# umautobots/LONER

Hardware: AMD Instinct MI355X
Metric: training rays/sec (higher is better)
Workload: dtype f32

## Files before the change

include/loner_hip.h:

```cpp
#ifndef LONER_HIP_H
#define LONER_HIP_H

#include <stddef.h>
#include <stdint.h>

#ifdef __cplusplus
extern "C" {
#endif

#define LNR_RAY_STRIDE 13
#define LNR_LOSS_RAYS_PER_BLOCK 4
#define LNR_MAX_LEVELS 32

typedef enum LnrStatus {
    LNR_OK = 0,
    LNR_ERR_INVALID_ARG = -1,
    LNR_ERR_UNSUPPORTED = -2,
    LNR_ERR_LAUNCH = -3,
    LNR_ERR_WORKSPACE = -4
} LnrStatus;

typedef enum LnrEncoding { LNR_ENC_HASHGRID = 0, LNR_ENC_FREQUENCY = 1 } LnrEncoding;

typedef enum LnrPrecision { LNR_PREC_F32 = 0, LNR_PREC_F16 = 1, LNR_PREC_F32_CHAIN = 2 } LnrPrecision;

typedef enum LnrPosRounding { LNR_POS_FMA = 0, LNR_POS_MUL_ADD = 1 } LnrPosRounding;

#define LNR_POISON_NAN_LOSS 1
#define LNR_POISON_POSE_GRAD 2
#define LNR_POISON_POSE 3

#define LNR_BWD_TABLE_ATOMICS 1
#define LNR_BWD_BINS 4
#define LNR_BWD_BINS_W8 8
#define LNR_BWD_DEFER_WEIGHT_FOLD 16
#define LNR_BWD_REPORT_REGIONS 2
#define LNR_BWD_OVERWRITE_GRAD 32

typedef enum LnrActivation {
    LNR_ACT_NONE = 0, LNR_ACT_RELU = 1, LNR_ACT_SINE = 2, LNR_ACT_LEAKY_RELU = 3,
    LNR_ACT_EXPONENTIAL = 4, LNR_ACT_SIGMOID = 5, LNR_ACT_SQUAREPLUS = 6,
    LNR_ACT_SOFTPLUS = 7, LNR_ACT_TANH = 8
} LnrActivation;

typedef struct LnrNetSpec {
    int32_t encoding;
    int32_t n_levels;
    int32_t n_features;
    int32_t log2_table;
    int32_t base_res;
    float   per_level_scale;
    int32_t n_frequencies;
    int32_t activation;
    int32_t n_neurons;
    int32_t n_hidden;
    int32_t precision;
    int32_t pos_rounding;
    int32_t enc_dim;
    int32_t in_dim;
    int32_t n_mlp_params;
    int64_t n_params;
    float    level_scale[LNR_MAX_LEVELS];
    uint32_t level_res[LNR_MAX_LEVELS];
    uint32_t level_size[LNR_MAX_LEVELS];
    uint32_t level_offset[LNR_MAX_LEVELS];
    uint32_t level_hashed[LNR_MAX_LEVELS];
} LnrNetSpec;

typedef struct LnrLossConfig {
    int32_t selection;
    float min_js, max_js, js_alpha;
    float los_lambda;
    float depth_lambda;
    float min_eps;
    float fixed_eps;
} LnrLossConfig;

const char* lnr_last_error(void);
int  lnr_version(void);

int lnr_profile_enable(int32_t on);
int lnr_profile_read(char* names, int32_t name_stride, float* total_ms, int32_t* calls, int32_t capacity);

int lnr_net_spec_finalize(LnrNetSpec* spec );

size_t lnr_density_workspace(const LnrNetSpec* spec , int64_t n_points);
size_t lnr_density_workspace_forward(const LnrNetSpec* spec , int64_t n_points);

typedef enum LnrRouteKind {
    LNR_ROUTE_UNSUPPORTED = 0, LNR_ROUTE_WIDE = 1, LNR_ROUTE_F16_FAST = 2, LNR_ROUTE_F16_FREQ = 3, LNR_ROUTE_F16_GEN = 4,
    LNR_ROUTE_BF3 = 5, LNR_ROUTE_FAST32 = 6, LNR_ROUTE_REGS = 7, LNR_ROUTE_LDS = 8
} LnrRouteKind;
typedef struct LnrDensityRoute { int32_t kind, w_lds, waves, dw64, f16_part; } LnrDensityRoute;
int lnr_density_route(const LnrNetSpec* spec , int64_t n_points, int32_t backward, LnrDensityRoute* out );

#define LNR_WORKSPACE_STATUS_BYTES 256
#define LNR_STATUS_CLIPPED 0
#define LNR_STATUS_OVF_LEVEL0 16
int lnr_density_workspace_init(void* workspace, size_t workspace_bytes, void* stream);
int lnr_density_workspace_release(void* workspace);

int lnr_density_forward(const LnrNetSpec* spec , const float* params,
                        const float* pts, int64_t n_points,
                        const float* rays, const float* z, int32_t n_rays, int32_t n_samples,
                        const int32_t* n_rays_dev,
                        float* sigma ,
                        void* workspace, size_t workspace_bytes, void* stream);

int lnr_density_backward(const LnrNetSpec* spec , const float* params,
                         const float* pts, int64_t n_points,
                         const float* rays, const float* z, int32_t n_rays, int32_t n_samples,
                         const int32_t* n_rays_dev,
                         const float* d_sigma, float* grad_params, float* d_pts, float* d_rays,
                         int32_t reuse_features, int32_t flags, void* workspace, size_t workspace_bytes,
                         void* input_grad_event ,
                         void* stream);

int lnr_density_fold_weight_grads(const LnrNetSpec* spec , int64_t n_points, float* grad_params,
                                  void* workspace, size_t workspace_bytes, int32_t flags, void* stream);

int lnr_build_lidar_rays(const float* directions , const float* distances ,
                         int64_t n_points, const int64_t* index , int32_t n_index,
                         const float* transform , float range_min, float range_max,
                         float scale, const float* shift ,
                         float* rays , float* depths ,
                         uint8_t* keep , void* stream);

int lnr_build_window_rays(const float* const* directions, const float* const* distances, const float* const_distance,
                          const int64_t* n_points, const int32_t* seg_start, const int32_t* seg_pose, int32_t n_seg,
                          const int64_t* index, int64_t* index_out, uint64_t seed, const float* transforms,
                          float range_min, float range_max, float scale, const float* shift ,
                          float* rays, float* depths, uint8_t* keep, void* stream);

int lnr_build_camera_rays(const float* directions , int64_t n_pixels, const int64_t* index ,
                          int32_t n_rays, int32_t width, const float* transform , float range_min, float scale,
                          const float* shift , float* rays , void* stream);

int lnr_pose_forward(const float* pose6, int32_t n, float* transforms, void* stream);
int lnr_pose_backward(const float* pose6, const float* d_transforms, const uint8_t* mask, int32_t n, float* d_pose6,
                      int32_t accumulate, int32_t* poison_dev, int32_t poison_tag, void* stream);

int lnr_compact_rays(const float* rays_in, const float* depths_in, const uint8_t* keep, const int64_t* src_index,
                     int32_t n_in, const int32_t* seg_start , int32_t n_seg,
                     float* rays_out, float* depths_out, int64_t* src_index_out,
                     int32_t* out_seg_start, int32_t* n_out_dev, void* stream);

int lnr_compact_rays_front(const float* rays_in, const float* depths_in, const uint8_t* keep, const int64_t* src_index,
                           int32_t n_in, const int32_t* seg_start , int32_t n_seg,
                           float* rays_out, float* depths_out, int64_t* src_index_out,
                           int32_t* out_seg_start, int32_t* n_out_dev,
                           int32_t* counts_dev , const int32_t* seg_order , int32_t cap,
                           float* record , void* stream);

int lnr_first_ray_key(const float* rays, const int32_t* out_seg_start , const int32_t* seg_order ,
                      int32_t n_seg, int64_t* key_out , void* stream);

#define LNR_FRONT_HEADER 4
int lnr_shard_front_pack(const float* rays, const int32_t* out_seg_start , const int32_t* seg_order ,
                         int32_t n_seg, const float* depths, int32_t n_rays, const int32_t* n_rays_dev, int32_t cap,
                         float* record , void* stream);
int lnr_shard_front_reduce(const float* records , int32_t world, int32_t stride,
                           int32_t* counts_dev , float* far0_dev , void* stream);

#define LNR_COMM_ID_BYTES 128
typedef enum LnrCommDtype { LNR_COMM_F32 = 0, LNR_COMM_BF16 = 1, LNR_COMM_I64 = 2, LNR_COMM_I32 = 3, LNR_COMM_U8 = 4 } LnrCommDtype;
typedef enum LnrCommOp { LNR_COMM_SUM = 0, LNR_COMM_MIN = 1, LNR_COMM_MAX = 2 } LnrCommOp;
int lnr_comm_available(void);
int lnr_comm_unique_id(void* id , size_t id_bytes);
int lnr_comm_init(const void* id, size_t id_bytes, int32_t rank, int32_t world, void** comm_out);
int lnr_comm_destroy(void* comm);
int lnr_comm_all_reduce(void* comm, void* buf, size_t count, int32_t dtype , int32_t op , void* stream);
int lnr_comm_reduce_scatter(void* comm, const void* send, void* recv, size_t recv_count, int32_t dtype, void* stream);
int lnr_comm_all_gather(void* comm, const void* send, void* recv, size_t bytes_per_rank, void* stream);
int lnr_comm_broadcast(void* comm, void* buf, size_t bytes, int32_t root, void* stream);

int lnr_lidar_rays_backward(const float* d_rays , const float* rays ,
                            const int64_t* src_index , const int32_t* seg_start ,
                            int32_t n_seg, const float* const* directions ,
                            const int64_t* n_points , const float* transforms ,
                            float scale, float* d_transform , void* stream);

int lnr_occ_interpolate(const float* grid , int32_t V, const float* pts ,
                        int64_t n, float* out , void* stream);

int lnr_sample_rays_occ(const float* rays, int32_t n_rays, const int32_t* n_rays_dev,
                        const float* grid, int32_t V, int32_t n_samples, float perturb,
                        const float* steps, const float* u_jitter, const float* u_pdf, uint64_t seed,
                        float* z_out ,
                        int64_t* dbg_inds, float* dbg_probs, float* dbg_cdf, void* stream);

int lnr_sample_rays_uniform(const float* rays, int32_t n_rays, const int32_t* n_rays_dev,
                            int32_t n_samples, float perturb, const float* steps,
                            const float* u_jitter, uint64_t seed, float* z_out, void* stream);

#define LNR_DRAW_JITTER 0
#define LNR_DRAW_PDF 1
#define LNR_DRAW_NOISE 2
#define LNR_DRAW_RAY_INDEX 16
int lnr_rng_draws(int32_t which, uint64_t seed, int32_t n_rays, int32_t n_per_ray, float* out , void* stream);

int lnr_render_forward(const float* sigma, const float* z, const float* rays, int32_t n_rays,
                       const int32_t* n_rays_dev, int32_t n_samples,
                       const float* noise, float noise_std, uint64_t seed,
                       float* depth, float* weights, float* opacity, float* variance, void* stream);

int lnr_render_forward_peak(const float* sigma, const float* z, const float* rays, int32_t n_rays,
                            const int32_t* n_rays_dev, int32_t n_samples,
                            const float* noise, float noise_std, uint64_t seed,
                            float* depth, float* opacity, float* variance, float* peak_z, int32_t* peak_index, void* stream);

int lnr_depth_colormap(const float* values, int64_t n, float multiplier, double min_depth, double max_depth,
                       const uint8_t* table , uint8_t* rgba , void* stream);

int lnr_render_backward(const float* sigma, const float* z, const float* rays, int32_t n_rays,
                        const int32_t* n_rays_dev, int32_t n_samples,
                        const float* noise, float noise_std, uint64_t seed,
                        const float* g_depth, const float* g_weights, const float* g_opacity,
                        const float* g_variance, float* d_sigma, float* d_rays, void* stream);

int lnr_points_grad_to_rays(const float* d_pts , const float* z, int32_t n_rays,
                            const int32_t* n_rays_dev, int32_t n_samples, float* d_rays, void* stream);

typedef struct LnrMeshGrid {
    int32_t n[3];
    float lo[3], hi[3];
    double first[3], inv_step[3];
    const double* axis[3];
} LnrMeshGrid;

int lnr_render_mesh_accumulate(const float* sigma, const float* z, const float* rays, int32_t n_rays, const int32_t* n_rays_dev,
                               int32_t n_samples, const float* noise, float noise_std, uint64_t seed, const LnrMeshGrid* grid,
                               float depth_max, int32_t use_var, float var_max, float* volume, uint64_t* counters, void* stream);

#define LNR_MC_TABLE_WIDTH 16
size_t lnr_mc_workspace(int32_t nx, int32_t ny, int32_t nz);
int lnr_mc_count(const float* volume, int32_t nx, int32_t ny, int32_t nz, float level, void* workspace, size_t workspace_bytes,
                 uint64_t* totals_dev, void* stream);
int lnr_mc_emit(const float* volume, int32_t nx, int32_t ny, int32_t nz, float level, const float* spacing ,
                const float* origin , void* workspace, size_t workspace_bytes, int64_t n_verts, int64_t n_tris,
                float* verts, int32_t* tris, void* stream);
int lnr_mc_case_table(int8_t* out);

size_t lnr_cloud_workspace(int64_t n_points);

int lnr_lidar_scan_points(const float* depth, const float* variance, const int64_t* ray_index, int64_t n_rays,
                          const float* directions, int64_t n_directions, float scale, float var_max, float depth_max,
                          void* workspace, size_t workspace_bytes, double* points, int32_t* n_points_dev, void* stream);

int lnr_voxel_down_sample(const double* points, int64_t n_points, const int32_t* n_points_dev, double voxel_size,
                          void* workspace, size_t workspace_bytes, double* out, int64_t* info_dev, void* stream);

int lnr_cloud_append_transformed(const double* src, int64_t n_points, const double* transform, double* dst, void* stream);

size_t lnr_nn_grid_bytes(int64_t n_targets);
int lnr_nn_grid_build(const double* targets, int64_t n_targets, double cell_edge, void* workspace, size_t workspace_bytes,
                      void* grid, size_t grid_bytes, int64_t* info_dev, void* stream);

int lnr_nn_distance(const void* grid, int64_t n_targets, const double* queries, int64_t n_queries, double* distance,
                    double* sq_distance, void* workspace, size_t workspace_bytes, int64_t* counters_dev, void* stream);

#define LNR_KNN_MAX 32
#define LNR_ICP_RESULT 64

int lnr_cloud_normals(const void* grid, int64_t n_points, int32_t knn, double* normals, double* covariances, void* workspace,
                      size_t workspace_bytes, int64_t* counters_dev, void* stream);

int lnr_icp_correspondences(const void* grid, int64_t n_targets, const double* queries, int64_t n_queries, double max_distance,
                            int32_t* index, double* sq_distance, int64_t* counters_dev, void* stream);

size_t lnr_icp_workspace(int64_t n_source);
int lnr_icp_point_to_plane(const void* grid, int64_t n_targets, const double* target_normals, const double* source, int64_t n_source,
                           double max_distance, const double* init, double relative_fitness, double relative_rmse, int32_t max_iteration,
                           void* workspace, size_t workspace_bytes, double* result_dev, int64_t* info_dev, void* stream);

size_t lnr_mesh_sample_workspace(int64_t n_triangles);
int lnr_mesh_sample_points(const double* vertices, int64_t n_vertices, const int32_t* triangles, int64_t n_triangles, int64_t n_points,
                           uint64_t seed, void* workspace, size_t workspace_bytes, double* points, int32_t* triangle_index,
                           int64_t* info_dev, void* stream);

size_t lnr_cloud_tools_workspace(int64_t n_points);

int lnr_cloud_knn_mean_distance(const void* grid, int64_t n_points, int32_t nb_neighbors, double* mean_distance, void* workspace,
                                size_t workspace_bytes, int64_t* counters_dev, void* stream);

int lnr_cloud_outlier_threshold(const void* grid, const double* mean_distance, int64_t n_points, double std_ratio, void* workspace,
                                size_t workspace_bytes, double* result_dev, void* stream);

int lnr_cloud_trajectory_transform(const double* points, const double* timestamps, int64_t n_points, const double* traj_times,
                                   const double* traj_positions, const double* traj_rotations, const double* traj_rotvecs,
                                   int64_t n_poses, double min_range, void* workspace, size_t workspace_bytes, double* out,
                                   int64_t* info_dev, void* stream);

#define LNR_MOCOMP_CONSTS 30
#define LNR_SKY_MAX_RAYS 65160

int lnr_frame_cloud(const float* ray_directions, const float* distances, int64_t n_points, int64_t start, int64_t stop, int64_t step,
                    double* points, void* stream);

int lnr_motion_compensate(float* ray_directions, float* distances, const void* timestamps, int32_t timestamps_fp64, int64_t n_points,
                          double t0, double denom, const double* consts , void* stream);

size_t lnr_sky_rays_workspace(void);
int lnr_sky_rays(const float* ray_directions, int64_t n_points, const float* rotation, void* workspace, size_t workspace_bytes,
                 float* sky, int64_t sky_stride, int32_t* info_dev, void* stream);

#define LNR_SCAN_MAX_FOV_SEGMENTS 8
#define LNR_SCAN_TIME_NONE 0
#define LNR_SCAN_TIME_GIVEN 1
#define LNR_SCAN_TIME_RECOMPUTE 2
#define LNR_SCAN_NANOSECONDS 1
#define LNR_SCAN_NEGATIVE_START 2
#define LNR_SCAN_LOCAL 4
#define LNR_SCAN_GLOBAL 8
#define LNR_SCAN_CONSTANT 16
#define LNR_SCAN_NO_TIMES 32

size_t lnr_scan_from_points_workspace(int64_t n_points);
int lnr_scan_from_points(const float* xyz, const float* point_times , int64_t n_points, int32_t time_mode, float stamp,
                         int32_t fov_enabled, const float* fov_segments , int32_t n_fov_segments, float min_range,
                         void* workspace, size_t workspace_bytes, float* ray_directions, float* distances, float* timestamps,
                         int64_t* order, int64_t* info_dev, void* stream);

int lnr_weights_gt(const float* s , const float* g , const float* eps_ray,
                   float eps_scalar, int32_t normalise, int32_t n_rays, int32_t n_samples,
                   float* out , void* stream);

int lnr_logits_grad(const float* s , const float* g , int32_t n_rays, int32_t n_samples,
                    float margin, float l_free, float l_occ, float* out, void* stream);

int lnr_render_ftb_gather(const float* rays, const float* z, int32_t n_samples, const int32_t* idx, const int32_t* n_alive_dev,
                          int32_t cap, int32_t b0, int32_t block_samples, float* rays_c , float* z_c ,
                          int32_t* next_count_dev, void* stream);
int lnr_render_ftb_composite(const float* sigma_c , const float* z, const float* rays, int32_t n_samples, const int32_t* idx,
                             const int32_t* n_alive_dev, int32_t cap, int32_t b0, int32_t block_samples,
                             const float* noise , float noise_std, uint64_t seed, float* transmittance, float* depth_acc, float* opacity_acc, int32_t* next_idx, int32_t* next_count_dev,
                             int32_t last, void* stream);

int lnr_count_opaque(const float* rays, const float* depth_gt, int32_t n_rays, const int32_t* n_rays_dev,
                     const float* far0_dev, int32_t* counts_dev , void* stream);
int lnr_los_loss_fused(const float* sigma, const float* z, const float* rays, const float* depth_gt,
                       int32_t n_rays, const int32_t* n_rays_dev, int32_t n_samples,
                       const float* noise, float noise_std, uint64_t seed,
                       float scale, const LnrLossConfig* cfg , const int32_t* counts_dev, const float* far0_dev,
                       float* loss_out, float* d_sigma, float* d_rays, float* ray_stats,
                       float* weights_out, float* block_partials, int32_t* poison_dev, int32_t poison_tag, void* stream);

int lnr_adam_step(float* params, float* grads, float* exp_avg, float* exp_avg_sq, int64_t count,
                  float lr, float beta1, float beta2, float eps, int32_t step, float grad_scale,
                  int32_t zero_grad, const int32_t* poison_dev, void* stream);

int lnr_occ_grid_step(float* grid, int32_t V, const float* rays, const float* z, const float* depth_gt,
                      int32_t n_rays, const int32_t* n_rays_dev, int32_t n_samples, float scale,
                      float lr, float margin, float l_free, float l_occ, int64_t* grad_acc, void* stream);
int lnr_occ_grid_apply(float* grid, int64_t* grad_acc, int64_t count, float lr, int32_t zero_grad, const int32_t* poison_dev,
                       void* stream);

int lnr_selftest_mfma(float* out , void* stream);

#ifdef __cplusplus
}
#endif
#endif
```

loner_amd/csrc/lnr_pose.hip:

```cpp
#include "lnr_common.h"

struct QuatParts { float w, x, y, z, k, theta, half; bool small; };

__device__ __forceinline__ QuatParts pose_quat(const float* __restrict__ p) {
    QuatParts q;
    const float a = p[3], b = p[4], c = p[5];
    q.theta = sqrtf(a * a + b * b + c * c);
    q.half = 0.5f * q.theta;
    q.small = fabsf(q.theta) < 1e-6f;
    q.k = q.small ? 0.5f - q.theta * q.theta / 48.0f : sinf(q.half) / q.theta;
    q.w = cosf(q.half); q.x = a * q.k; q.y = b * q.k; q.z = c * q.k;
    return q;
}

__global__ void pose_forward_kernel(const float* __restrict__ pose6, int n, float* __restrict__ T12) {
    const int i = blockIdx.x * blockDim.x + threadIdx.x;
    if (i >= n) return;
    const float* p = pose6 + 6 * i;
    const QuatParts q = pose_quat(p);
    const float w = q.w, x = q.x, y = q.y, z = q.z;
    const float s2 = 2.0f / (w * w + x * x + y * y + z * z);
    float* T = T12 + 12 * i;
    T[0] = 1.0f - s2 * (y * y + z * z); T[1] = s2 * (x * y - z * w);        T[2] = s2 * (x * z + y * w);        T[3] = p[0];
    T[4] = s2 * (x * y + z * w);        T[5] = 1.0f - s2 * (x * x + z * z); T[6] = s2 * (y * z - x * w);        T[7] = p[1];
    T[8] = s2 * (x * z - y * w);        T[9] = s2 * (y * z + x * w);        T[10] = 1.0f - s2 * (x * x + y * y); T[11] = p[2];
}

__global__ void pose_backward_kernel(const float* __restrict__ pose6, const float* __restrict__ dT12, const uint8_t* __restrict__ mask,
                                     int n, float* __restrict__ d_pose6, int accumulate, int32_t* __restrict__ poison, int32_t poison_tag) {
    const int i = blockIdx.x * blockDim.x + threadIdx.x;
    if (i >= n) return;
    const float* p = pose6 + 6 * i;
    const float* G = dT12 + 12 * i;
    const QuatParts q = pose_quat(p);
    const float w = q.w, x = q.x, y = q.y, z = q.z;
    const float nn = w * w + x * x + y * y + z * z;
    const float s2 = 2.0f / nn;
    const float G00 = G[0], G01 = G[1], G02 = G[2], G10 = G[4], G11 = G[5], G12 = G[6], G20 = G[8], G21 = G[9], G22 = G[10];
    const float d_s2 = -G00 * (y * y + z * z) + G01 * (x * y - z * w) + G02 * (x * z + y * w) + G10 * (x * y + z * w) - G11 * (x * x + z * z) +
                       G12 * (y * z - x * w) + G20 * (x * z - y * w) + G21 * (y * z + x * w) - G22 * (x * x + y * y);
    float dw = s2 * (-z * G01 + y * G02 + z * G10 - x * G12 - y * G20 + x * G21);
    float dx = s2 * (y * G01 + z * G02 + y * G10 - 2.0f * x * G11 - w * G12 + z * G20 + w * G21 - 2.0f * x * G22);
    float dy = s2 * (-2.0f * y * G00 + x * G01 + w * G02 + x * G10 + z * G12 - w * G20 + z * G21 - 2.0f * y * G22);
    float dz = s2 * (-2.0f * z * G00 - w * G01 + x * G02 + w * G10 - 2.0f * z * G11 + y * G12 + x * G20 + y * G21);
    const float ds2_dq = -0.5f * s2 * s2 * 2.0f;
    dw += d_s2 * ds2_dq * w; dx += d_s2 * ds2_dq * x; dy += d_s2 * ds2_dq * y; dz += d_s2 * ds2_dq * z;
    const float a = p[3], b = p[4], c = p[5];
    const float dk = q.small ? -q.theta / 24.0f : (0.5f * cosf(q.half) * q.theta - sinf(q.half)) / (q.theta * q.theta);
    const float d_theta = dk * (a * dx + b * dy + c * dz) - 0.5f * sinf(q.half) * dw;
    const float inv_theta = q.theta > 0.0f ? 1.0f / q.theta : 0.0f;
    const float m = mask ? (mask[i] ? 1.0f : 0.0f) : 1.0f;
    float out[6];
    out[0] = G[3]; out[1] = G[7]; out[2] = G[11];
    out[3] = q.k * dx + d_theta * a * inv_theta;
    out[4] = q.k * dy + d_theta * b * inv_theta;
    out[5] = q.k * dz + d_theta * c * inv_theta;
    float* o = d_pose6 + 6 * i;
    bool bad_grad = false, bad_pose = false;
    for (int j = 0; j < 6; ++j) {
        const float v = (accumulate ? o[j] : 0.0f) + (m != 0.0f ? out[j] : 0.0f);
        o[j] = v;
        bad_grad |= !isfinite(v);
        bad_pose |= !isfinite(p[j]);
    }
    if (poison != nullptr && (bad_grad || bad_pose) && atomicCAS(poison, 0, bad_grad ? LNR_POISON_POSE_GRAD : LNR_POISON_POSE) == 0)
        poison[1] = poison_tag;
}

extern "C" int lnr_pose_forward(const float* pose6, int32_t n, float* transforms, void* stream) {
    LNR_REQUIRE(pose6 && transforms && n >= 0, "lnr_pose_forward: bad argument");
    if (n == 0) return LNR_OK;
    hipLaunchKernelGGL(pose_forward_kernel, dim3(lnr_div_up(n, 64)), dim3(64), 0, (hipStream_t)stream, pose6, n, transforms);
    LNR_CHECK_LAUNCH("lnr_pose_forward");
    return LNR_OK;
}

extern "C" int lnr_pose_backward(const float* pose6, const float* d_transforms, const uint8_t* mask, int32_t n, float* d_pose6,
                                 int32_t accumulate, int32_t* poison_dev, int32_t poison_tag, void* stream) {
    LNR_REQUIRE(pose6 && d_transforms && d_pose6 && n >= 0, "lnr_pose_backward: bad argument");
    if (n == 0) return LNR_OK;
    hipLaunchKernelGGL(pose_backward_kernel, dim3(lnr_div_up(n, 64)), dim3(64), 0, (hipStream_t)stream, pose6, d_transforms, mask, n,
                       d_pose6, accumulate, poison_dev, poison_tag);
    LNR_CHECK_LAUNCH("lnr_pose_backward");
    return LNR_OK;
}
```

loner_amd/csrc/lnr_rays.hip:

```cpp
#include "lnr_common.h"

#define LNR_MAX_SEG 64

struct SegTable {
    int32_t n;
    int32_t start[LNR_MAX_SEG + 1];
};
struct DirTable {
    const float* dirs[LNR_MAX_SEG];
    int64_t n_points[LNR_MAX_SEG];
};

__device__ __forceinline__ float cube_exit(const float o[3], const float d[3], int* axis_out, float* t_out, float* dd_out) {
    float best = 0.0f;
    int best_axis = 0;
    float best_t = 0.0f, best_dd = 1.0f;
#pragma unroll
    for (int a = 0; a < 3; ++a) {
        const float dd = d[a] + 1e-15f;
        const float t_lo = (-1.0f - o[a]) / dd;
        const float t_hi = (1.0f - o[a]) / dd;
        const float c_lo = fmaxf(t_lo, 0.0f), c_hi = fmaxf(t_hi, 0.0f);
        const bool hi_sel = c_hi > c_lo;
        const float c = hi_sel ? c_hi : c_lo;
        const float t_raw = hi_sel ? t_hi : t_lo;
        if (a == 0 || c < best) { best = c; best_axis = a; best_t = t_raw; best_dd = dd; }
    }
    if (axis_out) { *axis_out = best_axis; *t_out = best_t; *dd_out = best_dd; }
    return best;
}

__global__ void build_lidar_rays_kernel(const float* __restrict__ directions, const float* __restrict__ distances, int64_t n_points,
                                        const int64_t* __restrict__ index, int n_index, const float* __restrict__ T,
                                        float range_min, float range_max, float scale, float sx, float sy, float sz,
                                        float* __restrict__ rays, float* __restrict__ depths, uint8_t* __restrict__ keep) {
    const int i = blockIdx.x * blockDim.x + threadIdx.x;
    if (i >= n_index) return;
    const int64_t src = index[i];
    const float l0 = directions[src], l1 = directions[n_points + src], l2 = directions[2 * n_points + src];
    const float dist = distances[src];
    float o[3], d[3];
    o[0] = (T[3] + sx) / scale;
    o[1] = (T[7] + sy) / scale;
    o[2] = (T[11] + sz) / scale;
    float v[3];
#pragma unroll
    for (int r = 0; r < 3; ++r) v[r] = T[4 * r] * l0 + T[4 * r + 1] * l1 + T[4 * r + 2] * l2;
    const float nrm = sqrtf(v[0] * v[0] + v[1] * v[1] + v[2] * v[2]);
#pragma unroll
    for (int r = 0; r < 3; ++r) d[r] = v[r] / nrm;
    const float near = range_min / scale;
    const float far_range = range_max / scale;
    const float far = fminf(far_range, cube_exit(o, d, nullptr, nullptr, nullptr));
    float* rec = rays + (size_t)i * LNR_RAY_STRIDE;
    rec[0] = o[0]; rec[1] = o[1]; rec[2] = o[2];
    rec[3] = d[0]; rec[4] = d[1]; rec[5] = d[2];
    rec[6] = -d[0]; rec[7] = -d[1]; rec[8] = -d[2];
    rec[9] = 0.0f; rec[10] = 0.0f;
    rec[11] = near; rec[12] = far;
    depths[i] = dist / scale;
    keep[i] = (far > near + 1.0f / scale) ? 1 : 0;
}

extern "C" int lnr_build_lidar_rays(const float* directions, const float* distances, int64_t n_points, const int64_t* index,
                                    int32_t n_index, const float* transform, float range_min, float range_max, float scale,
                                    const float* shift, float* rays, float* depths, uint8_t* keep, void* stream) {
    LNR_REQUIRE(directions && distances && index && transform && shift && rays && depths && keep, "lnr_build_lidar_rays: null argument");
    LNR_REQUIRE(n_points > 0 && n_index >= 0 && scale > 0.0f, "lnr_build_lidar_rays: bad sizes");
    if (n_index == 0) return LNR_OK;
    hipLaunchKernelGGL(build_lidar_rays_kernel, dim3(lnr_div_up(n_index, 256)), dim3(256), 0, (hipStream_t)stream, directions, distances,
                       n_points, index, n_index, transform, range_min, range_max, scale, shift[0], shift[1], shift[2], rays, depths, keep);
    LNR_CHECK_LAUNCH("lnr_build_lidar_rays");
    return LNR_OK;
}

struct WindowTable {
    int32_t n_seg;
    int32_t start[LNR_MAX_SEG + 1];
    int32_t pose[LNR_MAX_SEG];
    const float* dirs[LNR_MAX_SEG];
    const float* dist[LNR_MAX_SEG];
    float const_dist[LNR_MAX_SEG];
    int64_t n_points[LNR_MAX_SEG];
};

__global__ void build_window_rays_kernel(const WindowTable tab, const int64_t* __restrict__ index, int64_t* __restrict__ index_out,
                                         uint64_t seed, const float* __restrict__ transforms, float range_min, float range_max,
                                         float scale, float sx, float sy, float sz, float* __restrict__ rays,
                                         float* __restrict__ depths, uint8_t* __restrict__ keep) {
    const int i = blockIdx.x * blockDim.x + threadIdx.x;
    const int total = tab.start[tab.n_seg];
    if (i >= total) return;
    int seg = 0;
    while (seg + 1 < tab.n_seg && i >= tab.start[seg + 1]) ++seg;
    const int64_t n_points = tab.n_points[seg];
    int64_t src;
    if (index) src = index[i];
    else {
        const float u = lnr_rand_uniform(seed, 0x44ull + (uint64_t)seg, (uint64_t)(i - tab.start[seg]) >> 2, (uint32_t)(i - tab.start[seg]) & 3u);
        src = (int64_t)(u * (float)n_points);
        if (src >= n_points) src = n_points - 1;
    }
    if (index_out) index_out[i] = src;
    const float* D = tab.dirs[seg];
    const float l0 = D[src], l1 = D[n_points + src], l2 = D[2 * n_points + src];
    const float dist = tab.dist[seg] ? tab.dist[seg][src] : tab.const_dist[seg];
    const float* T = transforms + 12 * tab.pose[seg];
    float o[3], d[3], v[3];
    o[0] = (T[3] + sx) / scale; o[1] = (T[7] + sy) / scale; o[2] = (T[11] + sz) / scale;
#pragma unroll
    for (int r = 0; r < 3; ++r) v[r] = T[4 * r] * l0 + T[4 * r + 1] * l1 + T[4 * r + 2] * l2;
    const float nrm = sqrtf(v[0] * v[0] + v[1] * v[1] + v[2] * v[2]);
#pragma unroll
    for (int r = 0; r < 3; ++r) d[r] = v[r] / nrm;
    const float near = range_min / scale;
    const float far = fminf(range_max / scale, cube_exit(o, d, nullptr, nullptr, nullptr));
    float* rec = rays + (size_t)i * LNR_RAY_STRIDE;
    rec[0] = o[0]; rec[1] = o[1]; rec[2] = o[2];
    rec[3] = d[0]; rec[4] = d[1]; rec[5] = d[2];
    rec[6] = -d[0]; rec[7] = -d[1]; rec[8] = -d[2];
    rec[9] = 0.0f; rec[10] = 0.0f; rec[11] = near; rec[12] = far;
    depths[i] = dist / scale;
    keep[i] = (far > near + 1.0f / scale) ? 1 : 0;
}

extern "C" int lnr_build_window_rays(const float* const* directions, const float* const* distances, const float* const_distance,
                                     const int64_t* n_points, const int32_t* seg_start, const int32_t* seg_pose, int32_t n_seg,
                                     const int64_t* index, int64_t* index_out, uint64_t seed, const float* transforms,
                                     float range_min, float range_max, float scale, const float* shift, float* rays, float* depths,
                                     uint8_t* keep, void* stream) {
    LNR_REQUIRE(directions && distances && const_distance && n_points && seg_start && seg_pose && transforms && shift && rays && depths && keep,
                "lnr_build_window_rays: null argument");
    LNR_REQUIRE(n_seg >= 1 && n_seg <= LNR_MAX_SEG, "lnr_build_window_rays: n_seg must be in [1,%d]", LNR_MAX_SEG);
    LNR_REQUIRE(index != nullptr || index_out != nullptr, "lnr_build_window_rays: need index or index_out");
    WindowTable tab;
    tab.n_seg = n_seg;
    for (int s = 0; s < n_seg; ++s) {
        tab.start[s] = seg_start[s]; tab.pose[s] = seg_pose[s]; tab.dirs[s] = directions[s]; tab.dist[s] = distances[s];
        tab.const_dist[s] = const_distance[s]; tab.n_points[s] = n_points[s];
        LNR_REQUIRE(directions[s] != nullptr && n_points[s] > 0, "lnr_build_window_rays: segment %d has no points", s);
    }
    tab.start[n_seg] = seg_start[n_seg];
    const int total = seg_start[n_seg];
    if (total <= 0) return LNR_OK;
    hipLaunchKernelGGL(build_window_rays_kernel, dim3(lnr_div_up(total, 256)), dim3(256), 0, (hipStream_t)stream, tab, index, index_out, seed,
                       transforms, range_min, range_max, scale, shift[0], shift[1], shift[2], rays, depths, keep);
    LNR_CHECK_LAUNCH("lnr_build_window_rays");
    return LNR_OK;
}

__global__ void build_camera_rays_kernel(const float* __restrict__ directions, int64_t n_pixels, const int64_t* __restrict__ index, int n_rays, int width,
                                         const float* __restrict__ T, float range_min, float scale, float sx, float sy, float sz,
                                         float* __restrict__ rays) {
// ... 13 lines not shown
    o[2] = (T[11] + sz) / scale;
#pragma unroll
    for (int r = 0; r < 3; ++r) v[r] = T[4 * r] * l0 + T[4 * r + 1] * l1 + T[4 * r + 2] * l2;
    const float nrm = sqrtf(v[0] * v[0] + v[1] * v[1] + v[2] * v[2]);
#pragma unroll
    for (int r = 0; r < 3; ++r) d[r] = v[r] / nrm;
    rec[0] = o[0]; rec[1] = o[1]; rec[2] = o[2];
    rec[3] = d[0]; rec[4] = d[1]; rec[5] = d[2];
    rec[6] = -d[0]; rec[7] = -d[1]; rec[8] = -d[2];
    rec[9] = (float)(src % width); rec[10] = (float)(src / width);
    rec[11] = range_min / scale;
    rec[12] = cube_exit(o, d, nullptr, nullptr, nullptr);
}

extern "C" int lnr_build_camera_rays(const float* directions, int64_t n_pixels, const int64_t* index, int32_t n_rays, int32_t width,
                                     const float* transform, float range_min, float scale, const float* shift, float* rays, void* stream) {
    LNR_REQUIRE(directions && transform && shift && rays, "lnr_build_camera_rays: null argument");
    LNR_REQUIRE(n_pixels > 0 && n_rays >= 0 && width > 0 && scale > 0.0f, "lnr_build_camera_rays: bad sizes");
    LNR_REQUIRE(index != nullptr || (int64_t)n_rays <= n_pixels, "lnr_build_camera_rays: %d rays of an image of %lld pixels", n_rays, (long long)n_pixels);
    if (n_rays == 0) return LNR_OK;
    hipLaunchKernelGGL(build_camera_rays_kernel, dim3(lnr_div_up(n_rays, 256)), dim3(256), 0, (hipStream_t)stream, directions, n_pixels, index,
                       n_rays, width, transform, range_min, scale, shift[0], shift[1], shift[2], rays);
    LNR_CHECK_LAUNCH("lnr_build_camera_rays");
    return LNR_OK;
}

struct SegOrder { int n; int order[LNR_MAX_SEG]; };
struct CompactTail { int32_t* counts; float* record; int cap; SegOrder ord; };

__global__ void __launch_bounds__(1024)
compact_rays_kernel(const float* __restrict__ rays_in, const float* __restrict__ depths_in, const uint8_t* __restrict__ keep,
                    const int64_t* __restrict__ src_in, int n_in, const SegTable seg, float* __restrict__ rays_out,
                    float* __restrict__ depths_out, int64_t* __restrict__ src_out, int32_t* __restrict__ out_seg_start,
                    int32_t* __restrict__ n_out, const CompactTail tail) {
    __shared__ int wave_tot[16];
    __shared__ int running;
    const int tid = threadIdx.x, lane = tid & 63, wave = tid >> 6;
    if (tid == 0) running = 0;
    __syncthreads();
    for (int base = 0; base < n_in; base += 1024) {
        const int i = base + tid;
        const bool k = (i < n_in) && keep[i];
        const unsigned long long b = __ballot(k);
        const int within = __popcll(b & ((1ull << lane) - 1ull));
        if (lane == 0) wave_tot[wave] = __popcll(b);
        __syncthreads();
        int before = running;
        for (int w = 0; w < wave; ++w) before += wave_tot[w];
        const int pos = before + within;
        if (i < n_in) {
            for (int s = 0; s <= seg.n; ++s) if (seg.start[s] == i) out_seg_start[s] = pos;
        }
        if (k) {
            const float* a = rays_in + (size_t)i * LNR_RAY_STRIDE;
            float* o = rays_out + (size_t)pos * LNR_RAY_STRIDE;
#pragma unroll
            for (int c = 0; c < LNR_RAY_STRIDE; ++c) o[c] = a[c];
            depths_out[pos] = depths_in[i];
            if (src_out) src_out[pos] = src_in[i];
        }
        __syncthreads();
        if (tid == 0) { int t = 0; for (int w = 0; w < 16; ++w) t += wave_tot[w]; running += t; }
        __syncthreads();
    }
    if (tid <= seg.n && seg.start[tid] >= n_in) out_seg_start[tid] = running;
    if (tid == 0) *n_out = running;
    if (tail.counts == nullptr && tail.record == nullptr) return;
    __syncthreads();
    const int n = running;
    if (tail.counts != nullptr) {
        __shared__ int partial[16];
        const float far0 = n > 0 ? rays_out[12] : 0.0f;
        int c = 0;
        for (int i = tid; i < n; i += 1024) {
            const float d = depths_out[i];
            c += ((d > 0.0f) && !(d > far0)) ? 1 : 0;
        }
        for (int o = 32; o > 0; o >>= 1) c += __shfl_xor(c, o, 64);
        if (lane == 0) partial[wave] = c;
        __syncthreads();
        if (tid == 0) {
            int t = 0;
            for (int w = 0; w < 16; ++w) t += partial[w];
            tail.counts[0] = n;
            tail.counts[1] = t;
        }
    }
    if (tail.record != nullptr) {
        const int m = min(n, tail.cap);
        if (tid == 0) {
            long long k = 0x7FFFFFFFFFFFFFFFll;
            for (int sgi = 0; sgi < tail.ord.n; ++sgi) {
                const int lo = out_seg_start[sgi], hi = out_seg_start[sgi + 1];
                if (hi > lo) {
                    k = ((long long)tail.ord.order[sgi] << 32) | (long long)__float_as_uint(rays_out[(size_t)lo * LNR_RAY_STRIDE + 12]);
                    break;
                }
            }
            tail.record[0] = __uint_as_float((uint32_t)((unsigned long long)k & 0xFFFFFFFFull));
            tail.record[1] = __uint_as_float((uint32_t)((unsigned long long)k >> 32));
            tail.record[2] = __int_as_float(m);
            tail.record[3] = 0.0f;
        }
        for (int i = tid; i < tail.cap; i += 1024) tail.record[LNR_FRONT_HEADER + i] = i < m ? depths_out[i] : 0.0f;
    }
}

extern "C" int lnr_compact_rays(const float* rays_in, const float* depths_in, const uint8_t* keep, const int64_t* src_index, int32_t n_in,
                                const int32_t* seg_start, int32_t n_seg, float* rays_out, float* depths_out, int64_t* src_index_out,
                                int32_t* out_seg_start, int32_t* n_out_dev, void* stream) {
    LNR_REQUIRE(rays_in && depths_in && keep && seg_start && rays_out && depths_out && out_seg_start && n_out_dev, "lnr_compact_rays: null argument");
    LNR_REQUIRE(n_seg >= 1 && n_seg <= LNR_MAX_SEG, "lnr_compact_rays: n_seg must be in [1,%d]", LNR_MAX_SEG);
    LNR_REQUIRE((src_index == nullptr) == (src_index_out == nullptr), "lnr_compact_rays: src_index in/out must both be given or both be null");
    SegTable seg;
    seg.n = n_seg;
    for (int s = 0; s <= n_seg; ++s) seg.start[s] = seg_start[s];
    LNR_REQUIRE(seg.start[0] == 0 && seg.start[n_seg] == n_in, "lnr_compact_rays: seg_start must run from 0 to n_in");
    CompactTail tail;
    tail.counts = nullptr; tail.record = nullptr; tail.cap = 0; tail.ord.n = 0;
    hipLaunchKernelGGL(compact_rays_kernel, dim3(1), dim3(1024), 0, (hipStream_t)stream, rays_in, depths_in, keep, src_index, n_in, seg,
                       rays_out, depths_out, src_index_out, out_seg_start, n_out_dev, tail);
    LNR_CHECK_LAUNCH("lnr_compact_rays");
    return LNR_OK;
}

extern "C" int lnr_compact_rays_front(const float* rays_in, const float* depths_in, const uint8_t* keep, const int64_t* src_index, int32_t n_in,
                                      const int32_t* seg_start, int32_t n_seg, float* rays_out, float* depths_out, int64_t* src_index_out,
                                      int32_t* out_seg_start, int32_t* n_out_dev, int32_t* counts_dev, const int32_t* seg_order, int32_t cap,
                                      float* record, void* stream) {
    LNR_REQUIRE(rays_in && depths_in && keep && seg_start && rays_out && depths_out && out_seg_start && n_out_dev, "lnr_compact_rays_front: null argument");
    LNR_REQUIRE(n_seg >= 1 && n_seg <= LNR_MAX_SEG, "lnr_compact_rays_front: n_seg must be in [1,%d]", LNR_MAX_SEG);
    LNR_REQUIRE((src_index == nullptr) == (src_index_out == nullptr), "lnr_compact_rays_front: src_index in/out must both be given or both be null");
    LNR_REQUIRE((counts_dev != nullptr) != (record != nullptr), "lnr_compact_rays_front: pass counts_dev (unsharded batch) or record (sharded), one of them");
    SegTable seg;
    seg.n = n_seg;
    for (int s = 0; s <= n_seg; ++s) seg.start[s] = seg_start[s];
    LNR_REQUIRE(seg.start[0] == 0 && seg.start[n_seg] == n_in, "lnr_compact_rays_front: seg_start must run from 0 to n_in");
    CompactTail tail;
    tail.counts = counts_dev; tail.record = record; tail.cap = cap; tail.ord.n = 0;
    if (record != nullptr) {
        LNR_REQUIRE(seg_order != nullptr && cap >= n_in, "lnr_compact_rays_front: a front record of %d depth slots cannot hold the %d candidate rays of this rank", cap, n_in);
        tail.ord.n = n_seg;
        for (int s = 0; s < n_seg; ++s) {
            LNR_REQUIRE(seg_order[s] >= 0 && (s == 0 || seg_order[s] > seg_order[s - 1]), "lnr_compact_rays_front: seg_order must be non-negative and ascending");
            tail.ord.order[s] = seg_order[s];
        }
    }
    hipLaunchKernelGGL(compact_rays_kernel, dim3(1), dim3(1024), 0, (hipStream_t)stream, rays_in, depths_in, keep, src_index, n_in, seg,
                       rays_out, depths_out, src_index_out, out_seg_start, n_out_dev, tail);
    LNR_CHECK_LAUNCH("lnr_compact_rays_front");
    return LNR_OK;
}

__global__ void first_ray_key_kernel(const float* __restrict__ rays, const int32_t* __restrict__ out_seg_start, const SegOrder ord, long long* __restrict__ key) {
    if (threadIdx.x != 0 || blockIdx.x != 0) return;
    long long k = 0x7FFFFFFFFFFFFFFFll;
    for (int s = 0; s < ord.n; ++s) {
        const int lo = out_seg_start[s], hi = out_seg_start[s + 1];
        if (hi > lo) {
            k = ((long long)ord.order[s] << 32) | (long long)__float_as_uint(rays[(size_t)lo * LNR_RAY_STRIDE + 12]);
            break;
        }
    }
    *key = k;
}

extern "C" int lnr_first_ray_key(const float* rays, const int32_t* out_seg_start, const int32_t* seg_order, int32_t n_seg, int64_t* key_out, void* stream) {
    LNR_REQUIRE(rays && out_seg_start && seg_order && key_out, "lnr_first_ray_key: null argument");
    LNR_REQUIRE(n_seg >= 1 && n_seg <= LNR_MAX_SEG, "lnr_first_ray_key: n_seg must be in [1,%d]", LNR_MAX_SEG);
    SegOrder ord;
    ord.n = n_seg;
    for (int s = 0; s < n_seg; ++s) {
        LNR_REQUIRE(seg_order[s] >= 0 && (s == 0 || seg_order[s] > seg_order[s - 1]), "lnr_first_ray_key: seg_order must be non-negative and ascending");
        ord.order[s] = seg_order[s];
    }
    hipLaunchKernelGGL(first_ray_key_kernel, dim3(1), dim3(64), 0, (hipStream_t)stream, rays, out_seg_start, ord, reinterpret_cast<long long*>(key_out));
    LNR_CHECK_LAUNCH("lnr_first_ray_key");
    return LNR_OK;
}

__global__ void __launch_bounds__(256)
shard_front_pack_kernel(const float* __restrict__ rays, const int32_t* __restrict__ out_seg_start, const SegOrder ord,
                        const float* __restrict__ depths, int n_rays, const int32_t* __restrict__ n_rays_dev, int cap, float* __restrict__ rec) {
    const int n = min(lnr_live_rays(n_rays, n_rays_dev), cap);
    if (threadIdx.x == 0) {
        long long k = 0x7FFFFFFFFFFFFFFFll;
        for (int s = 0; s < ord.n; ++s) {
            const int lo = out_seg_start[s], hi = out_seg_start[s + 1];
            if (hi > lo) {
                k = ((long long)ord.order[s] << 32) | (long long)__float_as_uint(rays[(size_t)lo * LNR_RAY_STRIDE + 12]);
                break;
            }
        }
        rec[0] = __uint_as_float((uint32_t)((unsigned long long)k & 0xFFFFFFFFull));
        rec[1] = __uint_as_float((uint32_t)((unsigned long long)k >> 32));
        rec[2] = __int_as_float(n);
        rec[3] = 0.0f;
    }
    for (int i = threadIdx.x; i < cap; i += blockDim.x) rec[LNR_FRONT_HEADER + i] = i < n ? depths[i] : 0.0f;
}

__global__ void __launch_bounds__(1024)
shard_front_reduce_kernel(const float* __restrict__ recs, int world, int stride, int32_t* __restrict__ counts, float* __restrict__ far0_out) {
    __shared__ int partial[16];
    unsigned long long kmin = 0x7FFFFFFFFFFFFFFFull;
    int n_all = 0;
    for (int r = 0; r < world; ++r) {
        const float* rec = recs + (size_t)r * stride;
        const unsigned long long k = (unsigned long long)__float_as_uint(rec[0]) | ((unsigned long long)__float_as_uint(rec[1]) << 32);
        kmin = k < kmin ? k : kmin;
        n_all += max(0, min(__float_as_int(rec[2]), stride - LNR_FRONT_HEADER));
    }
    const float far0 = __uint_as_float((uint32_t)(kmin & 0xFFFFFFFFull));
    int c = 0;
    for (int r = 0; r < world; ++r) {
        const float* rec = recs + (size_t)r * stride;
        const int n = max(0, min(__float_as_int(rec[2]), stride - LNR_FRONT_HEADER));
        for (int i = threadIdx.x; i < n; i += blockDim.x) {
            const float d = rec[LNR_FRONT_HEADER + i];
            c += ((d > 0.0f) && !(d > far0)) ? 1 : 0;
        }
    }
    for (int o = 32; o > 0; o >>= 1) c += __shfl_xor(c, o, 64);
    if ((threadIdx.x & 63) == 0) partial[threadIdx.x >> 6] = c;
    __syncthreads();
    if (threadIdx.x == 0) {
        int t = 0;
        for (int w = 0; w < (int)(blockDim.x >> 6); ++w) t += partial[w];
        counts[0] = n_all;
        counts[1] = t;
        far0_out[0] = far0;
    }
}

extern "C" int lnr_shard_front_pack(const float* rays, const int32_t* out_seg_start, const int32_t* seg_order, int32_t n_seg,
                                    const float* depths, int32_t n_rays, const int32_t* n_rays_dev, int32_t cap, float* record, void* stream) {
    LNR_REQUIRE(record && cap >= 0 && n_rays >= 0 && n_seg >= 0 && n_seg <= LNR_MAX_SEG, "lnr_shard_front_pack: bad argument");
    LNR_REQUIRE(n_seg == 0 || (rays && out_seg_start && seg_order && depths), "lnr_shard_front_pack: null argument");
    LNR_REQUIRE(n_seg == 0 || n_rays <= cap, "lnr_shard_front_pack: a front record of %d depth slots cannot hold the %d rays of this rank "
                "(every rank must size its record for the fullest rank: DistContext.front_capacity)", cap, n_rays);
    SegOrder ord;
    ord.n = n_seg;
    for (int s = 0; s < n_seg; ++s) {
        LNR_REQUIRE(seg_order[s] >= 0 && (s == 0 || seg_order[s] > seg_order[s - 1]), "lnr_shard_front_pack: seg_order must be non-negative and ascending");
        ord.order[s] = seg_order[s];
    }
    hipLaunchKernelGGL(shard_front_pack_kernel, dim3(1), dim3(256), 0, (hipStream_t)stream, rays, out_seg_start, ord, depths,
                       n_seg == 0 ? 0 : n_rays, n_seg == 0 ? nullptr : n_rays_dev, cap, record);
    LNR_CHECK_LAUNCH("lnr_shard_front_pack");
    return LNR_OK;
}

extern "C" int lnr_shard_front_reduce(const float* records, int32_t world, int32_t stride, int32_t* counts_dev, float* far0_dev, void* stream) {
    LNR_REQUIRE(records && counts_dev && far0_dev && world >= 1 && stride >= LNR_FRONT_HEADER, "lnr_shard_front_reduce: bad argument");
    hipLaunchKernelGGL(shard_front_reduce_kernel, dim3(1), dim3(1024), 0, (hipStream_t)stream, records, world, stride, counts_dev, far0_dev);
    LNR_CHECK_LAUNCH("lnr_shard_front_reduce");
    return LNR_OK;
}

__global__ void __launch_bounds__(256)
lidar_rays_backward_kernel(const float* __restrict__ d_rays, const float* __restrict__ rays, const int64_t* __restrict__ src_index,
                           const int32_t* __restrict__ seg_start, const DirTable dirs, const float* __restrict__ transforms,
                           float scale, float far_range_unused, float* __restrict__ d_transform) {
    __shared__ float red[4][12];
    const int seg = blockIdx.x;
    const int lo = seg_start[seg], hi = seg_start[seg + 1];
    const float* T = transforms + seg * 12;
    const float* D = dirs.dirs[seg];
    const int64_t n = dirs.n_points[seg];
    float acc[12];
#pragma unroll
    for (int k = 0; k < 12; ++k) acc[k] = 0.0f;
    for (int ray = lo + threadIdx.x; ray < hi; ray += blockDim.x) {
        const float* g = d_rays + (size_t)ray * LNR_RAY_STRIDE;
        const float* rec = rays + (size_t)ray * LNR_RAY_STRIDE;
        const int64_t src = src_index[ray];
        const float l[3] = {D[src], D[n + src], D[2 * n + src]};
        float go[3] = {g[0], g[1], g[2]};
        float gd[3] = {g[3] - g[6], g[4] - g[7], g[5] - g[8]};
        const float gfar = g[12];
        const float o[3] = {rec[0], rec[1], rec[2]};
        const float d[3] = {rec[3], rec[4], rec[5]};
        if (gfar != 0.0f) {
            int axis; float t_raw, dd;
            const float clip = cube_exit(o, d, &axis, &t_raw, &dd);
            if (clip <= rec[12] && t_raw > 0.0f) {
                const float inv = 1.0f / dd;
                const float go_a = -gfar * inv, gd_a = -gfar * t_raw * inv;
                if (axis == 0) { go[0] += go_a; gd[0] += gd_a; } else if (axis == 1) { go[1] += go_a; gd[1] += gd_a; } else { go[2] += go_a; gd[2] += gd_a; }
            }
        }
        float v[3];
#pragma unroll
        for (int r = 0; r < 3; ++r) v[r] = T[4 * r] * l[0] + T[4 * r + 1] * l[1] + T[4 * r + 2] * l[2];
        const float nrm = sqrtf(v[0] * v[0] + v[1] * v[1] + v[2] * v[2]);
        const float dot = d[0] * gd[0] + d[1] * gd[1] + d[2] * gd[2];
#pragma unroll
        for (int r = 0; r < 3; ++r) {
            const float gv = (gd[r] - d[r] * dot) / nrm;
            acc[4 * r + 0] += gv * l[0];
            acc[4 * r + 1] += gv * l[1];
            acc[4 * r + 2] += gv * l[2];
            acc[4 * r + 3] += go[r] / scale;
        }
    }
    const int lane = threadIdx.x & 63, wave = threadIdx.x >> 6;
// ... 22 lines not shown
```

loner_amd/csrc/lnr_render.hip:

```cpp
#include "lnr_common.h"
#include "lnr_render_ray.h"

__device__ __forceinline__ float wave_excl_suffix_sum(float v, int lane) {
    float inc = v;
#pragma unroll
    for (int o = 1; o < 64; o <<= 1) {
        float t = __shfl_down(inc, o, 64);
        if (lane + o < 64) inc += t;
    }
    float ex = __shfl_down(inc, 1, 64);
    return lane == 63 ? 0.0f : ex;
}

template <int C>
__device__ __forceinline__ void render_ray_backward(const RayState<C>& st, const float G[C], float g_far, int ray, int S, int lane,
                                                    const float* __restrict__ rayrec, float* __restrict__ d_sigma,
                                                    float* __restrict__ d_rays) {
    const int base = lane * C;
    float gw[C];
    float local = 0.0f;
#pragma unroll
    for (int t = 0; t < C; ++t) { gw[t] = G[t] * st.w[t]; local += gw[t]; }
    const float behind_lanes = wave_excl_suffix_sum(local, lane);
    float suffix = behind_lanes;
// ... 41 lines not shown
    if (lane == 0) {
        if (depth) depth[ray] = st.depth;
        if (opacity) opacity[ray] = st.opacity;
        if (variance) variance[ray] = st.variance;
    }
}

template <int C>
__global__ void __launch_bounds__(RENDER_BLOCK)
render_backward_kernel(const float* __restrict__ sigma, const float* __restrict__ z, const float* __restrict__ rays, int n_rays,
                       const int32_t* __restrict__ n_rays_dev, int S, const float* __restrict__ noise, float noise_std,
                       uint64_t seed, const float* __restrict__ g_depth, const float* __restrict__ g_weights,
                       const float* __restrict__ g_opacity, const float* __restrict__ g_variance,
                       float* __restrict__ d_sigma, float* __restrict__ d_rays) {
    const int lane = threadIdx.x & 63;
    const int ray = blockIdx.x * RAYS_PER_BLOCK + (threadIdx.x >> 6);
    if (ray >= lnr_live_rays(n_rays, n_rays_dev)) return;
    const float* rr = rays + (size_t)ray * LNR_RAY_STRIDE;
    RayState<C> st;
    render_ray<C>(st, sigma, z, noise, noise_std, seed, ray, S, lane, rr);
    const float gD = g_depth ? g_depth[ray] : 0.0f;
    const float gO = g_opacity ? g_opacity[ray] : 0.0f;
    const float gV = g_variance ? g_variance[ray] : 0.0f;
    float q_part = 0.0f;
#pragma unroll
    for (int t = 0; t < C; ++t) q_part += st.w[t] * (st.depth - st.z[t]);
    const float gD_tot = gD + gV * 2.0f * wave_sum(q_part);
    const float far = rr[12];
    float G[C];
#pragma unroll
    for (int t = 0; t < C; ++t) {
        const int i = lane * C + t;
        const float q = st.depth - st.z[t];
        float g = gO + gD_tot * (st.z[t] - far) + gV * q * q;
        if (g_weights && i < S) g += g_weights[(size_t)ray * S + i];
        G[t] = (i < S) ? g : 0.0f;
    }
    render_ray_backward<C>(st, G, gD_tot * (1.0f - st.opacity), ray, S, lane, rr, d_sigma, d_rays);
}

__device__ __forceinline__ float std_normal_cdf(float x) { return 0.5f * (1.0f + erff(x / 1.41421356237309515f)); }

__device__ __forceinline__ float target_raw(float s, float g, float eps, float sd, float clip_norm) {
    const bool inside = (s - (g - eps) > 0.0f) && ((g + eps) - s > 0.0f);
    if (!inside) return 0.0f;
    const float t = (s - g) / sd;
    return 0.39894228040143270f * expf(-0.5f * (t * t)) / sd / clip_norm;
}

__device__ __forceinline__ void target_params(float g, float eps, float* sd, float* clip_norm) {
    *sd = eps / 3.0f;
    const float lo = (g - eps - g) / *sd;
    const float hi = (g + eps - g) / *sd;
    *clip_norm = std_normal_cdf(hi) - std_normal_cdf(lo);
}

__device__ __forceinline__ float gaussian_kl(float m1, float s1, float m2, float s2) {
    const float d = m1 - m2;
    return logf(s2 / s1) + (s1 * s1 + d * d) / (2.0f * (s2 * s2)) - 0.5f;
}
__device__ __forceinline__ float gaussian_js(float m1, float s1, float m2, float s2) {
    const float mm = 0.5f * (m1 + m2);
    const float sm = 0.5f * sqrtf(s1 * s1 + s2 * s2);
    return 0.5f * gaussian_kl(m1, s1, mm, sm) + 0.5f * gaussian_kl(m2, s2, mm, sm);
}

template <int C>
__device__ __forceinline__ void los_loss_ray(const float* __restrict__ sigma, const float* __restrict__ z, const float* __restrict__ rays,
                                             const float* __restrict__ depth_gt, int S, const float* __restrict__ noise, float noise_std,
                                             uint64_t seed, float scale, const LnrLossConfig& cfg, const int32_t* __restrict__ counts,
                                             float* terms, bool terms_atomic, float* __restrict__ d_sigma, float* __restrict__ d_rays,
                                             float* __restrict__ ray_stats, float* __restrict__ weights_out, int ray, int lane,
                                             const float* __restrict__ far0_dev) {
    const float* rr = rays + (size_t)ray * LNR_RAY_STRIDE;
    RayState<C> st;
    render_ray<C>(st, sigma, z, noise, noise_std, seed, ray, S, lane, rr);

    const float dgt = depth_gt[ray];
    const float far0 = far0_dev ? far0_dev[0] : rays[12];
    const bool opaque = (dgt > 0.0f) && !(dgt > far0);
    const float g = dgt * scale;
    const float n_all = (float)counts[0] * (float)S;
    const float n_op = (float)counts[1];

    float m_part = 0.0f;
#pragma unroll
    for (int t = 0; t < C; ++t) m_part += (st.z[t] * scale) * st.w[t];
    const float wden = st.opacity + 1e-10f;
    const float mean = wave_sum(m_part) / wden;
    float v_part = 0.0f;
#pragma unroll
    for (int t = 0; t < C; ++t) { const float q = st.z[t] * scale - mean; v_part += q * q * st.w[t]; }
    const float var = wave_sum(v_part) / wden + 1e-10f;
    const float sd_pred = sqrtf(var);
    const float js = gaussian_js(g, cfg.min_eps / 3.0f, mean, sd_pred);

    float eps;
    if (cfg.selection <= 1) {
        float score = js;
        if (score < cfg.min_js) score = 0.0f;
        if (score > cfg.max_js) score = cfg.max_js;
        eps = cfg.min_eps * (1.0f + cfg.js_alpha * score);
    } else {
        eps = cfg.fixed_eps;
    }
    float sd_t, clip_norm;
    target_params(g, eps, &sd_t, &clip_norm);
    float raw[C];
    float r_part = 0.0f;
#pragma unroll
    for (int t = 0; t < C; ++t) {
        raw[t] = (lane * C + t < S) ? target_raw(st.z[t] * scale, g, eps, sd_t, clip_norm) : 0.0f;
        r_part += raw[t];
    }
    const float rden = wave_sum(r_part) + 1e-6f;

    const bool l1 = (cfg.selection == 0 || cfg.selection == 2);
    const float depth_m = st.depth * scale;
    const float gO = opaque ? ((st.opacity - 1.0f > 0.0f) ? 1.0f : (st.opacity - 1.0f < 0.0f ? -1.0f : 0.0f)) / n_op : 0.0f;
    const float gD = opaque ? cfg.depth_lambda * 2.0f * (depth_m - g) * scale / n_op : 0.0f;
    const float far = rr[12];
    float G[C];
    float los_part = 0.0f;
#pragma unroll
    for (int t = 0; t < C; ++t) {
        const int i = lane * C + t;
        const float target = opaque ? raw[t] / rden : 0.0f;
        const float diff = st.w[t] - target;
        float gw;
        if (l1) { los_part += fabsf(diff); gw = (diff > 0.0f ? 1.0f : (diff < 0.0f ? -1.0f : 0.0f)); }
        else { los_part += diff * diff; gw = 2.0f * diff; }
        G[t] = (i < S) ? cfg.los_lambda * gw / n_all + gO + gD * (st.z[t] - far) : 0.0f;
        if (weights_out && i < S) weights_out[(size_t)ray * S + i] = st.w[t];
    }
    const float los_sum = wave_sum(los_part);
    render_ray_backward<C>(st, G, gD * (1.0f - st.opacity), ray, S, lane, rr, d_sigma, d_rays);

    if (lane == 0) {
        const float l_depth = opaque ? cfg.depth_lambda * (depth_m - g) * (depth_m - g) / n_op : 0.0f;
        const float l_los = cfg.los_lambda * los_sum / n_all;
        const float l_op = opaque ? fabsf(st.opacity - 1.0f) / n_op : 0.0f;
        const float t5[5] = {l_depth + l_los + l_op, l_depth, l_los, l_op, eps};
#pragma unroll
        for (int q = 0; q < 5; ++q) { if (terms_atomic) atomicAdd(terms + q, t5[q]); else terms[q] = t5[q]; }
        if (ray_stats) {
            float* o = ray_stats + (size_t)ray * 8;
            o[0] = st.depth; o[1] = st.opacity; o[2] = st.variance; o[3] = mean; o[4] = sd_pred; o[5] = js; o[6] = eps;
            o[7] = opaque ? 1.0f : 0.0f;
        }
    }
}


template <int C>
__global__ void __launch_bounds__(RENDER_BLOCK)
los_loss_fused_kernel(const float* __restrict__ sigma, const float* __restrict__ z, const float* __restrict__ rays,
                      const float* __restrict__ depth_gt, int n_rays, const int32_t* __restrict__ n_rays_dev, int S,
                      const float* __restrict__ noise, float noise_std, uint64_t seed, float scale, const LnrLossConfig cfg,
                      const int32_t* __restrict__ counts, float* __restrict__ loss_out, float* __restrict__ d_sigma,
                      float* __restrict__ d_rays, float* __restrict__ ray_stats, float* __restrict__ weights_out,
                      float* __restrict__ block_partials, const float* __restrict__ far0_dev) {
    __shared__ float s_terms[RAYS_PER_BLOCK][5];
    const int lane = threadIdx.x & 63;
    const int ray = blockIdx.x * RAYS_PER_BLOCK + (threadIdx.x >> 6);
    const bool alive = ray < lnr_live_rays(n_rays, n_rays_dev);
    if (block_partials) {
        if (lane < 5) s_terms[threadIdx.x >> 6][lane] = 0.0f;
        if (alive) los_loss_ray<C>(sigma, z, rays, depth_gt, S, noise, noise_std, seed, scale, cfg, counts, s_terms[threadIdx.x >> 6], false,
                                   d_sigma, d_rays, ray_stats, weights_out, ray, lane, far0_dev);
        __syncthreads();
        if (threadIdx.x < 8) {
            float v = 0.0f;
            if (threadIdx.x < 5) for (int r = 0; r < RAYS_PER_BLOCK; ++r) v += s_terms[r][threadIdx.x];
            block_partials[(size_t)blockIdx.x * 8 + threadIdx.x] = v;
        }
    } else if (alive) {
        los_loss_ray<C>(sigma, z, rays, depth_gt, S, noise, noise_std, seed, scale, cfg, counts, loss_out, true,
                        d_sigma, d_rays, ray_stats, weights_out, ray, lane, far0_dev);
    }
}

__global__ void loss_reduce_kernel(const float* __restrict__ block_partials, int n_blocks, float* __restrict__ loss_out,
                                   int32_t* __restrict__ poison, int32_t poison_tag) {
    __shared__ float part[4][8];
    const int term = threadIdx.x & 7, slice = threadIdx.x >> 3;
    float v = 0.0f;
    for (int b = slice; b < n_blocks; b += 32) v += block_partials[(size_t)b * 8 + term];
    v += __shfl_xor(v, 8, 64); v += __shfl_xor(v, 16, 64); v += __shfl_xor(v, 32, 64);
    if ((threadIdx.x & 63) < 8) part[threadIdx.x >> 6][term] = v;
    __syncthreads();
    if (threadIdx.x < 5) {
        const float t = loss_out[threadIdx.x] + (part[0][threadIdx.x] + part[1][threadIdx.x] + part[2][threadIdx.x] + part[3][threadIdx.x]);
        loss_out[threadIdx.x] = t;
        if (threadIdx.x == 0 && poison != nullptr && t != t && atomicCAS(poison, 0, LNR_POISON_NAN_LOSS) == 0) poison[1] = poison_tag;
    }
}

__global__ void count_opaque_kernel(const float* __restrict__ rays, const float* __restrict__ depth_gt, int n_rays,
                                    const int32_t* __restrict__ n_rays_dev, int32_t* __restrict__ counts,
                                    const float* __restrict__ far0_dev) {
    __shared__ int partial[16];
    const int n = lnr_live_rays(n_rays, n_rays_dev);
    const float far0 = far0_dev ? far0_dev[0] : (n > 0 ? rays[12] : 0.0f);
    int c = 0;
    for (int i = threadIdx.x; i < n; i += blockDim.x) {
        const float d = depth_gt[i];
        c += ((d > 0.0f) && !(d > far0)) ? 1 : 0;
    }
    for (int o = 32; o > 0; o >>= 1) c += __shfl_xor(c, o, 64);
    if ((threadIdx.x & 63) == 0) partial[threadIdx.x >> 6] = c;
    __syncthreads();
    if (threadIdx.x == 0) {
        int t = 0;
        for (int w = 0; w < (int)(blockDim.x >> 6); ++w) t += partial[w];
        counts[0] = n;
        counts[1] = t;
    }
}

__global__ void weights_gt_kernel(const float* __restrict__ s, const float* __restrict__ g, const float* __restrict__ eps_ray,
                                  float eps_scalar, int normalise, int n_rays, int S, float* __restrict__ out) {
    const int lane = threadIdx.x & 63;
    const int ray = blockIdx.x * RAYS_PER_BLOCK + (threadIdx.x >> 6);
    if (ray >= n_rays) return;
    const float gg = g[ray];
    const float eps = eps_ray ? eps_ray[ray] : eps_scalar;
    float sd, cn;
    target_params(gg, eps, &sd, &cn);
    float part = 0.0f;
    for (int i = lane; i < S; i += 64) part += target_raw(s[(size_t)ray * S + i], gg, eps, sd, cn);
    const float den = wave_sum(part) + 1e-6f;
    for (int i = lane; i < S; i += 64) {
        const float v = target_raw(s[(size_t)ray * S + i], gg, eps, sd, cn);
        out[(size_t)ray * S + i] = normalise ? v / den : v;
    }
}

__global__ void logits_grad_kernel(const float* __restrict__ s, const float* __restrict__ g, int64_t total, int S, float margin,
                                   float l_free, float l_occ, float* __restrict__ out) {
    const int64_t i = (int64_t)blockIdx.x * blockDim.x + threadIdx.x;
    if (i >= total) return;
    const float x = s[i] - g[i / S];
    const float free_side = (-x - margin > 0.0f) ? 1.0f : 0.0f;
    const float near_surface = ((x + margin > 0.0f) && (margin - x > 0.0f)) ? 1.0f : 0.0f;
    out[i] = l_free * free_side - l_occ * near_surface;
}

__global__ void points_grad_to_rays_kernel(const float* __restrict__ d_pts, const float* __restrict__ z, int n_rays,
                                           const int32_t* __restrict__ n_rays_dev, int S, float* __restrict__ d_rays) {
    const int lane = threadIdx.x & 63;
    const int ray = blockIdx.x * RAYS_PER_BLOCK + (threadIdx.x >> 6);
    if (ray >= lnr_live_rays(n_rays, n_rays_dev)) return;
    float a[6] = {0.0f, 0.0f, 0.0f, 0.0f, 0.0f, 0.0f};
    for (int i = lane; i < S; i += 64) {
        const size_t m = (size_t)ray * S + i;
        const float zv = z[m];
        const float gx = d_pts[3 * m], gy = d_pts[3 * m + 1], gz = d_pts[3 * m + 2];
        a[0] += gx; a[1] += gy; a[2] += gz;
        a[3] += zv * gx; a[4] += zv * gy; a[5] += zv * gz;
    }
#pragma unroll
    for (int k = 0; k < 6; ++k) a[k] = wave_sum(a[k]);
    if (lane < 6) {
        float v = lane == 0 ? a[0] : lane == 1 ? a[1] : lane == 2 ? a[2] : lane == 3 ? a[3] : lane == 4 ? a[4] : a[5];
        d_rays[(size_t)ray * LNR_RAY_STRIDE + lane] += v;
    }
}


extern "C" int lnr_render_forward(const float* sigma, const float* z, const float* rays, int32_t n_rays, const int32_t* n_rays_dev,
                                  int32_t n_samples, const float* noise, float noise_std, uint64_t seed, float* depth,
                                  float* weights, float* opacity, float* variance, void* stream) {
    LNR_REQUIRE(sigma && z && rays && n_rays >= 0 && n_samples >= 2, "lnr_render_forward: bad argument");
    if (n_rays == 0) return LNR_OK;
    const dim3 grid(lnr_div_up(n_rays, RAYS_PER_BLOCK)), block(RENDER_BLOCK);
    hipStream_t st = (hipStream_t)stream;
    DISPATCH_C(n_samples, hipLaunchKernelGGL(render_forward_kernel<C>, grid, block, C >= 16 ? RAYS_PER_BLOCK * 64 * (C + 4) * sizeof(float) : 0, st,
                                             sigma, z, rays, n_rays, n_rays_dev, n_samples, noise, noise_std, seed, depth, weights, opacity, variance));
    LNR_CHECK_LAUNCH("lnr_render_forward");
    return LNR_OK;
}

#define FTB_T_MIN 5.9604644775390625e-08f

__global__ void __launch_bounds__(RENDER_BLOCK)
ftb_gather_kernel(const float* __restrict__ rays, const float* __restrict__ z, int S, const int32_t* __restrict__ idx,
                  const int32_t* __restrict__ n_alive, int cap, int b0, int B, float* __restrict__ rays_c, float* __restrict__ z_c,
                  int32_t* __restrict__ next_count) {
    if (blockIdx.x == 0 && threadIdx.x == 0) *next_count = 0;
    const int lane = threadIdx.x & 63;
    const int n = min(*n_alive, cap);
    for (int j = blockIdx.x * RAYS_PER_BLOCK + (threadIdx.x >> 6); j < n; j += gridDim.x * RAYS_PER_BLOCK) {
        const int ray = idx[j];
        if (lane < LNR_RAY_STRIDE) rays_c[(size_t)j * LNR_RAY_STRIDE + lane] = rays[(size_t)ray * LNR_RAY_STRIDE + lane];
        const float* src = z + (size_t)ray * S + b0;
        float* dst = z_c + (size_t)j * B;
        for (int i = 4 * lane; i < B; i += 256) *reinterpret_cast<float4*>(dst + i) = *reinterpret_cast<const float4*>(src + i);
    }
}

__global__ void __launch_bounds__(RENDER_BLOCK)
ftb_composite_kernel(const float* __restrict__ sigma_c, const float* __restrict__ z, const float* __restrict__ rays, int S,
                     const int32_t* __restrict__ idx, const int32_t* __restrict__ n_alive, int cap, int b0, const float* __restrict__ noise,
                     float noise_std, uint64_t seed, float* __restrict__ T_ray, float* __restrict__ depth_acc, float* __restrict__ opac_acc,
                     int32_t* __restrict__ next_idx, int32_t* __restrict__ next_count, int last) {
    constexpr int C = 4, B = 64 * C;
    const int lane = threadIdx.x & 63;
    const int n = min(*n_alive, cap);
    for (int j = blockIdx.x * RAYS_PER_BLOCK + (threadIdx.x >> 6); j < n; j += gridDim.x * RAYS_PER_BLOCK) {
        const int ray = idx[j];
        const float* rec = rays + (size_t)ray * LNR_RAY_STRIDE;
        const float dnorm = sqrtf(rec[3] * rec[3] + rec[4] * rec[4] + rec[5] * rec[5]);
        const int i0 = b0 + C * lane;
        const float4 zv = *reinterpret_cast<const float4*>(z + (size_t)ray * S + i0);
        const float4 sv = *reinterpret_cast<const float4*>(sigma_c + (size_t)j * B + C * lane);
        const float zl[C] = {zv.x, zv.y, zv.z, zv.w};
        float dens[C] = {sv.x, sv.y, sv.z, sv.w};
        if (noise != nullptr) {
            const float4 nv = *reinterpret_cast<const float4*>(noise + (size_t)ray * S + i0);
            dens[0] += nv.x; dens[1] += nv.y; dens[2] += nv.z; dens[3] += nv.w;
        } else if (noise_std > 0.0f) {
#pragma unroll
            for (int t = 0; t < C; ++t) dens[t] += lnr_rand_normal(seed, (uint64_t)ray, (uint32_t)(i0 + t)) * noise_std;
        }
        float z_after = __shfl_down(zl[0], 1, 64);
        if (lane == 63) z_after = (b0 + B < S) ? z[(size_t)ray * S + b0 + B] : 0.0f;
        float e[C], Tl[C], tprod = 1.0f;
#pragma unroll
        for (int t = 0; t < C; ++t) {
            const int i = i0 + t;
            float delta = (i < S - 1) ? ((t + 1 < C) ? zl[(t + 1 < C) ? t + 1 : t] : z_after) - zl[t] : 1e10f;
            delta *= dnorm;
            const float r = dens[t] > 0.0f ? dens[t] : 0.0f;
            e[t] = expf(-delta * r);
            Tl[t] = tprod;
            tprod *= (1.0f - (1.0f - e[t]) + 1e-10f);
        }
        const float prefix = wave_excl_prod(tprod, lane) * T_ray[ray];
        float o_part = 0.0f, d_part = 0.0f;
#pragma unroll
        for (int t = 0; t < C; ++t) {
            const float w = (1.0f - e[t]) * (Tl[t] * prefix);
            o_part += w;
            d_part += w * zl[t];
        }
        const float o_sum = wave_sum(o_part), d_sum = wave_sum(d_part);
        const float T_out = __shfl(prefix * tprod, 63, 64);
        if (lane == 0) {
            depth_acc[ray] += d_sum;
            opac_acc[ray] += o_sum;
            T_ray[ray] = T_out;
            if (!last && T_out >= FTB_T_MIN) next_idx[atomicAdd(next_count, 1)] = ray;
        }
    }
}

extern "C" int lnr_render_ftb_gather(const float* rays, const float* z, int32_t n_samples, const int32_t* idx, const int32_t* n_alive_dev,
                                     int32_t cap, int32_t b0, int32_t block_samples, float* rays_c, float* z_c, int32_t* next_count_dev,
                                     void* stream) {
    LNR_REQUIRE(rays && z && idx && n_alive_dev && rays_c && z_c && next_count_dev, "lnr_render_ftb_gather: null argument");
    LNR_REQUIRE(cap >= 0 && block_samples > 0 && block_samples % 4 == 0 && b0 >= 0 && b0 % 4 == 0 && b0 + block_samples <= n_samples && n_samples % 4 == 0,
                "lnr_render_ftb_gather: a block must lie inside the ray's samples (multiples of four)");
    if (cap == 0) return LNR_OK;
    const int blocks = lnr_div_up(cap, RAYS_PER_BLOCK);
    hipLaunchKernelGGL(ftb_gather_kernel, dim3(blocks > 4096 ? 4096 : blocks), dim3(RENDER_BLOCK), 0, (hipStream_t)stream, rays, z, n_samples, idx,
                       n_alive_dev, cap, b0, block_samples, rays_c, z_c, next_count_dev);
    LNR_CHECK_LAUNCH("lnr_render_ftb_gather");
    return LNR_OK;
}

extern "C" int lnr_render_ftb_composite(const float* sigma_c, const float* z, const float* rays, int32_t n_samples, const int32_t* idx,
                                        const int32_t* n_alive_dev, int32_t cap, int32_t b0, int32_t block_samples, const float* noise, float noise_std,
                                        uint64_t seed, float* transmittance, float* depth_acc, float* opacity_acc, int32_t* next_idx, int32_t* next_count_dev,
                                        int32_t last, void* stream) {
    LNR_REQUIRE(sigma_c && z && rays && idx && n_alive_dev && transmittance && depth_acc && opacity_acc && next_idx && next_count_dev,
                "lnr_render_ftb_composite: null argument");
    LNR_REQUIRE(block_samples == 256, "lnr_render_ftb_composite: blocks of 256 samples (one wave per ray, four samples per lane)");
    LNR_REQUIRE(cap >= 0 && b0 >= 0 && b0 % 4 == 0 && b0 + block_samples <= n_samples && n_samples % 4 == 0, "lnr_render_ftb_composite: a block must lie inside the ray's samples");
    if (cap == 0) return LNR_OK;
    const int blocks = lnr_div_up(cap, RAYS_PER_BLOCK);
    hipLaunchKernelGGL(ftb_composite_kernel, dim3(blocks > 4096 ? 4096 : blocks), dim3(RENDER_BLOCK), 0, (hipStream_t)stream, sigma_c, z, rays, n_samples,
                       idx, n_alive_dev, cap, b0, noise, noise_std, seed, transmittance, depth_acc, opacity_acc, next_idx, next_count_dev, last);
    LNR_CHECK_LAUNCH("lnr_render_ftb_composite");
    return LNR_OK;
}

extern "C" int lnr_render_backward(const float* sigma, const float* z, const float* rays, int32_t n_rays, const int32_t* n_rays_dev,
                                   int32_t n_samples, const float* noise, float noise_std, uint64_t seed, const float* g_depth,
                                   const float* g_weights, const float* g_opacity, const float* g_variance, float* d_sigma,
                                   float* d_rays, void* stream) {
    LNR_REQUIRE(sigma && z && rays && d_sigma && d_rays && n_rays >= 0 && n_samples >= 2, "lnr_render_backward: bad argument");
    if (n_rays == 0) return LNR_OK;
    const dim3 grid(lnr_div_up(n_rays, RAYS_PER_BLOCK)), block(RENDER_BLOCK);
    hipStream_t st = (hipStream_t)stream;
    DISPATCH_C(n_samples, hipLaunchKernelGGL(render_backward_kernel<C>, grid, block, 0, st, sigma, z, rays, n_rays, n_rays_dev, n_samples,
                                             noise, noise_std, seed, g_depth, g_weights, g_opacity, g_variance, d_sigma, d_rays));
    LNR_CHECK_LAUNCH("lnr_render_backward");
    return LNR_OK;
}

extern "C" int lnr_count_opaque(const float* rays, const float* depth_gt, int32_t n_rays, const int32_t* n_rays_dev,
                                const float* far0_dev, int32_t* counts_dev, void* stream) {
    LNR_REQUIRE(counts_dev && n_rays >= 0 && (n_rays == 0 || (rays && depth_gt)), "lnr_count_opaque: bad argument");
    hipLaunchKernelGGL(count_opaque_kernel, dim3(1), dim3(1024), 0, (hipStream_t)stream, rays, depth_gt, n_rays, n_rays_dev, counts_dev,
                       far0_dev);
    LNR_CHECK_LAUNCH("lnr_count_opaque");
    return LNR_OK;
}

extern "C" int lnr_los_loss_fused(const float* sigma, const float* z, const float* rays, const float* depth_gt, int32_t n_rays,
                                  const int32_t* n_rays_dev, int32_t n_samples, const float* noise, float noise_std, uint64_t seed,
                                  float scale, const LnrLossConfig* cfg, const int32_t* counts_dev, const float* far0_dev, float* loss_out,
                                  float* d_sigma, float* d_rays, float* ray_stats, float* weights_out, float* block_partials,
                                  int32_t* poison_dev, int32_t poison_tag, void* stream) {
    LNR_REQUIRE(sigma && z && rays && depth_gt && cfg && counts_dev && loss_out && d_sigma && d_rays, "lnr_los_loss_fused: null argument");
    LNR_REQUIRE(poison_dev == nullptr || block_partials != nullptr, "lnr_los_loss_fused: the failure guard needs block_partials (the deterministic reduction)");
    LNR_REQUIRE(cfg->selection >= 0 && cfg->selection <= 3, "lnr_los_loss_fused: unknown loss selection %d", cfg->selection);
    LNR_REQUIRE(n_rays >= 0 && n_samples >= 2, "lnr_los_loss_fused: bad sizes");
    if (n_rays == 0) return LNR_OK;
    const dim3 grid(lnr_div_up(n_rays, RAYS_PER_BLOCK)), block(RENDER_BLOCK);
    hipStream_t st = (hipStream_t)stream;
    DISPATCH_C(n_samples, hipLaunchKernelGGL(los_loss_fused_kernel<C>, grid, block, 0, st, sigma, z, rays, depth_gt, n_rays, n_rays_dev,
                                             n_samples, noise, noise_std, seed, scale, *cfg, counts_dev, loss_out, d_sigma, d_rays,
                                             ray_stats, weights_out, block_partials, far0_dev));
    LNR_CHECK_LAUNCH("lnr_los_loss_fused");
    if (block_partials) {
        hipLaunchKernelGGL(loss_reduce_kernel, dim3(1), dim3(256), 0, st, block_partials, (int)grid.x, loss_out, poison_dev, poison_tag);
        LNR_CHECK_LAUNCH("lnr_los_loss_fused(reduce)");
    }
    return LNR_OK;
}

extern "C" int lnr_weights_gt(const float* s, const float* g, const float* eps_ray, float eps_scalar, int32_t normalise,
                              int32_t n_rays, int32_t n_samples, float* out, void* stream) {
    LNR_REQUIRE(s && g && out && n_rays >= 0 && n_samples > 0, "lnr_weights_gt: bad argument");
    if (n_rays == 0) return LNR_OK;
    hipLaunchKernelGGL(weights_gt_kernel, dim3(lnr_div_up(n_rays, RAYS_PER_BLOCK)), dim3(RENDER_BLOCK), 0, (hipStream_t)stream, s, g,
                       eps_ray, eps_scalar, normalise, n_rays, n_samples, out);
    LNR_CHECK_LAUNCH("lnr_weights_gt");
    return LNR_OK;
}

extern "C" int lnr_logits_grad(const float* s, const float* g, int32_t n_rays, int32_t n_samples, float margin, float l_free,
                               float l_occ, float* out, void* stream) {
    LNR_REQUIRE(s && g && out && n_rays >= 0 && n_samples > 0, "lnr_logits_grad: bad argument");
    const int64_t total = (int64_t)n_rays * n_samples;
    if (total == 0) return LNR_OK;
    hipLaunchKernelGGL(logits_grad_kernel, dim3(lnr_div_up(total, 256)), dim3(256), 0, (hipStream_t)stream, s, g, total, n_samples,
                       margin, l_free, l_occ, out);
    LNR_CHECK_LAUNCH("lnr_logits_grad");
    return LNR_OK;
}

extern "C" int lnr_points_grad_to_rays(const float* d_pts, const float* z, int32_t n_rays, const int32_t* n_rays_dev,
                                       int32_t n_samples, float* d_rays, void* stream) {
    LNR_REQUIRE(d_pts && z && d_rays && n_rays >= 0 && n_samples > 0, "lnr_points_grad_to_rays: bad argument");
    if (n_rays == 0) return LNR_OK;
    hipLaunchKernelGGL(points_grad_to_rays_kernel, dim3(lnr_div_up(n_rays, RAYS_PER_BLOCK)), dim3(RENDER_BLOCK), 0, (hipStream_t)stream,
                       d_pts, z, n_rays, n_rays_dev, n_samples, d_rays);
    LNR_CHECK_LAUNCH("lnr_points_grad_to_rays");
    return LNR_OK;
}


__global__ void noise_draws_kernel(uint64_t seed, int n_rays, int n_per_ray, float* __restrict__ out) {
    const int64_t i = (int64_t)blockIdx.x * blockDim.x + threadIdx.x;
    if (i >= (int64_t)n_rays * n_per_ray) return;
    out[i] = lnr_rand_normal(seed, (uint64_t)(i / n_per_ray), (uint32_t)(i % n_per_ray));
}

int lnr_render_noise_draws(uint64_t seed, int n_rays, int n_per_ray, float* out, hipStream_t st) {
    const int64_t n = (int64_t)n_rays * n_per_ray;
    hipLaunchKernelGGL(noise_draws_kernel, dim3((unsigned)((n + 255) / 256)), dim3(256), 0, st, seed, n_rays, n_per_ray, out);
    LNR_CHECK_LAUNCH("lnr_rng_draws");
    return LNR_OK;
}
```

loner_amd/hip.py:

```python
import ctypes as C
import os

import torch

_HERE = os.path.dirname(os.path.abspath(__file__))
LIB_PATH = os.environ.get("LNR_LIB_PATH") or os.path.join(_HERE, "_lib", "libloner_hip.so")

MAX_LEVELS = 32
RAY_STRIDE = 13
LOSS_RAYS_PER_BLOCK = 4
FRONT_HEADER = 4
KNN_MAX = 32
ICP_RESULT = 64
MOCOMP_CONSTS = 30
SKY_MAX_RAYS = 65160
SCAN_MAX_FOV_SEGMENTS = 8
SCAN_TIME_NONE, SCAN_TIME_GIVEN, SCAN_TIME_RECOMPUTE = 0, 1, 2
SCAN_NANOSECONDS, SCAN_NEGATIVE_START, SCAN_LOCAL, SCAN_GLOBAL, SCAN_CONSTANT, SCAN_NO_TIMES = 1, 2, 4, 8, 16, 32

ENCODINGS = {"HashGrid": 0, "Grid": 0, "Frequency": 1}
ACTIVATIONS = {"None": 0, "ReLU": 1, "Sine": 2, "LeakyReLU": 3, "Exponential": 4, "Sigmoid": 5,
               "Squareplus": 6, "Softplus": 7, "Tanh": 8}
LOSS_SELECTIONS = {"L1_JS": 0, "L2_JS": 1, "L1_LOS": 2, "L2_LOS": 3}
PRECISIONS = {"fp32": 0, "float32": 0, "fp16": 1, "half": 1, "float16": 1, "fp32_chain": 2}
POS_ROUNDINGS = {"fma": 0, "mul_add": 1}
BWD_TABLE_ATOMICS = 1
BWD_REPORT_REGIONS = 2
BWD_DEFER_WEIGHT_FOLD = 16
BWD_BINS = 4
BWD_BINS_W8 = 8
BWD_OVERWRITE_GRAD = 32
WORKSPACE_STATUS_BYTES, STATUS_CLIPPED = 256, 0
DRAW_JITTER, DRAW_PDF, DRAW_NOISE, DRAW_RAY_INDEX = 0, 1, 2, 16
POISON_NAN_LOSS, POISON_POSE_GRAD, POISON_POSE = 1, 2, 3


class NetSpec(C.Structure):
    _fields_ = [("encoding", C.c_int32), ("n_levels", C.c_int32), ("n_features", C.c_int32),
                ("log2_table", C.c_int32), ("base_res", C.c_int32), ("per_level_scale", C.c_float),
                ("n_frequencies", C.c_int32), ("activation", C.c_int32), ("n_neurons", C.c_int32),
                ("n_hidden", C.c_int32), ("precision", C.c_int32), ("pos_rounding", C.c_int32),
                ("enc_dim", C.c_int32), ("in_dim", C.c_int32), ("n_mlp_params", C.c_int32),
                ("n_params", C.c_int64),
                ("level_scale", C.c_float * MAX_LEVELS), ("level_res", C.c_uint32 * MAX_LEVELS),
                ("level_size", C.c_uint32 * MAX_LEVELS), ("level_offset", C.c_uint32 * MAX_LEVELS),
                ("level_hashed", C.c_uint32 * MAX_LEVELS)]


ROUTE_KINDS = ("unsupported", "wide", "f16_fast", "f16_freq", "f16_gen", "bf3", "fast32", "regs", "lds")


class DensityRoute(C.Structure):
    _fields_ = [("kind", C.c_int32), ("w_lds", C.c_int32), ("waves", C.c_int32), ("dw64", C.c_int32), ("f16_part", C.c_int32)]


class LossConfig(C.Structure):
    _fields_ = [("selection", C.c_int32), ("min_js", C.c_float), ("max_js", C.c_float), ("js_alpha", C.c_float),
                ("los_lambda", C.c_float), ("depth_lambda", C.c_float), ("min_eps", C.c_float),
                ("fixed_eps", C.c_float)]


class MeshGrid(C.Structure):
    _fields_ = [("n", C.c_int32 * 3), ("lo", C.c_float * 3), ("hi", C.c_float * 3), ("first", C.c_double * 3),
                ("inv_step", C.c_double * 3), ("axis", C.c_void_p * 3)]


MC_TABLE_WIDTH = 16

P = C.c_void_p
_SIGNATURES = {
    "lnr_last_error": (C.c_char_p, []),
    "lnr_version": (C.c_int, []),
    "lnr_profile_enable": (C.c_int, [C.c_int32]),
    "lnr_profile_read": (C.c_int, [P, C.c_int32, P, P, C.c_int32]),
    "lnr_net_spec_finalize": (C.c_int, [C.POINTER(NetSpec)]),
    "lnr_density_workspace": (C.c_size_t, [C.POINTER(NetSpec), C.c_int64]),
    "lnr_density_workspace_forward": (C.c_size_t, [C.POINTER(NetSpec), C.c_int64]),
    "lnr_density_route": (C.c_int, [C.POINTER(NetSpec), C.c_int64, C.c_int32, C.POINTER(DensityRoute)]),
    "lnr_density_workspace_init": (C.c_int, [P, C.c_size_t, P]),
    "lnr_density_workspace_release": (C.c_int, [P]),
    "lnr_density_forward": (C.c_int, [C.POINTER(NetSpec), P, P, C.c_int64, P, P, C.c_int32, C.c_int32, P, P, P, C.c_size_t, P]),
    "lnr_density_backward": (C.c_int, [C.POINTER(NetSpec), P, P, C.c_int64, P, P, C.c_int32, C.c_int32, P, P, P, P, P,
                                       C.c_int32, C.c_int32, P, C.c_size_t, P, P]),
    "lnr_density_fold_weight_grads": (C.c_int, [C.POINTER(NetSpec), C.c_int64, P, P, C.c_size_t, C.c_int32, P]),
    "lnr_build_lidar_rays": (C.c_int, [P, P, C.c_int64, P, C.c_int32, P, C.c_float, C.c_float, C.c_float,
                                       C.POINTER(C.c_float), P, P, P, P]),
    "lnr_build_window_rays": (C.c_int, [C.POINTER(C.c_void_p), C.POINTER(C.c_void_p), C.POINTER(C.c_float), C.POINTER(C.c_int64),
                                        C.POINTER(C.c_int32), C.POINTER(C.c_int32), C.c_int32, P, P, C.c_uint64, P, C.c_float, C.c_float,
                                        C.c_float, C.POINTER(C.c_float), P, P, P, P]),
    "lnr_build_camera_rays": (C.c_int, [P, C.c_int64, P, C.c_int32, C.c_int32, P, C.c_float, C.c_float, C.POINTER(C.c_float), P, P]),
    "lnr_pose_forward": (C.c_int, [P, C.c_int32, P, P]),
    "lnr_pose_backward": (C.c_int, [P, P, P, C.c_int32, P, C.c_int32, P, C.c_int32, P]),
    "lnr_compact_rays": (C.c_int, [P, P, P, P, C.c_int32, C.POINTER(C.c_int32), C.c_int32, P, P, P, P, P, P]),
    "lnr_compact_rays_front": (C.c_int, [P, P, P, P, C.c_int32, C.POINTER(C.c_int32), C.c_int32, P, P, P, P, P, P, C.POINTER(C.c_int32), C.c_int32, P, P]),
    "lnr_lidar_rays_backward": (C.c_int, [P, P, P, P, C.c_int32, C.POINTER(C.c_void_p), C.POINTER(C.c_int64), P,
                                          C.c_float, P, P]),
    "lnr_occ_interpolate": (C.c_int, [P, C.c_int32, P, C.c_int64, P, P]),
    "lnr_sample_rays_occ": (C.c_int, [P, C.c_int32, P, P, C.c_int32, C.c_int32, C.c_float, P, P, P, C.c_uint64,
                                      P, P, P, P, P]),
    "lnr_sample_rays_uniform": (C.c_int, [P, C.c_int32, P, C.c_int32, C.c_float, P, P, C.c_uint64, P, P]),
    "lnr_render_forward": (C.c_int, [P, P, P, C.c_int32, P, C.c_int32, P, C.c_float, C.c_uint64, P, P, P, P, P]),
    "lnr_render_forward_peak": (C.c_int, [P, P, P, C.c_int32, P, C.c_int32, P, C.c_float, C.c_uint64, P, P, P, P, P, P]),
    "lnr_depth_colormap": (C.c_int, [P, C.c_int64, C.c_float, C.c_double, C.c_double, P, P, P]),
    "lnr_render_backward": (C.c_int, [P, P, P, C.c_int32, P, C.c_int32, P, C.c_float, C.c_uint64, P, P, P, P, P, P, P]),
    "lnr_render_ftb_gather": (C.c_int, [P, P, C.c_int32, P, P, C.c_int32, C.c_int32, C.c_int32, P, P, P, P]),
    "lnr_render_ftb_composite": (C.c_int, [P, P, P, C.c_int32, P, P, C.c_int32, C.c_int32, C.c_int32, P, C.c_float, C.c_uint64, P, P, P, P, P, C.c_int32, P]),
    "lnr_render_mesh_accumulate": (C.c_int, [P, P, P, C.c_int32, P, C.c_int32, P, C.c_float, C.c_uint64, C.POINTER(MeshGrid),
                                             C.c_float, C.c_int32, C.c_float, P, P, P]),
    "lnr_mc_workspace": (C.c_size_t, [C.c_int32, C.c_int32, C.c_int32]),
    "lnr_mc_count": (C.c_int, [P, C.c_int32, C.c_int32, C.c_int32, C.c_float, P, C.c_size_t, P, P]),
    "lnr_mc_emit": (C.c_int, [P, C.c_int32, C.c_int32, C.c_int32, C.c_float, C.POINTER(C.c_float), C.POINTER(C.c_float), P, C.c_size_t,
                              C.c_int64, C.c_int64, P, P, P]),
    "lnr_mc_case_table": (C.c_int, [P]),
    "lnr_cloud_workspace": (C.c_size_t, [C.c_int64]),
    "lnr_lidar_scan_points": (C.c_int, [P, P, P, C.c_int64, P, C.c_int64, C.c_float, C.c_float, C.c_float, P, C.c_size_t, P, P, P]),
    "lnr_voxel_down_sample": (C.c_int, [P, C.c_int64, P, C.c_double, P, C.c_size_t, P, P, P]),
    "lnr_cloud_append_transformed": (C.c_int, [P, C.c_int64, C.POINTER(C.c_double), P, P]),
    "lnr_nn_grid_bytes": (C.c_size_t, [C.c_int64]),
    "lnr_nn_grid_build": (C.c_int, [P, C.c_int64, C.c_double, P, C.c_size_t, P, C.c_size_t, P, P]),
    "lnr_nn_distance": (C.c_int, [P, C.c_int64, P, C.c_int64, P, P, P, C.c_size_t, P, P]),
    "lnr_cloud_normals": (C.c_int, [P, C.c_int64, C.c_int32, P, P, P, C.c_size_t, P, P]),
    "lnr_icp_correspondences": (C.c_int, [P, C.c_int64, P, C.c_int64, C.c_double, P, P, P, P]),
    "lnr_icp_workspace": (C.c_size_t, [C.c_int64]),
    "lnr_icp_point_to_plane": (C.c_int, [P, C.c_int64, P, P, C.c_int64, C.c_double, C.POINTER(C.c_double), C.c_double, C.c_double,
                                         C.c_int32, P, C.c_size_t, P, P, P]),
    "lnr_mesh_sample_workspace": (C.c_size_t, [C.c_int64]),
    "lnr_mesh_sample_points": (C.c_int, [P, C.c_int64, P, C.c_int64, C.c_int64, C.c_uint64, P, C.c_size_t, P, P, P, P]),
    "lnr_cloud_tools_workspace": (C.c_size_t, [C.c_int64]),
    "lnr_cloud_knn_mean_distance": (C.c_int, [P, C.c_int64, C.c_int32, P, P, C.c_size_t, P, P]),
    "lnr_cloud_outlier_threshold": (C.c_int, [P, P, C.c_int64, C.c_double, P, C.c_size_t, P, P]),
    "lnr_cloud_trajectory_transform": (C.c_int, [P, P, C.c_int64, P, P, P, P, C.c_int64, C.c_double, P, C.c_size_t, P, P, P]),
    "lnr_frame_cloud": (C.c_int, [P, P, C.c_int64, C.c_int64, C.c_int64, C.c_int64, P, P]),
    "lnr_motion_compensate": (C.c_int, [P, P, P, C.c_int32, C.c_int64, C.c_double, C.c_double, C.POINTER(C.c_double), P]),
    "lnr_sky_rays_workspace": (C.c_size_t, []),
    "lnr_sky_rays": (C.c_int, [P, C.c_int64, P, P, C.c_size_t, P, C.c_int64, P, P]),
    "lnr_scan_from_points_workspace": (C.c_size_t, [C.c_int64]),
    "lnr_scan_from_points": (C.c_int, [P, P, C.c_int64, C.c_int32, C.c_float, C.c_int32, C.POINTER(C.c_float), C.c_int32, C.c_float,
                                       P, C.c_size_t, P, P, P, P, P, P]),
    "lnr_points_grad_to_rays": (C.c_int, [P, P, C.c_int32, P, C.c_int32, P, P]),
    "lnr_weights_gt": (C.c_int, [P, P, P, C.c_float, C.c_int32, C.c_int32, C.c_int32, P, P]),
    "lnr_logits_grad": (C.c_int, [P, P, C.c_int32, C.c_int32, C.c_float, C.c_float, C.c_float, P, P]),
    "lnr_count_opaque": (C.c_int, [P, P, C.c_int32, P, P, P, P]),
    "lnr_los_loss_fused": (C.c_int, [P, P, P, P, C.c_int32, P, C.c_int32, P, C.c_float, C.c_uint64, C.c_float,
                                     C.POINTER(LossConfig), P, P, P, P, P, P, P, P, P, C.c_int32, P]),
    "lnr_adam_step": (C.c_int, [P, P, P, P, C.c_int64, C.c_float, C.c_float, C.c_float, C.c_float, C.c_int32,
                                C.c_float, C.c_int32, P, P]),
    "lnr_occ_grid_step": (C.c_int, [P, C.c_int32, P, P, P, C.c_int32, P, C.c_int32, C.c_float, C.c_float, C.c_float,
                                    C.c_float, C.c_float, P, P]),
    "lnr_occ_grid_apply": (C.c_int, [P, P, C.c_int64, C.c_float, C.c_int32, P, P]),
    "lnr_selftest_mfma": (C.c_int, [P, P]),
    "lnr_first_ray_key": (C.c_int, [P, P, C.POINTER(C.c_int32), C.c_int32, P, P]),
    "lnr_rng_draws": (C.c_int, [C.c_int32, C.c_uint64, C.c_int32, C.c_int32, P, P]),
    "lnr_shard_front_pack": (C.c_int, [P, P, C.POINTER(C.c_int32), C.c_int32, P, C.c_int32, P, C.c_int32, P, P]),
    "lnr_shard_front_reduce": (C.c_int, [P, C.c_int32, C.c_int32, P, P, P]),
    "lnr_comm_available": (C.c_int, []),
    "lnr_comm_unique_id": (C.c_int, [P, C.c_size_t]),
    "lnr_comm_init": (C.c_int, [P, C.c_size_t, C.c_int32, C.c_int32, C.POINTER(C.c_void_p)]),
    "lnr_comm_destroy": (C.c_int, [P]),
    "lnr_comm_all_reduce": (C.c_int, [P, P, C.c_size_t, C.c_int32, C.c_int32, P]),
    "lnr_comm_reduce_scatter": (C.c_int, [P, P, P, C.c_size_t, C.c_int32, P]),
    "lnr_comm_all_gather": (C.c_int, [P, P, P, C.c_size_t, P]),
    "lnr_comm_broadcast": (C.c_int, [P, P, C.c_size_t, C.c_int32, P]),
}
COMM_ID_BYTES = 128
COMM_DTYPES = {torch.float32: 0, torch.bfloat16: 1, torch.int64: 2, torch.int32: 3, torch.uint8: 4}
COMM_OPS = {"sum": 0, "min": 1, "max": 2}

_lib = None


def declared_symbols():
    return sorted(_SIGNATURES)


def load():
    global _lib
    if _lib is None:
        if not os.path.exists(LIB_PATH):
            raise RuntimeError(f"{LIB_PATH} not found - build it with `python -m loner_amd.build` "
                               "(there is no CPU fallback for the MI355X hot path)")
        lib = C.CDLL(LIB_PATH)
        for name, (res, args) in _SIGNATURES.items():
            fn = getattr(lib, name)
            fn.restype = res
            fn.argtypes = args
        _lib = lib
    return _lib


def _ptr(t):
    if t is None:
        return None
    if not t.is_contiguous():
        raise RuntimeError("loner_amd: tensor passed to the HIP library must be contiguous")
    return C.c_void_p(t.data_ptr())


_raw_stream = getattr(torch._C, "_cuda_getCurrentRawStream", None)
_raw_device = getattr(torch._C, "_cuda_getDevice", None) or torch.cuda.current_device


def _stream(device=None):
    if _raw_stream is not None and (device is None or isinstance(device, int)):
        return C.c_void_p(_raw_stream(_raw_device() if device is None else device))
    return C.c_void_p(torch.cuda.current_stream(device).cuda_stream)


def check(rc, what=""):
    if rc != 0:
        msg = load().lnr_last_error().decode(errors="replace")
        raise RuntimeError(f"loner_amd HIP call failed ({what}, status {rc}): {msg}")


def require_device(*tensors):
    for t in tensors:
        if t is not None and not t.is_cuda:
            raise RuntimeError("loner_amd: expected a tensor on the MI355X (cuda/hip device), got "
                               f"{t.device}; the hot path has no CPU implementation")


def make_net_spec(encoding_config: dict, network_config: dict) -> NetSpec:
    s = NetSpec()
    otype = str(encoding_config.get("otype", "HashGrid"))
    if otype not in ENCODINGS:
        raise RuntimeError(f"unsupported encoding otype {otype!r} (supported: {sorted(ENCODINGS)})")
    s.encoding = ENCODINGS[otype]
    s.n_levels = int(encoding_config.get("n_levels", 16))
    s.n_features = int(encoding_config.get("n_features_per_level", 2))
    s.log2_table = int(encoding_config.get("log2_hashmap_size", 19))
    s.base_res = int(encoding_config.get("base_resolution", 16))
    s.per_level_scale = float(encoding_config.get("per_level_scale", 2.0))
    s.n_frequencies = int(encoding_config.get("n_frequencies", 12))
    act = str(network_config.get("activation", "ReLU"))
    if act not in ACTIVATIONS:
        raise RuntimeError(f"unsupported activation {act!r}")
    out_act = str(network_config.get("output_activation", "None"))
    if out_act != "None":
        raise RuntimeError(f"output_activation {out_act!r} is not supported (the reference uses None)")
    s.activation = ACTIVATIONS[act]
    s.n_neurons = int(network_config.get("n_neurons", 64))
    s.n_hidden = int(network_config.get("n_hidden_layers", 1))
    prec = str(network_config.get("precision", "fp32"))
    if prec not in PRECISIONS:
        raise RuntimeError(f"unsupported precision {prec!r} (supported: {sorted(PRECISIONS)})")
    s.precision = PRECISIONS[prec]
    pos = str(encoding_config.get("pos_rounding", "fma"))
    if pos not in POS_ROUNDINGS:
        raise RuntimeError(f"unsupported pos_rounding {pos!r} (supported: {sorted(POS_ROUNDINGS)})")
    s.pos_rounding = POS_ROUNDINGS[pos]
    check(load().lnr_net_spec_finalize(C.byref(s)), "lnr_net_spec_finalize")
    return s
```

loner_amd/mapping/optimizer.py:

```python
import os
import time
from dataclasses import dataclass
from typing import List, Tuple

import torch

from .. import hip, ops
from ..common.pose_utils import WorldCube, tensor_to_transform
from ..common.ray_utils import device_scan
from ..models.model_tcnn import Model, OccupancyGridModel
from ..models.ray_sampling import OccGridRaySampler, UniformRaySampler


@dataclass
class OptimizationSettings:
    num_iterations: int = 1
    freeze_poses: bool = False
    latest_kf_only: bool = False
    freeze_sigma_mlp: bool = False
    freeze_rgb_mlp: bool = False

    def from_dict(dict):
        get = lambda k, d: dict[k] if k in dict else d
        return OptimizationSettings(get("num_iterations", 1), get("freeze_poses", False), get("latest_kf_only", False),
                                    get("freeze_sigma_mlp", False), get("freeze_rgb_mlp", False))


class HipAdam(torch.optim.Optimizer):

    def __init__(self, param_groups, poison=None):
        super().__init__(param_groups, dict(lr=1e-3, betas=(0.9, 0.999), eps=1e-8))
        self.poison = poison

    @torch.no_grad()
    def step(self, zero_grad=True, groups=None, ranges=None):
        return self.step_now(zero_grad, groups, ranges)

    @torch.no_grad()
    def step_now(self, zero_grad=True, groups=None, ranges=None):
        if groups is not None and len(groups) == 0:
            return
        for gi, group in enumerate(self.param_groups):
            if groups is not None and gi not in groups:
                continue
            for p in group["params"]:
                if p.grad is None:
                    continue
                st = self.state[p]
                if not st:
                    st["step"] = 0
                    st["exp_avg"] = torch.zeros_like(p)
                    st["exp_avg_sq"] = torch.zeros_like(p)
                st["step"] += 1
                flat = (p.data.view(-1), p.grad.view(-1), st["exp_avg"].view(-1), st["exp_avg_sq"].view(-1))
                for lo, hi in (ranges if ranges is not None else [(0, flat[0].numel())]):
                    ops.adam_step(flat[0][lo:hi], flat[1][lo:hi], flat[2][lo:hi], flat[3][lo:hi],
                                  group["lr"], st["step"], betas=group["betas"], eps=group["eps"], zero_grad=zero_grad,
                                  poison=self.poison)


class _LidarLossFn(torch.autograd.Function):

    @staticmethod
    def forward(ctx, rays, params, opt, depths, iteration_idx):
        out = opt._loss_and_grads(rays.detach().float().contiguous(), depths, params, iteration_idx,
                                  want_ray_grads=rays.requires_grad, want_param_grads=params.requires_grad)
        ctx.save_for_backward(out["d_rays"] if out["d_rays"] is not None else torch.empty(0),
                              out["grad_params"] if out["grad_params"] is not None else torch.empty(0))
        ctx.has = (out["d_rays"] is not None, out["grad_params"] is not None)
        ctx.rays_device = rays.device
        return out["loss"][0].clone()

    @staticmethod
    def backward(ctx, g):
        d_rays, grad_params = ctx.saved_tensors
        return ((g * d_rays).to(ctx.rays_device) if ctx.has[0] else None), (g * grad_params if ctx.has[1] else None), None, None, None


class Optimizer:
    def __init__(self, settings, calibration, world_cube: WorldCube, device, use_gt_poses: bool = False,
                 lidar_only: bool = True, enable_sky_segmentation: bool = True):
        if not torch.cuda.is_available():
            raise RuntimeError("loner_amd.mapping.Optimizer needs an MI355X/HIP device; there is no CPU path")
        hip.load()
        self._settings = settings
        self._calibration = calibration
        self._device = torch.device("cuda", device) if isinstance(device, int) else torch.device(device)
        self._use_gt_poses = use_gt_poses
        self._optimization_settings = OptimizationSettings()
        self._lidar_only = lidar_only
        self._model_config = settings.model_config
        self._scale_factor = world_cube.scale_factor
        self._data_prep_device = 'cpu' if settings.data_prep_on_cpu else self._device
        self._world_cube = world_cube.to(self._data_prep_device)
        self._ray_range = torch.Tensor(list(self._model_config.model.ray_range)).to(self._data_prep_device)
        self._ray_range_f = [float(v) for v in self._ray_range.reshape(-1).cpu()]
        self._scale_f = float(world_cube.scale_factor)
        self._shift_f = [float(v) for v in torch.as_tensor(world_cube.shift).reshape(-1).cpu()]

        self._model = Model(self._model_config.model).to(self._device)

        if self._settings.samples_selection.strategy == 'OGM':
            self._occupancy_grid_model = OccupancyGridModel(self._model_config.model.occ_model).to(self._device)
            self._occupancy_grid = self._occupancy_grid_model()
            occ_params = [p for p in self._occupancy_grid_model.parameters() if p.requires_grad]
            self._occupancy_grid_optimizer = torch.optim.SGD(occ_params, lr=self._model_config.model.occ_model.lr)
            self._ray_sampler = OccGridRaySampler()
            self._ray_sampler.update_occ_grid(self._occupancy_grid.detach())
        elif self._settings.samples_selection.strategy == 'UNIFORM':
            self._ray_sampler = UniformRaySampler()
        else:
            raise RuntimeError(f"Can't find samples_selection strategy: {self._settings.samples_selection.strategy}")
        if not self._lidar_only:
            raise NotImplementedError("camera rays are not enabled in the reference either (optimizer.py:433-434)")

        self._keyframe_count = 0
        self._global_step = 0
        self._keyframe_schedule = self._settings["keyframe_schedule"]
        self._optimizer = None
        self._num_lidar_samples = self._settings.num_samples.lidar
        self._enable_sky_segmentation = enable_sky_segmentation
        self._progress_bar = None

        self._draws = None
        self._dist = None
        self._results_lidar = None
        self._depth_eps = None
        self._grad_buf = None
        self._pipeline = True
        self._side_stream = None
        self._grad_event = None
        self._poison = None
        self.last_failure = None
        self._pc = None
        self._pending_density = None
        self._defer_density_step = True
        self._overwrite_grads = True
        self.last_stats = {}

    def _consts(self):
        pc = self._pc
        if pc is None:
            render, lc = self._model_config.model.render, self._model_config.loss
            if lc.loss_selection not in hip.LOSS_SELECTIONS:
                raise ValueError(f"Can't use unknown Loss {lc.loss_selection}")
            ogm = self._settings.samples_selection.strategy == 'OGM'
            pc = self._pc = dict(
                S=render.N_samples_train, perturb=render.perturb, noise_std=float(render.raw_noise_std), ogm=ogm,
                occ_every=int(self._model_config.model.occ_model.N_iters_acc) if ogm else 0,
                strategy=self._settings.rays_selection.strategy,
                loss=dict(selection=hip.LOSS_SELECTIONS[lc.loss_selection], min_js=lc.JS_loss.min_js_score, max_js=lc.JS_loss.max_js_score,
                          js_alpha=lc.JS_loss.alpha, depth_lambda=lc.depthloss_lambda, min_eps=lc.min_depth_eps,
                          decay_los=bool(lc.decay_los_lambda), los_lambda=lc.los_lambda,
                          los_rate=lc.los_lambda_decay_rate if lc.decay_los_lambda else None,
                          los_steps=lc.los_lambda_decay_steps if lc.decay_los_lambda else None,
                          min_los=lc.min_los_lambda if lc.decay_los_lambda else None,
                          decay_eps=bool(lc.decay_depth_eps), depth_eps=lc.depth_eps,
                          eps_rate=lc.depth_eps_decay_rate if lc.decay_depth_eps else None,
                          eps_steps=lc.depth_eps_decay_steps if lc.decay_depth_eps else None))
        return pc

    def set_draws(self, draws):
        self._draws = draws

    def set_distributed(self, dist_ctx):
        self._dist = dist_ctx

    def iterate_optimizer(self, keyframe_window: List, optimizer_settings: OptimizationSettings = None) -> float:
        cumulative_kf_idx = 0
        for item in self._keyframe_schedule:
            kf_count = item["num_keyframes"]
            iteration_schedule = item["iteration_schedule"]
            cumulative_kf_idx += kf_count
            if cumulative_kf_idx >= self._keyframe_count + 1 or kf_count == -1:
                break
        num_its = sum(i["num_iterations"] for i in iteration_schedule)
        if self._settings.debug.profile_optimizer:
            from torch.profiler import ProfilerActivity, profile, schedule, tensorboard_trace_handler
            prof_dir = f"{self._settings.log_directory}/profile"
            os.makedirs(prof_dir, exist_ok=True)
            prof = profile(activities=[ProfilerActivity.CPU, ProfilerActivity.CUDA], profile_memory=True, record_shapes=True,
                           with_stack=True, with_modules=True, schedule=schedule(wait=1, warmup=1, active=max(num_its - 2, 1)),
                           on_trace_ready=tensorboard_trace_handler(f"{prof_dir}/tensorboard_optimizer/"))
            prof.start()
            start_time = time.time()
            result = self._do_iterate_optimizer(keyframe_window, iteration_schedule, prof, optimizer_settings=optimizer_settings)
            torch.cuda.synchronize(self._device)
            elapsed_time = time.time() - start_time
            prof.stop()
            print(f"Elapsed Time: {elapsed_time}. Per Iteration: {elapsed_time / num_its}, Its/Sec: {num_its / elapsed_time}")
        else:
            start_time = time.time()
            result = self._do_iterate_optimizer(keyframe_window, iteration_schedule, optimizer_settings=optimizer_settings)
            torch.cuda.synchronize(self._device)
            elapsed_time = time.time() - start_time
            os.makedirs(self._settings.log_directory, exist_ok=True)
            with open(f"{self._settings.log_directory}/timing.csv", 'a+') as f:
                f.write(f"{num_its},{elapsed_time}\n")
            if self._progress_bar is None:
                print(f"Elapsed Time: {elapsed_time}. Per Iteration: {elapsed_time / num_its}, Its/Sec: {num_its / elapsed_time}")
        self._keyframe_count += 1
        return result

    def should_enable_lidar(self) -> bool:
        return not self._optimization_settings.freeze_sigma_mlp or not self._optimization_settings.freeze_poses

    def should_enable_camera(self) -> bool:
        return False

    def _do_iterate_optimizer(self, keyframe_window: List, iteration_schedule, profiler=None,
                              optimizer_settings: OptimizationSettings = None) -> float:
        if len(keyframe_window) == 1:
            keyframe_window[0].is_anchored = True
        if len(iteration_schedule) > 1 and self._settings.skip_pose_refinement:
            iteration_schedule = iteration_schedule[1:]
        losses_log, depth_eps_log = [], []
        if optimizer_settings is not None:
            iteration_schedule = [None]

        for iteration_config in iteration_schedule:
            if optimizer_settings is None:
                os_ = self._optimization_settings
                os_.freeze_poses = iteration_config["freeze_poses"] or self._settings.freeze_poses or self._use_gt_poses
                os_.latest_kf_only = iteration_config["latest_kf_only"] if "latest_kf_only" in iteration_config else False
                os_.freeze_rgb_mlp = iteration_config["freeze_rgb_mlp"]
                os_.freeze_sigma_mlp = iteration_config["freeze_sigma_mlp"]
                os_.num_iterations = iteration_config["num_iterations"]
            else:
                self._optimization_settings = optimizer_settings
            os_ = self._optimization_settings
            os_.freeze_poses = os_.freeze_poses or self._settings.freeze_poses or self._use_gt_poses
            self._pc = None
            pc = self._consts()

            if self._settings.samples_selection.strategy == 'OGM':
                self._ray_sampler.update_occ_grid(self._occupancy_grid.detach())
            self._model.freeze_sigma_head(os_.freeze_sigma_mlp)
            self._model.freeze_rgb_head(True)
            optimize_poses = not os_.freeze_poses

            if os_.latest_kf_only:
                active_all = [max(keyframe_window, key=lambda kf: float(kf.get_time()))]
            else:
                active_all = list(keyframe_window)
            active = self._dist.owned(active_all) if self._dist is not None else active_all
            self._active_order = self._dist.owned_indices(len(active_all)) if self._dist is not None else list(range(len(active_all)))
            n_sky_cfg = self._settings.num_samples.sky if self._enable_sky_segmentation else 0
            self._front_cap = self._dist.front_capacity(len(active_all), self._num_lidar_samples + n_sky_cfg) if self._dist is not None else 0
            for kf in active:
                if not kf.is_anchored:
                    kf.get_lidar_pose().set_fixed(not optimize_poses)
            tracking = (not os_.freeze_poses) and os_.freeze_rgb_mlp and os_.freeze_sigma_mlp

            sigma_params = self._model.get_sigma_parameters()
            groups = []
            density_group = None
            if not tracking and sigma_params:
                density_group = len(groups)
                groups.append({'params': sigma_params, 'lr': self._model_config.train.lrate_sigma_mlp})
            pose_objs = [(kf._frame._gt_lidar_pose if self._use_gt_poses else kf.get_lidar_pose()) for kf in active]
            free_list = [bool(optimize_poses and not kf.is_anchored) for kf in active]
            pose_cpu = [p.get_pose_tensor() for p in pose_objs]
            if active and all(p.device.type == "cpu" for p in pose_cpu):
                pose_dev = torch.stack([p.detach().float() for p in pose_cpu]).to(self._device).contiguous()
            elif active:
                pose_dev = torch.stack([p.detach().to(self._device, torch.float32) for p in pose_cpu]).contiguous()
            else:
                pose_dev = torch.zeros(0, 6, device=self._device)
            free_rows = torch.tensor(free_list, device=self._device).to(torch.uint8)
            tab = self._window_tables(active) if active else None
            if tab is not None and not all(free_list):
                with torch.no_grad():
                    fixed = [(torch.zeros(12) if fr else p.get_transformation_matrix().detach().float().cpu()[:3, :4].reshape(12))
                             for p, fr in zip(pose_objs, free_list)]
                tab.fixed_T12 = torch.stack(fixed).to(self._device).contiguous()
                tab.free_col = free_rows.bool()[:, None]
                tab.any_free = any(free_list)
            elif tab is not None:
                tab.fixed_T12 = None
            any_free = bool(optimize_poses and any(not kf.is_anchored for kf in active))
            pose_dev.requires_grad_(any_free)
            if any_free:
                groups.append({'params': [pose_dev], 'lr': self._model_config.train.lrate_pose})
            poison = torch.zeros(2, device=self._device, dtype=torch.int32)
            self._poison = poison
            self._idle_grad_cleared = False
            self._optimizer = HipAdam(groups if groups else [{'params': []}], poison=poison)
            gamma = float(self._model_config.train.lrate_gamma)
            base_lrs = [g['lr'] for g in groups]
            if os_.freeze_sigma_mlp or not self._defer_density_step:
                density_group = None
            n_it = os_.num_iterations
            loss_log = torch.zeros(max(n_it, 1), 8, device=self._device)
            valid_log = torch.zeros(max(n_it, 1), device=self._device, dtype=torch.int32)

            pipelined = len(active) >= 2 and self._dist is None and self._pipeline and profiler is None and self.should_enable_lidar()
            if pipelined:
                main = torch.cuda.current_stream(self._device)
                if self._side_stream is None:
                    self._side_stream = torch.cuda.Stream(self._device)
                    self._grad_event = torch.cuda.Event()
                    self._grad_event.record(main)
                side, ev = self._side_stream, self._grad_event
                sp = sigma_params[0] if sigma_params else self._model.nerf_model._model_sigma.params

                def front_end(it_next):
                    b = self._build_window_rays(active, pose_dev, tab, n_out=valid_log[it_next:it_next + 1])
                    b["front"] = self._sample_front(b["rays"], b["depths"], b["n_dev"], pre=b)
                    return b
                batch = front_end(0) if n_it > 0 else None
                for it_idx in range(n_it):
                    out = self._loss_and_grads(batch["rays"], batch["depths"], sp, it_idx, want_ray_grads=any_free,
                                               want_param_grads=not os_.freeze_sigma_mlp, n_rays_dev=batch["n_dev"],
                                               loss_out=loss_log[it_idx], accumulate_into_param_grad=True, want_stats=False,
                                               defer_grad_wait=True, poison=poison, front=batch["front"], input_grad_event=ev,
                                               defer_weight_fold=density_group is not None)
                    side.wait_event(ev)
                    with torch.cuda.stream(side):
                        if out["grad_params"] is not None and density_group is not None:
                            ops.density_fold_weight_grads(self._model.nerf_model._model_sigma.spec, out["grad_params"],
                                                          batch["rays"].shape[0] * batch["front"]["z"].shape[1],
                                                          overwrite_grad=self._overwrite_grads)
                        if any_free:
                            self._pose_backward(batch, out["d_rays"], pose_dev, free_rows, poison=poison, poison_tag=it_idx)
                        if groups:
                            for g, lr0 in zip(self._optimizer.param_groups, base_lrs):
                                g['lr'] = lr0 * (gamma ** it_idx)
                            dg = density_group if density_group is not None else \
                                (0 if (sigma_params and not tracking and not os_.freeze_sigma_mlp) else None)
                            self._optimizer.step_now(zero_grad=True, groups=tuple(i for i in range(len(groups)) if i != dg))
                        else:
                            dg = None
                        if pc["ogm"] and self._global_step % pc["occ_every"] == 0:
                            self._step_occupancy_grid()
                        if it_idx + 1 < n_it:
                            batch = front_end(it_idx + 1)
                    if groups and dg is not None:
                        if density_group is None:
                            main.wait_stream(side)
                            self._step_density(out["grad_work"], dg)
                        else:
                            self._pending_density = (out["grad_work"], density_group, self._optimizer.param_groups[density_group]['lr'])
                    main.wait_stream(side)
                    self._global_step += 1
                    if self._progress_bar is not None:
                        self._progress_bar.update()
                n_loop = 0
            else:
                n_loop = n_it
            for it_idx in range(n_loop):
                if not self.should_enable_lidar():
                    break
                if active:
                    batch = self._build_window_rays(active, pose_dev, tab, n_out=valid_log[it_idx:it_idx + 1])
                    out = self._loss_and_grads(batch["rays"], batch["depths"], sigma_params[0] if sigma_params else
                                               self._model.nerf_model._model_sigma.params, it_idx, want_ray_grads=any_free,
                                               want_param_grads=not os_.freeze_sigma_mlp, n_rays_dev=batch["n_dev"],
                                               loss_out=loss_log[it_idx], accumulate_into_param_grad=True, want_stats=False,
                                               defer_grad_wait=True, poison=poison, shard_segments=(batch["seg_start"], tab.seg_order_c), pre=batch)
                else:
                    out = self._join_without_rays(sigma_params[0] if sigma_params else None, want_param_grads=not os_.freeze_sigma_mlp)
                if any_free:
                    self._pose_backward(batch, out["d_rays"], pose_dev, free_rows, poison=poison, poison_tag=it_idx)
                if groups:
                    for g, lr0 in zip(self._optimizer.param_groups, base_lrs):
                        g['lr'] = lr0 * (gamma ** it_idx)
                    if density_group is None:
                        dg = 0 if (sigma_params and not tracking and not os_.freeze_sigma_mlp) else None
                        self._optimizer.step_now(zero_grad=True, groups=tuple(i for i in range(len(groups)) if i != dg))
                        if dg is not None:
                            self._step_density(out["grad_work"], dg)
                    else:
                        self._optimizer.step_now(zero_grad=True, groups=tuple(i for i in range(len(groups)) if i != density_group))
                        self._pending_density = (out["grad_work"], density_group, self._optimizer.param_groups[density_group]['lr'])
                if self.should_enable_lidar() and pc["ogm"] and self._global_step % pc["occ_every"] == 0:
                    self._step_occupancy_grid()
                self._global_step += 1
                if profiler is not None:
                    profiler.step()
                if self._progress_bar is not None:
                    self._progress_bar.update()

            self._flush_density_step()
            if self._dist is not None:
                poison.copy_(self._dist.earliest_failure(poison))
            n_log = max(n_it, 1)
            res = self._results_lidar
            if active and n_it and res is not None:
                last = res["rays"]
                n_live_t = res["n_rays_dev"].reshape(1).float() if res["n_rays_dev"] is not None else \
                    torch.full((1,), float(last.shape[0]), device=self._device)
                row = torch.arange(last.shape[0], device=self._device, dtype=torch.float32)[:, None]
                outside = ((last[:, :3].abs() > 1) & (row < n_live_t)).any().reshape(1).float()
            else:
                outside = torch.zeros(1, device=self._device)
            pose_ok = torch.isfinite(pose_dev.detach()).all().reshape(1).float()
            pieces = [poison.view(torch.float32), valid_log.view(torch.float32), loss_log.detach().reshape(-1),
                      pose_dev.detach().reshape(-1).float(), pose_ok, outside]
            host = torch.cat(pieces).cpu().split([p_.numel() for p_ in pieces])
            code, failed_it = (int(v) for v in host[0].view(torch.int32))
            valid_host = host[1].view(torch.int32).float()
            loss_terms_host = host[2].reshape(loss_log.shape).clone()
            pose_host = host[3].reshape(pose_dev.shape)
            pose_finite, origins_outside = bool(host[4][0] != 0), bool(host[5][0] != 0)
            self._poison = None
            self._model.nerf_model.warn_if_clipped(self._device)
            loss_host = loss_terms_host[:, 0]

            def hand_poses_back():
                with torch.no_grad():
                    for k, p_ in enumerate(pose_cpu):
                        if free_list[k]:
                            p_.data.copy_(pose_host[k].to(p_.device))
            if code != 0:
                hand_poses_back()
                self.last_failure = {"code": code, "iteration": failed_it}
                if code == hip.POISON_NAN_LOSS:
                    raise AssertionError("NaN Loss Encountered")
                if code == hip.POISON_POSE_GRAD:
                    raise RuntimeError("Fatal: Encountered invalid gradient in pose.")
                raise RuntimeError("Fatal: Encountered invalid pose tensor.")
            if n_it and torch.isnan(loss_host).any():
                raise AssertionError("NaN Loss Encountered")
            if any_free and not pose_finite:
                raise RuntimeError("Fatal: Encountered invalid pose tensor.")
            if origins_outside:
                raise AssertionError("ray origins are outside the world cube")
            hand_poses_back()
            sigma = self._model.nerf_model._model_sigma.params
            if sigma.grad is not None and os_.freeze_sigma_mlp:
                sigma.grad = None
            elif sigma.grad is not None and self._overwrite_grads and n_it:
                sigma.grad.zero_()
            losses_log.append(loss_host.tolist())
            depth_eps_log.append((loss_terms_host[:, 4] / valid_host.clamp(min=1)).tolist())
            self._depth_eps = depth_eps_log[-1][-1] if n_it else None
            self.last_stats = {"n_valid_rays": int(valid_host.sum().item()), "iterations": n_it, "loss_terms": loss_terms_host}

        if self._settings.debug.log_losses:
            for name, logs in (("losses", losses_log), ("depth_eps", depth_eps_log)):
                d = f"{self._settings.log_directory}/{name}/keyframe_{self._keyframe_count}"
                os.makedirs(d, exist_ok=True)
                for i, log in enumerate(logs):
                    with open(f"{d}/phase_{i}.csv", 'w+') as f:
                        f.write("\n".join(str(v) for v in log))
        return None

    def _window_tables(self, active):
        dev = self._device
        n_lidar = self._num_lidar_samples
        n_sky = self._settings.num_samples.sky if self._enable_sky_segmentation else 0
        rr = [float(self._ray_range[0]), float(self._ray_range[1])]
        dirs_l, dist_l, const_l, counts, poses, is_sky, lens = [], [], [], [], [], [], []
        for k, kf in enumerate(active):
            scan = kf.get_lidar_scan()
            dirs, dist = device_scan(scan, dev)
            dirs_l.append(dirs); dist_l.append(dist); const_l.append(0.0); counts.append(n_lidar); poses.append(k)
            is_sky.append(False); lens.append(dirs.shape[1])
            sky = scan.sky_rays
            if n_sky > 0 and sky is not None and sky.nelement() > 0:
                sdirs = sky.detach().to(dev, torch.float32).contiguous()
                dirs_l.append(sdirs); dist_l.append(None); const_l.append(rr[1] + 1.0); counts.append(n_sky); poses.append(k)
                is_sky.append(True); lens.append(sdirs.shape[1])
        tab = ops.WindowTables(dirs_l, dist_l, const_l, counts, poses)
        tab.is_sky, tab.seg_kf, tab.lens, tab.dirs_list = is_sky, poses, lens, dirs_l
        order_of = getattr(self, "_active_order", None) or list(range(len(active)))
        tab.seg_order = [2 * order_of[k] + (1 if sky_ else 0) for k, sky_ in zip(poses, is_sky)]
        import ctypes as _C
        tab.seg_order_c = (_C.c_int32 * len(tab.seg_order))(*tab.seg_order)
        tab.fixed_T12 = None
        tab.seg_kf_dev = torch.tensor(poses, device=dev)
        tab.lidar_seg_mask = torch.tensor([0.0 if s else 1.0 for s in is_sky], device=dev)[:, None]
        tab.has_sky = any(is_sky)
        return tab

    def _draw_window_indices(self, active, tab):
        strat = self._consts()["strategy"]
        if strat == 'RANDOM' and self._draws is None:
            return None
        out = []
        for s in range(tab.n_seg):
            kf = active[tab.seg_kf[s]]
            count = tab.seg_start_list[s + 1] - tab.seg_start_list[s]
            if tab.is_sky[s]:
                idx = self._draws.sky_index(tab.lens[s], count) if self._draws is not None else \
                    torch.randint(0, tab.lens[s], (count,))
            elif strat == 'RANDOM':
                idx = self._draws.ray_index(tab.lens[s], count)
            elif strat == 'MASK':
                m = kf.get_lidar_scan().mask.nonzero(as_tuple=True)[0]
                idx = m[torch.randint(len(m), (count,))]
            elif strat == 'FIXED':
                idx = torch.arange(count)
            else:
                raise RuntimeError(f"Can't find rays_selection strategy: {strat}")
            out.append(idx.to(self._device))
        return torch.cat(out)

    def _build_window_rays(self, active, pose_dev, tab, n_out=None):
        if tab.fixed_T12 is not None and not tab.any_free:
            T12 = tab.fixed_T12
        else:
            T12 = ops.pose_forward(pose_dev)
            if tab.fixed_T12 is not None:
                T12 = torch.where(tab.free_col, T12, tab.fixed_T12)
        rr = self._ray_range_f
        index = self._draw_window_indices(active, tab)
        seed = int(torch.randint(0, 2 ** 62, (1,)).item()) if index is None else 0
        rays_c, depths_c, keep, src_c = ops.build_window_rays(tab, T12, rr, self._scale_f, self._shift_f, index=index, seed=seed)
        if self._dist is not None:
            rays, depths, src, out_seg, n_dev, rec = ops.compact_rays(rays_c, depths_c, keep, src_c, tab.seg_start, n_out=n_out,
                                                                      front=(tab.seg_order_c, self._front_cap))
            return dict(rays=rays, depths=depths, src=src, seg_start=out_seg, n_dev=n_dev, T12=T12, tab=tab, front_record=rec)
        rays, depths, src, out_seg, n_dev, counts = ops.compact_rays(rays_c, depths_c, keep, src_c, tab.seg_start, n_out=n_out, want_counts=True)
        return dict(rays=rays, depths=depths, src=src, seg_start=out_seg, n_dev=n_dev, T12=T12, tab=tab, counts=counts)

    def _pose_backward(self, batch, d_rays, pose_dev, free_mask_u8, poison=None, poison_tag=0):
        tab = batch["tab"]
        seg_T = batch["T12"] if not tab.has_sky else batch["T12"][tab.seg_kf_dev]
        dT_seg = ops.lidar_rays_backward(d_rays, batch["rays"], batch["src"], batch["seg_start"], tab.dirs_list, seg_T, self._scale_f)
        if tab.has_sky:
            dT = torch.zeros(pose_dev.shape[0], 12, device=self._device).index_add_(0, tab.seg_kf_dev, dT_seg * tab.lidar_seg_mask)
        else:
            dT = dT_seg
        if pose_dev.grad is None:
            pose_dev.grad = ops.pose_backward(pose_dev, dT, mask=free_mask_u8, poison=poison, poison_tag=poison_tag)
        else:
            ops.pose_backward(pose_dev, dT, mask=free_mask_u8, out=pose_dev.grad, accumulate=True, poison=poison, poison_tag=poison_tag)

    def _loss_config(self, iteration_idx) -> hip.LossConfig:
        lc = self._consts()["loss"]
        cfg = hip.LossConfig()
        cfg.selection = lc["selection"]
        cfg.min_js, cfg.max_js, cfg.js_alpha = lc["min_js"], lc["max_js"], lc["js_alpha"]
        if lc["decay_los"]:
            cfg.los_lambda = max(lc["los_lambda"] * (lc["los_rate"] ** ((self._global_step + 1) / lc["los_steps"])), lc["min_los"])
        else:
            cfg.los_lambda = lc["los_lambda"]
        cfg.depth_lambda = lc["depth_lambda"]
        cfg.min_eps = lc["min_eps"]
        if lc["decay_eps"]:
            cfg.fixed_eps = max(lc["depth_eps"] * (lc["eps_rate"] ** (iteration_idx / lc["eps_steps"])), lc["min_eps"])
        else:
            cfg.fixed_eps = lc["depth_eps"]
        return cfg

    def _sample_front(self, rays, depths, n_rays_dev, draws=None, shard_segments=None, pre=None):
        draws = draws if draws is not None else self._draws
        pc = self._consts()
        S, perturb, ogm = pc["S"], pc["perturb"], pc["ogm"]
        dev = self._device
        n = rays.shape[0]
        seed = int(torch.randint(0, 2 ** 62, (1,)).item()) if draws is None else 0
        u1 = u2 = None
        if draws is not None:
            if perturb > 0:
                u1 = draws.jitter(n, S // 2 if ogm else S).to(dev)
            if ogm:
                u2 = draws.pdf(n, S // 2).to(dev)
        counts = far0 = front_work = None
        if self._dist is not None:
            if shard_segments is not None:
                seg_start, seg_order, cap = shard_segments[0], shard_segments[1], self._front_cap
            else:
                seg_start, seg_order = torch.tensor([0, n], device=dev, dtype=torch.int32), [self._dist.rank]
                cap = self._dist.max_over_ranks(n)
            rec = pre.get("front_record") if (pre is not None and shard_segments is not None) else None
            if rec is None:
                rec = ops.shard_front_pack(rays, seg_start, seg_order, depths, n_rays_dev, cap)
            front_work = self._dist.gather_front(rec)
        else:
            counts = pre.get("counts") if pre is not None else None
            if counts is None:
                counts = ops.count_opaque(rays, depths, n_rays_dev=n_rays_dev)
        if ogm:
            z = ops.sample_rays_occ(rays, self._occupancy_grid.detach(), S, perturb, u_jitter=u1, u_pdf=u2, seed=seed,
                                    n_rays_dev=n_rays_dev)
        else:
            z = ops.sample_rays_uniform(rays, S, perturb, u_jitter=u1, seed=seed, n_rays_dev=n_rays_dev)
        return dict(counts=counts, front_work=front_work, z=z, seed=seed, far0=far0)

    def _loss_and_grads(self, rays, depths, params, iteration_idx, want_ray_grads, want_param_grads, n_rays_dev=None,
                        loss_out=None, accumulate_into_param_grad=False, draws=None, want_stats=True, defer_grad_wait=False,
                        poison=None, front=None, input_grad_event=None, defer_weight_fold=False, shard_segments=None, pre=None):
        draws = draws if draws is not None else self._draws
        pc = self._consts()
        S, noise_std = pc["S"], pc["noise_std"]
        spec = self._model.nerf_model._model_sigma.spec
        dev = self._device
        n = rays.shape[0]
        if front is None:
            front = self._sample_front(rays, depths, n_rays_dev, draws, shard_segments=shard_segments, pre=pre)
        counts, front_work, z, seed, far0 = front["counts"], front["front_work"], front["z"], front["seed"], front["far0"]
        noise = None
        if draws is not None and noise_std > 0:
            noise = (draws.noise(n, S) * noise_std).to(dev)
        p = params.detach()
        self._flush_density_step()
        sigma = ops.density_forward(spec, p, rays=rays, z=z, n_rays_dev=n_rays_dev)
        if front_work is not None:
            counts, far0 = front_work.wait()
        loss, d_sigma, d_rays, stats, _ = ops.los_loss_fused(sigma, z, rays, depths, self._scale_f, self._loss_config(iteration_idx),
                                                            counts, noise=noise, noise_std=noise_std, seed=seed + 1,
                                                            n_rays_dev=n_rays_dev, want_stats=want_stats, loss_out=loss_out, far0=far0,
                                                            poison=poison, poison_tag=iteration_idx, zero_dead_rows=not defer_grad_wait)
        grad_params = None
        grad_work = None
        if want_param_grads or want_ray_grads:
            if not want_param_grads:
                grad_params = None
            elif accumulate_into_param_grad:
                if params.grad is None:
                    params.grad = torch.zeros_like(params)
                grad_params = params.grad
            else:
                grad_params = torch.zeros_like(p)
            overwrite = self._overwrite_grads and defer_grad_wait and accumulate_into_param_grad and grad_params is not None
            ops.density_backward(spec, p, d_sigma, grad_params, rays=rays, z=z, n_rays_dev=n_rays_dev,
                                 reuse_features=True, d_rays=d_rays if want_ray_grads else None, input_grad_event=input_grad_event,
                                 defer_weight_fold=defer_weight_fold and grad_params is not None, overwrite_grad=overwrite)
            if self._dist is not None and want_param_grads:
                grad_work = self._dist.exchange_grads(grad_params, async_op=True, force_all_reduce=not defer_grad_wait,
                                                      zero_rest=not overwrite)
                if not defer_grad_wait:
                    grad_work.wait()
                    grad_work = None
        elif input_grad_event is not None:
            input_grad_event.record()
        self._results_lidar = {"rays": rays, "depths": depths, "samples_fine": z, "n_rays_dev": n_rays_dev, "stats": stats}
        return dict(loss=loss, d_rays=d_rays if want_ray_grads else None,
                    grad_params=grad_params if want_param_grads else None, stats=stats, z=z, grad_work=grad_work)

    def _join_without_rays(self, params, want_param_grads):
        dev = self._device
        front_work = self._dist.gather_front(ops.shard_front_pack(None, None, (), None, None, self._front_cap, device=dev))
        self._flush_density_step()
        front_work.wait()
        grad_work = None
        if want_param_grads and params is not None:
            if params.grad is None:
                params.grad = torch.zeros_like(params)
            elif self._overwrite_grads:
                sl = self._dist.owned_range(params.grad.numel())
                if sl is None or not self._idle_grad_cleared:
                    params.grad.zero_()
                    self._idle_grad_cleared = True
                else:
                    params.grad.view(-1)[sl[0]:sl[1]].zero_()
            grad_work = self._dist.exchange_grads(params.grad.view(-1), async_op=True, zero_rest=not self._overwrite_grads)
        self._results_lidar = None
        return dict(loss=None, d_rays=None, grad_params=params.grad if (want_param_grads and params is not None) else None,
                    stats=None, z=None, grad_work=grad_work)

    def _flush_density_step(self):
        if self._pending_density is None:
            return
        work, group, lr = self._pending_density
        self._pending_density = None
        self._optimizer.param_groups[group]['lr'] = lr
        self._step_density(work, group)

    def _step_density(self, work, group):
        if work is not None:
            work.wait()
        ranges = None
        if self._dist is not None:
            sl = self._dist.owned_range(self._model.nerf_model._model_sigma.params.numel())
            if sl is not None:
                ranges = [sl]
        self._optimizer.step_now(zero_grad=not self._overwrite_grads, groups=(group,), ranges=ranges)
        if ranges is not None:
            self._dist.gather_params(self._model.nerf_model._model_sigma.params.data.view(-1))

    def compute_loss(self, camera_samples: Tuple[torch.Tensor, torch.Tensor], lidar_samples: Tuple[torch.Tensor, torch.Tensor],
                     iteration_idx: int, override_enables: bool = False, tracking=False) -> torch.Tensor:
        if not ((override_enables or self.should_enable_lidar()) and lidar_samples is not None):
            print("Warning: zero loss")
            return torch.zeros((), device=self._device)
        rays, depths = lidar_samples
        rays = rays.reshape(-1, rays.shape[-1])
        depths = depths.reshape(-1).to(self._device).float().contiguous()
        self._pc = None
        params = self._model.nerf_model._model_sigma.params
        rays_dev = rays if rays.device == self._device else rays.to(self._device)
        loss = _LidarLossFn.apply(rays_dev, params, self, depths, iteration_idx)
        stats = self._results_lidar["stats"]
        self._results_lidar.update(depth_fine=stats[:, 0], opacity_fine=stats[:, 1], variance=stats[:, 2])
        self._depth_eps = float(stats[:, 6].mean().item())
        assert not torch.isnan(loss), "NaN Loss Encountered"
        return loss

    def compute_loss_api(self, lidar_samples: Tuple[torch.Tensor, torch.Tensor], iteration_idx: int) -> torch.Tensor:
        lc = self._model_config.loss
        self._pc = None
        rays, depths = lidar_samples
        rays = rays.reshape(-1, rays.shape[-1])
        rays = rays if rays.device == self._device else rays.to(self._device)
        scale = self._scale_f
        g = depths.reshape(-1, 1).to(self._device).float() * scale
        transparent = depths.reshape(-1).to(self._device) > rays[0, 12].detach()
        opaque = (depths.reshape(-1).to(self._device) > 0) & ~transparent
        res = self._model(rays, self._ray_sampler, self._scale_factor, camera=False, return_variance=True)
        s = res["samples_fine"] * scale
        w = res["weights_fine"]
        w_sum = w.sum(1) + 1e-10
        mean = (s * w).sum(1) / w_sum
        var = ((s - mean[:, None]) ** 2 * w).sum(1) / w_sum + 1e-10
        std = var.sqrt()
        js = self.calculate_JS_divergence(g, lc.min_depth_eps / 3., mean[:, None], std[:, None]).reshape(-1)
        loss = lc.depthloss_lambda * torch.nn.functional.mse_loss((res["depth_fine"] * scale)[opaque], g[opaque, 0])
        cfg = self._loss_config(iteration_idx)
        if lc.loss_selection in ("L1_JS", "L2_JS"):
            js = torch.where(js < lc.JS_loss.min_js_score, torch.zeros_like(js), js).clamp(max=lc.JS_loss.max_js_score)
            eps = (lc.min_depth_eps * (1 + lc.JS_loss.alpha * js))[:, None].detach()
            self._depth_eps = float(eps.mean().item())
        else:
            eps = cfg.fixed_eps
            self._depth_eps = eps
        from ..models.losses import get_weights_gt
        w_gt = get_weights_gt(s.detach(), g, eps)
        w_gt = w_gt * opaque[:, None]
        los = (w - w_gt).abs().mean() if lc.loss_selection in ("L1_JS", "L1_LOS") else ((w - w_gt) ** 2).mean()
        loss = loss + cfg.los_lambda * los + (res["opacity_fine"][opaque] - 1).abs().mean()
        res.update(rays=rays.detach(), depths=depths.reshape(-1).to(self._device).float(), n_rays_dev=None, stats=None)
        self._results_lidar = res
        assert not torch.isnan(loss), "NaN Loss Encountered"
        return loss

    def _step_occupancy_grid(self):
        res = self._results_lidar
        if res is None and self._dist is None:
            raise RuntimeError("_step_occupancy_grid called before compute_loss")
        occ = self._model_config.model.occ_model
        grid = self._occupancy_grid_model.occupancy_grid
        if self._grad_buf is None:
            self._grad_buf = torch.zeros(grid.numel(), device=grid.device, dtype=torch.int64)
        if res is not None:
            ops.occ_grid_step(grid.data, res["rays"], res["samples_fine"], res["depths"], self._scale_f, occ.lr,
                              grad_buf=self._grad_buf, n_rays_dev=res["n_rays_dev"])
        if self._dist is not None:
            self._dist.all_reduce_grads(self._grad_buf)
        ops.occ_grid_apply(grid.data, self._grad_buf, occ.lr, zero_grad=True, poison=self._poison)
        self._occupancy_grid = self._occupancy_grid_model()
        self._ray_sampler.update_occ_grid(self._occupancy_grid.detach())

    def calculate_KL_divergence(self, mean1, std1, mean2, std2):
        var1, var2 = std1 * std1, std2 * std2
        return torch.log(std2 / std1) + (var1 + (mean1 - mean2) ** 2) / (2 * var2) - 0.5

    def calculate_JS_divergence(self, mean1, std1, mean2, std2):
        mean_m = 0.5 * (mean1 + mean2)
        std_m = 0.5 * torch.sqrt(std1 ** 2 + std2 ** 2)
        return 0.5 * self.calculate_KL_divergence(mean1, std1, mean_m, std_m) + \
            0.5 * self.calculate_KL_divergence(mean2, std2, mean_m, std_m)
```

loner_amd/ops.py:

```python
import ctypes as C
import math
import os

import torch

from . import hip
from .hip import _ptr, _stream, check, load, require_device

_steps_cache = {}


def linspace_table(count: int, device) -> torch.Tensor:
    key = (count, str(device))
    t = _steps_cache.get(key)
    if t is None:
        t = torch.linspace(0, 1, count).to(device)
        _steps_cache[key] = t
    return t


def _f32c(t):
    if t is None:
        return None
    if t.dtype != torch.float32:
# ... 102 lines not shown
        reuse = int(bool(reuse_features))
        if reuse and ent["features_of"] != (params.data_ptr(), pts.data_ptr(), 0, n):
            raise RuntimeError("density_backward(reuse_features=True): workspace features belong to a different forward call")
        d_pts = torch.empty(n, 3, device=params.device, dtype=torch.float32) if want_d_pts else None
        check(load().lnr_density_backward(C.byref(spec), _ptr(params), _ptr(pts), n, None, None, 0, 0, None,
                                          _ptr(d_sigma), _ptr(grad_params), _ptr(d_pts), None, reuse, flags, _ptr(ent["buf"]), need,
                                          _event(input_grad_event), _stream()), "lnr_density_backward")
        return d_pts
    rays, z = _f32c(rays), _f32c(z)
    n, s = z.shape
    reuse = int(bool(reuse_features))
    if reuse and ent["features_of"] != (params.data_ptr(), rays.data_ptr(), z.data_ptr(), n * s):
        raise RuntimeError("density_backward(reuse_features=True): workspace features belong to a different forward call")
    d_pts = torch.empty(n, s, 3, device=params.device, dtype=torch.float32) if want_d_pts else None
    check(load().lnr_density_backward(C.byref(spec), _ptr(params), None, 0, _ptr(rays), _ptr(z), n, s,
                                      _ptr(n_rays_dev), _ptr(d_sigma), _ptr(grad_params), _ptr(d_pts), _ptr(d_rays), reuse, flags,
                                      _ptr(ent["buf"]), need, _event(input_grad_event), _stream()), "lnr_density_backward")
    return d_pts


def density_fold_weight_grads(spec, grad_params, n_points, overwrite_grad=False):
    require_device(grad_params)
    ent, need = _workspace(spec, grad_params.device, n_points)
    check(load().lnr_density_fold_weight_grads(C.byref(spec), int(n_points), _ptr(grad_params), _ptr(ent["buf"]), need,
                                               hip.BWD_OVERWRITE_GRAD if overwrite_grad else 0, _stream()),
          "lnr_density_fold_weight_grads")


def build_lidar_rays(directions, distances, index, transform12, ray_range, scale, shift):
    require_device(directions, distances, index, transform12)
    directions, distances, transform12 = _f32c(directions), _f32c(distances), _f32c(transform12)
    index = index.to(torch.int64).contiguous()
    m = index.shape[0]
    dev = directions.device
    rays = torch.empty(m, hip.RAY_STRIDE, device=dev, dtype=torch.float32)
    depths = torch.empty(m, device=dev, dtype=torch.float32)
    keep = torch.empty(m, device=dev, dtype=torch.uint8)
    sh = (C.c_float * 3)(float(shift[0]), float(shift[1]), float(shift[2]))
    check(load().lnr_build_lidar_rays(_ptr(directions), _ptr(distances), directions.shape[1], _ptr(index), m,
                                      _ptr(transform12), float(ray_range[0]), float(ray_range[1]), float(scale), sh,
                                      _ptr(rays), _ptr(depths), _ptr(keep), _stream()), "lnr_build_lidar_rays")
    return rays, depths, keep


def build_camera_rays(directions, index, width, transform12, range_min, scale, shift):
    require_device(directions, index, transform12)
    directions, transform12 = _f32c(directions), _f32c(transform12)
    assert directions.dim() == 2 and directions.shape[1] == 3 and transform12.numel() == 12
    n_pixels = directions.shape[0]
    if index is not None:
        index = index.to(torch.int64).contiguous()
    n = n_pixels if index is None else index.shape[0]
    rays = torch.empty(n, hip.RAY_STRIDE, device=directions.device, dtype=torch.float32)
    sh = (C.c_float * 3)(float(shift[0]), float(shift[1]), float(shift[2]))
    check(load().lnr_build_camera_rays(_ptr(directions), n_pixels, _ptr(index), n, int(width), _ptr(transform12), float(range_min),
                                       float(scale), sh, _ptr(rays), _stream()), "lnr_build_camera_rays")
    return rays


class WindowTables:

    def __init__(self, dirs_list, dist_list, const_dist, seg_counts, seg_pose):
        n = len(dirs_list)
        self.n_seg = n
        self.keepalive = (list(dirs_list), list(dist_list))
        self.dirs = (C.c_void_p * n)(*[d.data_ptr() for d in dirs_list])
        self.dist = (C.c_void_p * n)(*[(d.data_ptr() if d is not None else None) for d in dist_list])
        self.const_dist = (C.c_float * n)(*[float(c) for c in const_dist])
        self.n_points = (C.c_int64 * n)(*[int(d.shape[1]) for d in dirs_list])
        starts = [0]
        for c in seg_counts:
            starts.append(starts[-1] + int(c))
        self.seg_start_list = starts
        self.seg_start = (C.c_int32 * (n + 1))(*starts)
        self.seg_pose = (C.c_int32 * n)(*[int(p) for p in seg_pose])
        self.total = starts[-1]


def build_window_rays(tab: WindowTables, transforms, ray_range, scale, shift, index=None, seed=0):
    require_device(transforms, index)
    dev = transforms.device
    rays = torch.empty(tab.total, hip.RAY_STRIDE, device=dev, dtype=torch.float32)
    depths = torch.empty(tab.total, device=dev, dtype=torch.float32)
    keep = torch.empty(tab.total, device=dev, dtype=torch.uint8)
    idx_out = None
    if index is None:
        idx_out = torch.empty(tab.total, device=dev, dtype=torch.int64)
    else:
        index = index.to(torch.int64).contiguous()
    sh = (C.c_float * 3)(float(shift[0]), float(shift[1]), float(shift[2]))
    check(load().lnr_build_window_rays(tab.dirs, tab.dist, tab.const_dist, tab.n_points, tab.seg_start, tab.seg_pose, tab.n_seg,
                                       _ptr(index), _ptr(idx_out), int(seed) & (2 ** 64 - 1), _ptr(_f32c(transforms)),
                                       float(ray_range[0]), float(ray_range[1]), float(scale), sh, _ptr(rays), _ptr(depths),
                                       _ptr(keep), _stream()), "lnr_build_window_rays")
    return rays, depths, keep, (index if index is not None else idx_out)


def pose_forward(pose6):
    require_device(pose6)
    p = _f32c(pose6.detach()).reshape(-1, 6)
    T = torch.empty(p.shape[0], 12, device=p.device, dtype=torch.float32)
    if p.shape[0] == 0:
        return T
    check(load().lnr_pose_forward(_ptr(p), p.shape[0], _ptr(T), _stream()), "lnr_pose_forward")
    return T


def pose_backward(pose6, d_transforms, mask=None, out=None, accumulate=False, poison=None, poison_tag=0):
    require_device(pose6, d_transforms, mask, out, poison)
    p = _f32c(pose6.detach()).reshape(-1, 6)
    if out is None:
        out = torch.empty_like(p)
        accumulate = False
    if p.shape[0] == 0:
        return out
    check(load().lnr_pose_backward(_ptr(p), _ptr(_f32c(d_transforms)), _ptr(mask), p.shape[0], _ptr(out), int(accumulate),
                                   _ptr(poison), int(poison_tag), _stream()), "lnr_pose_backward")
    return out


def compact_rays(rays, depths, keep, src_index, seg_start, n_out=None, want_counts=False, front=None):
    require_device(rays, depths, keep, src_index)
    n_in = rays.shape[0]
    dev = rays.device
    n_seg = len(seg_start) - 1
    rays_out = torch.empty_like(rays)
    depths_out = torch.empty_like(depths)
    src_out = torch.empty_like(src_index) if src_index is not None else None
    out_seg = torch.empty(n_seg + 1, device=dev, dtype=torch.int32)
    if n_out is None:
        n_out = torch.empty(1, device=dev, dtype=torch.int32)
    else:
        require_device(n_out)
        assert n_out.dtype == torch.int32 and n_out.numel() == 1 and n_out.is_contiguous()
    seg = seg_start if isinstance(seg_start, C.Array) else (C.c_int32 * (n_seg + 1))(*[int(v) for v in seg_start])
    if want_counts or front is not None:
        counts = rec = order = None
        cap = 0
        if front is not None:
            order, cap = front
            if not isinstance(order, C.Array):
                order = (C.c_int32 * n_seg)(*[int(v) for v in order])
            rec = torch.empty(hip.FRONT_HEADER + int(cap), device=dev, dtype=torch.float32)
        else:
            counts = torch.empty(2, device=dev, dtype=torch.int32)
        check(load().lnr_compact_rays_front(_ptr(rays), _ptr(depths), _ptr(keep), _ptr(src_index), n_in, seg, n_seg,
                                            _ptr(rays_out), _ptr(depths_out), _ptr(src_out), _ptr(out_seg), _ptr(n_out),
                                            _ptr(counts), order, int(cap), _ptr(rec), _stream()), "lnr_compact_rays_front")
        return rays_out, depths_out, src_out, out_seg, n_out, (rec if front is not None else counts)
    check(load().lnr_compact_rays(_ptr(rays), _ptr(depths), _ptr(keep), _ptr(src_index), n_in, seg, n_seg,
                                  _ptr(rays_out), _ptr(depths_out), _ptr(src_out), _ptr(out_seg), _ptr(n_out), _stream()),
          "lnr_compact_rays")
    return rays_out, depths_out, src_out, out_seg, n_out


def first_ray_key(rays, out_seg_start, seg_order):
    require_device(rays, out_seg_start)
    n_seg = len(seg_order)
    key = torch.empty(1, device=rays.device, dtype=torch.int64)
    order = (C.c_int32 * n_seg)(*[int(v) for v in seg_order])
    check(load().lnr_first_ray_key(_ptr(rays), _ptr(out_seg_start), order, n_seg, _ptr(key), _stream()), "lnr_first_ray_key")
    return key


def shard_front_pack(rays, out_seg_start, seg_order, depths, n_rays_dev, cap, device=None):
    dev = rays.device if rays is not None else torch.device(device)
    rec = torch.empty(hip.FRONT_HEADER + int(cap), device=dev, dtype=torch.float32)
    if rays is None:
        check(load().lnr_shard_front_pack(None, None, None, 0, None, 0, None, int(cap), _ptr(rec), _stream()), "lnr_shard_front_pack")
        return rec
    require_device(rays, out_seg_start, depths, n_rays_dev)
    n_seg = len(seg_order)
    order = seg_order if isinstance(seg_order, C.Array) else (C.c_int32 * n_seg)(*[int(v) for v in seg_order])
    check(load().lnr_shard_front_pack(_ptr(rays), _ptr(out_seg_start), order, n_seg, _ptr(_f32c(depths)), rays.shape[0], _ptr(n_rays_dev),
                                      int(cap), _ptr(rec), _stream()), "lnr_shard_front_pack")
    return rec


def shard_front_reduce(records, world, stride):
    require_device(records)
    assert records.dtype == torch.float32 and records.numel() == world * stride
    counts = torch.empty(2, device=records.device, dtype=torch.int32)
    far0 = torch.empty(1, device=records.device, dtype=torch.float32)
    check(load().lnr_shard_front_reduce(_ptr(records), int(world), int(stride), _ptr(counts), _ptr(far0), _stream()), "lnr_shard_front_reduce")
    return counts, far0


def lidar_rays_backward(d_rays, rays, src_index, seg_start_dev, directions_list, transforms, scale):
    require_device(d_rays, rays, src_index, seg_start_dev, transforms)
    n_seg = len(directions_list)
    dev = rays.device
    out = torch.empty(n_seg, 12, device=dev, dtype=torch.float32) if rays.shape[0] > 0 else torch.zeros(n_seg, 12, device=dev)
    ptrs = (C.c_void_p * n_seg)(*[d.data_ptr() for d in directions_list])
    npts = (C.c_int64 * n_seg)(*[int(d.shape[1]) for d in directions_list])
    check(load().lnr_lidar_rays_backward(_ptr(_f32c(d_rays)), _ptr(rays), _ptr(src_index), _ptr(seg_start_dev), n_seg, ptrs,
                                         npts, _ptr(_f32c(transforms)), float(scale), _ptr(out), _stream()),
          "lnr_lidar_rays_backward")
    return out


def occ_interpolate(grid, pts):
    require_device(grid, pts)
    v = grid.shape[-1]
    g = _f32c(grid).reshape(v, v, v)
    p = _f32c(pts)
    out = torch.empty(p.shape[:-1], device=p.device, dtype=torch.float32)
    check(load().lnr_occ_interpolate(_ptr(g), v, _ptr(p), out.numel(), _ptr(out), _stream()), "lnr_occ_interpolate")
    return out


def sample_rays_occ(rays, grid, n_samples, perturb, u_jitter=None, u_pdf=None, seed=0, n_rays_dev=None, debug=False):
    require_device(rays, grid, u_jitter, u_pdf)
    rays = _f32c(rays)
    v = grid.shape[-1]
    g = _f32c(grid).reshape(v, v, v)
    n = rays.shape[0]
    h = n_samples // 2
    steps = linspace_table(h, rays.device)
    z = torch.empty(n, n_samples, device=rays.device, dtype=torch.float32)
    inds = probs = cdf = None
    if debug:
        inds = torch.zeros(n, h, device=rays.device, dtype=torch.int64)
        probs = torch.zeros(n, h, device=rays.device, dtype=torch.float32)
        cdf = torch.zeros(n, h - 1, device=rays.device, dtype=torch.float32)
    check(load().lnr_sample_rays_occ(_ptr(rays), n, _ptr(n_rays_dev), _ptr(g), v, n_samples, float(perturb), _ptr(steps),
                                     _ptr(_f32c(u_jitter)), _ptr(_f32c(u_pdf)), int(seed) & (2 ** 64 - 1), _ptr(z),
                                     _ptr(inds), _ptr(probs), _ptr(cdf), _stream()), "lnr_sample_rays_occ")
    if debug:
        return z, dict(inds=inds, probs=probs, cdf=cdf)
    return z


def sample_rays_uniform(rays, n_samples, perturb, u_jitter=None, seed=0, n_rays_dev=None):
    require_device(rays, u_jitter)
    rays = _f32c(rays)
    n = rays.shape[0]
    steps = linspace_table(n_samples, rays.device)
    z = torch.zeros(n, n_samples, device=rays.device, dtype=torch.float32)
    check(load().lnr_sample_rays_uniform(_ptr(rays), n, _ptr(n_rays_dev), n_samples, float(perturb), _ptr(steps),
                                         _ptr(_f32c(u_jitter)), int(seed) & (2 ** 64 - 1), _ptr(z), _stream()),
          "lnr_sample_rays_uniform")
    return z


def ftb_gather(rays, z, idx, n_alive, b0, block, rays_c, z_c, next_count):
    require_device(rays, z, idx, n_alive, rays_c, z_c, next_count)
    check(load().lnr_render_ftb_gather(_ptr(rays), _ptr(z), z.shape[1], _ptr(idx), _ptr(n_alive), rays.shape[0], int(b0), int(block),
                                       _ptr(rays_c), _ptr(z_c), _ptr(next_count), _stream()), "lnr_render_ftb_gather")


def ftb_composite(sigma_c, z, rays, idx, n_alive, b0, block, noise_std, seed, transmittance, depth_acc, opacity_acc, next_idx, next_count, last, noise=None):
    require_device(sigma_c, z, rays, idx, n_alive, transmittance, depth_acc, opacity_acc, next_idx, next_count, noise)
    check(load().lnr_render_ftb_composite(_ptr(sigma_c), _ptr(z), _ptr(rays), z.shape[1], _ptr(idx), _ptr(n_alive), rays.shape[0], int(b0), int(block),
                                          _ptr(_f32c(noise) if noise is not None else None), float(noise_std), int(seed), _ptr(transmittance), _ptr(depth_acc), _ptr(opacity_acc), _ptr(next_idx),
                                          _ptr(next_count), 1 if last else 0, _stream()), "lnr_render_ftb_composite")


def render_forward(sigma, z, rays, noise=None, noise_std=0.0, seed=0, n_rays_dev=None, want_weights=True):
    require_device(sigma, z, rays, noise)
    sigma, z, rays = _f32c(sigma), _f32c(z), _f32c(rays)
    n, s = z.shape
    dev = z.device
    depth = torch.zeros(n, device=dev); opacity = torch.zeros(n, device=dev); variance = torch.zeros(n, device=dev)
    weights = torch.zeros(n, s, device=dev) if want_weights else None
    check(load().lnr_render_forward(_ptr(sigma), _ptr(z), _ptr(rays), n, _ptr(n_rays_dev), s, _ptr(_f32c(noise)),
                                    float(noise_std), int(seed), _ptr(depth), _ptr(weights), _ptr(opacity), _ptr(variance),
                                    _stream()), "lnr_render_forward")
    return depth, weights, opacity, variance


def render_forward_peak(sigma, z, rays, noise=None, noise_std=0.0, seed=0, n_rays_dev=None):
    require_device(sigma, z, rays, noise)
    sigma, z, rays = _f32c(sigma), _f32c(z), _f32c(rays)
    n, s = z.shape
    dev = z.device
    depth = torch.zeros(n, device=dev); opacity = torch.zeros(n, device=dev); variance = torch.zeros(n, device=dev)
    peak_z = torch.zeros(n, device=dev)
    peak_index = torch.zeros(n, device=dev, dtype=torch.int32)
    check(load().lnr_render_forward_peak(_ptr(sigma), _ptr(z), _ptr(rays), n, _ptr(n_rays_dev), s, _ptr(_f32c(noise)),
                                         float(noise_std), int(seed), _ptr(depth), _ptr(opacity), _ptr(variance), _ptr(peak_z),
                                         _ptr(peak_index), _stream()), "lnr_render_forward_peak")
    return depth, opacity, variance, peak_z, peak_index


def depth_colormap(values, table, multiplier=1.0, min_depth=1.0, max_depth=50.0):
    require_device(values, table)
    values = _f32c(values)
    assert table.dtype == torch.uint8 and table.is_contiguous() and tuple(table.shape) == (256, 3)
    if not float(max_depth) > float(min_depth):
        raise ValueError(f"depth_colormap: max_depth must exceed min_depth, got {min_depth!r} and {max_depth!r}")
    rgba = torch.empty(tuple(values.shape) + (4,), device=values.device, dtype=torch.uint8)
    check(load().lnr_depth_colormap(_ptr(values), values.numel(), float(multiplier), float(min_depth), float(max_depth), _ptr(table),
                                    _ptr(rgba), _stream()), "lnr_depth_colormap")
    return rgba


class MeshLattice:

    def __init__(self, axes, bound, device):
        import numpy as np
        self.axes = [torch.as_tensor(np.asarray(a, dtype=np.float64)).to(device).contiguous() for a in axes]
        self.shape = tuple(int(a.numel()) for a in self.axes)
        g = hip.MeshGrid()
        for i, a in enumerate(axes):
            a = np.asarray(a, dtype=np.float64)
            g.n[i] = a.shape[0]
# ... 379 lines not shown
        raise ValueError(f"scan_from_points: {len(segs)} FOV segments, at most {hip.SCAN_MAX_FOV_SEGMENTS}")
    stamp, min_range = float(stamp), float(min_range)
    if not math.isfinite(stamp) or math.isnan(min_range):
        raise ValueError(f"scan_from_points: stamp must be finite and min_range a number, got {stamp!r} and {min_range!r}")
    mode = hip.SCAN_TIME_NONE if point_times is None else hip.SCAN_TIME_RECOMPUTE if recompute_timestamps else hip.SCAN_TIME_GIVEN
    lib = load()
    dev = xyz.device
    need = int(lib.lnr_scan_from_points_workspace(n))
    if need == 0:
        raise RuntimeError(f"scan_from_points: {n} points, the limit per call is 2^31 - 4096")
    ws = _scan_ws.get(str(dev))
    if ws is None or ws.numel() < need:
        _scan_ws.pop(str(dev), None)
        ws = _scan_ws[str(dev)] = torch.empty(need, device=dev, dtype=torch.uint8)
    dirs = torch.empty(3 * n, device=dev, dtype=torch.float32)
    dist = torch.empty(n, device=dev, dtype=torch.float32)
    times = torch.empty(n, device=dev, dtype=torch.float32)
    order = torch.empty(n, device=dev, dtype=torch.int64)
    info = torch.empty(8, device=dev, dtype=torch.int64)
    flat = (C.c_float * max(2 * len(segs), 1))(*[v for s in segs for v in s])
    times_in = None if mode != hip.SCAN_TIME_GIVEN else point_times.contiguous()
    check(lib.lnr_scan_from_points(_ptr(xyz.contiguous()), _ptr(times_in), n, mode, stamp, int(fov_segments is not None), flat, len(segs),
                                   min_range, _ptr(ws), need, _ptr(dirs), _ptr(dist), _ptr(times), _ptr(order), _ptr(info), _stream()),
          "lnr_scan_from_points")
    info = [int(v) for v in info.cpu()]
    m = info[0]
    return dirs[:3 * m].view(3, m), dist[:m], times[:m], order[:m], info


def _scan_soa(directions, distances, what):
    require_device(directions, distances)
    if directions.dim() != 2 or directions.shape[0] != 3 or distances.dim() != 1 or distances.shape[0] != directions.shape[1]:
        raise ValueError(f"{what}: ray_directions [3,n] and distances [n], got {tuple(directions.shape)} and {tuple(distances.shape)}")
    if directions.dtype != torch.float32 or distances.dtype != torch.float32:
        raise ValueError(f"{what}: ray_directions and distances must be float32")


def frame_cloud(directions, distances, start, stop, step):
    _scan_soa(directions, distances, "frame_cloud")
    n = distances.shape[0]
    start, stop, step = int(start), int(stop), int(step)
    if not (0 <= start and stop <= n and step >= 1):
        raise ValueError(f"frame_cloud: bad window [{start}, {stop}) step {step} of {n} points")
    m = len(range(start, stop, step))
    points = torch.empty(m, 3, device=distances.device, dtype=torch.float64)
    check(load().lnr_frame_cloud(_ptr(_f32c(directions)), _ptr(_f32c(distances)), n, start, stop, step, _ptr(points), _stream()),
          "lnr_frame_cloud")
    return points


def motion_compensate(directions, distances, timestamps, t0, denom, consts):
    _scan_soa(directions, distances, "motion_compensate")
    require_device(timestamps)
    n = distances.shape[0]
    if timestamps.shape != (n,) or timestamps.dtype not in (torch.float32, torch.float64):
        raise ValueError(f"motion_compensate: timestamps [n] float32 or float64, got {tuple(timestamps.shape)} {timestamps.dtype}")
    if not (directions.is_contiguous() and distances.is_contiguous()):
        raise ValueError("motion_compensate: works in place, ray_directions and distances must be contiguous")
    consts = [float(x) for x in consts]
    if len(consts) != hip.MOCOMP_CONSTS:
        raise ValueError(f"motion_compensate: {hip.MOCOMP_CONSTS} constants, got {len(consts)}")
    if not all(math.isfinite(x) for x in consts + [float(t0), float(denom)]):
        raise ValueError("motion_compensate: a pose or a pose time is not finite")
    c = (C.c_double * hip.MOCOMP_CONSTS)(*consts)
    check(load().lnr_motion_compensate(_ptr(directions), _ptr(distances), _ptr(timestamps.contiguous()),
                                       int(timestamps.dtype == torch.float64), n, float(t0), float(denom), c, _stream()),
          "lnr_motion_compensate")


_sky_ws = {}


def sky_rays(directions, rotation):
    require_device(directions, rotation)
    if directions.dim() != 2 or directions.shape[0] != 3 or directions.shape[1] == 0 or directions.dtype != torch.float32:
        raise ValueError(f"sky_rays: ray_directions float32 [3,n] with n >= 1, got {tuple(directions.shape)} {directions.dtype}")
    dev = directions.device
    rot = rotation.detach().to(device=dev, dtype=torch.float32).contiguous()
    if rot.shape != (3, 3):
        raise ValueError(f"sky_rays: rotation [3,3], got {tuple(rot.shape)}")
    lib = load()
    need = int(lib.lnr_sky_rays_workspace())
    held = _sky_ws.get(str(dev))
    if held is None:
        held = _sky_ws[str(dev)] = (torch.empty(need, device=dev, dtype=torch.uint8),
                                    torch.empty(3, hip.SKY_MAX_RAYS, device=dev, dtype=torch.float32))
    ws, sky = held
    info = torch.empty(8, device=dev, dtype=torch.int32)
    check(lib.lnr_sky_rays(_ptr(_f32c(directions)), directions.shape[1], _ptr(rot), _ptr(ws), need, _ptr(sky), hip.SKY_MAX_RAYS,
                           _ptr(info), _stream()), "lnr_sky_rays")
    info = [int(x) for x in info.cpu()]
    if info[0]:
        raise RuntimeError(f"sky_rays: {info[6]} ray directions are not finite")
    return sky[:, :info[1]].contiguous()


def render_backward(sigma, z, rays, g_depth, g_weights, g_opacity, g_variance, noise=None, noise_std=0.0, seed=0,
                    n_rays_dev=None):
    require_device(sigma, z, rays)
    sigma, z, rays = _f32c(sigma), _f32c(z), _f32c(rays)
    n, s = z.shape
    d_sigma = torch.zeros(n, s, device=z.device)
    d_rays = torch.zeros(n, hip.RAY_STRIDE, device=z.device)
    check(load().lnr_render_backward(_ptr(sigma), _ptr(z), _ptr(rays), n, _ptr(n_rays_dev), s, _ptr(_f32c(noise)),
                                     float(noise_std), int(seed), _ptr(_f32c(g_depth)), _ptr(_f32c(g_weights)),
                                     _ptr(_f32c(g_opacity)), _ptr(_f32c(g_variance)), _ptr(d_sigma), _ptr(d_rays), _stream()),
          "lnr_render_backward")
    return d_sigma, d_rays


def points_grad_to_rays(d_pts, z, d_rays, n_rays_dev=None):
    require_device(d_pts, z, d_rays)
    n, s = z.shape
    check(load().lnr_points_grad_to_rays(_ptr(_f32c(d_pts)), _ptr(_f32c(z)), n, _ptr(n_rays_dev), s, _ptr(d_rays), _stream()),
          "lnr_points_grad_to_rays")
    return d_rays


def weights_gt(s, g, eps, normalise=True):
    require_device(s, g)
    s = _f32c(s)
    n, k = s.shape
    g = _f32c(g).reshape(-1)
    out = torch.empty_like(s)
    if isinstance(eps, torch.Tensor):
        require_device(eps)
        e = _f32c(eps).reshape(-1)
        check(load().lnr_weights_gt(_ptr(s), _ptr(g), _ptr(e), 0.0, int(normalise), n, k, _ptr(out), _stream()), "lnr_weights_gt")
    else:
        check(load().lnr_weights_gt(_ptr(s), _ptr(g), None, float(eps), int(normalise), n, k, _ptr(out), _stream()), "lnr_weights_gt")
    return out


def logits_grad(s, g, margin=2.0, l_free=0.25, l_occ=2.5):
    require_device(s, g)
    s = _f32c(s)
    n, k = s.shape
    out = torch.empty_like(s)
    check(load().lnr_logits_grad(_ptr(s), _ptr(_f32c(g).reshape(-1)), n, k, float(margin), float(l_free), float(l_occ),
                                 _ptr(out), _stream()), "lnr_logits_grad")
    return out


def count_opaque(rays, depth_gt, n_rays_dev=None, far0=None):
    require_device(rays, depth_gt, far0)
    counts = torch.empty(2, device=rays.device, dtype=torch.int32)
    check(load().lnr_count_opaque(_ptr(_f32c(rays)), _ptr(_f32c(depth_gt)), rays.shape[0], _ptr(n_rays_dev), _ptr(far0),
                                  _ptr(counts), _stream()), "lnr_count_opaque")
    return counts


def los_loss_fused(sigma, z, rays, depth_gt, scale, cfg: hip.LossConfig, counts, noise=None, noise_std=0.0, seed=0,
                   n_rays_dev=None, want_stats=False, want_weights=False, loss_out=None, far0=None, poison=None, poison_tag=0,
                   zero_dead_rows=True):
    require_device(sigma, z, rays, depth_gt, counts, noise, far0, poison)
    sigma, z, rays, depth_gt = _f32c(sigma), _f32c(z), _f32c(rays), _f32c(depth_gt)
    n, s = z.shape
    dev = z.device
    if loss_out is None:
        loss_out = torch.zeros(8, device=dev)
    d_sigma = torch.empty(n, s, device=dev)
    d_rays = (torch.zeros if (zero_dead_rows and n_rays_dev is not None) else torch.empty)(n, hip.RAY_STRIDE, device=dev)
    stats = torch.zeros(n, 8, device=dev) if want_stats else None
    w = torch.zeros(n, s, device=dev) if want_weights else None
    partials = torch.empty(((n + hip.LOSS_RAYS_PER_BLOCK - 1) // hip.LOSS_RAYS_PER_BLOCK) * 8, device=dev)
    check(load().lnr_los_loss_fused(_ptr(sigma), _ptr(z), _ptr(rays), _ptr(depth_gt), n, _ptr(n_rays_dev), s,
                                    _ptr(_f32c(noise)), float(noise_std), int(seed), float(scale), C.byref(cfg), _ptr(counts),
                                    _ptr(far0), _ptr(loss_out), _ptr(d_sigma), _ptr(d_rays), _ptr(stats), _ptr(w), _ptr(partials),
                                    _ptr(poison), int(poison_tag), _stream()),
          "lnr_los_loss_fused")
    return loss_out, d_sigma, d_rays, stats, w


def adam_step(params, grads, exp_avg, exp_avg_sq, lr, step, betas=(0.9, 0.999), eps=1e-8, grad_scale=1.0, zero_grad=True, poison=None):
    require_device(params, grads, exp_avg, exp_avg_sq, poison)
    check(load().lnr_adam_step(_ptr(params), _ptr(grads), _ptr(exp_avg), _ptr(exp_avg_sq), params.numel(), float(lr),
                               float(betas[0]), float(betas[1]), float(eps), int(step), float(grad_scale), int(zero_grad),
                               _ptr(poison), _stream()), "lnr_adam_step")


def occ_grid_step(grid, rays, z, depth_gt, scale, lr, margin=2.0, l_free=0.25, l_occ=2.5, grad_buf=None, n_rays_dev=None):
    require_device(grid, rays, z, depth_gt, grad_buf)
    assert grad_buf is None or (grad_buf.dtype == torch.int64 and grad_buf.is_contiguous())
    v = grid.shape[-1]
    n, s = z.shape
    check(load().lnr_occ_grid_step(_ptr(grid), v, _ptr(_f32c(rays)), _ptr(_f32c(z)), _ptr(_f32c(depth_gt)), n, _ptr(n_rays_dev),
                                   s, float(scale), float(lr), float(margin), float(l_free), float(l_occ), _ptr(grad_buf),
                                   _stream()), "lnr_occ_grid_step")


def occ_grid_apply(grid, grad_buf, lr, zero_grad=True, poison=None):
    require_device(grid, grad_buf, poison)
    assert grad_buf.dtype == torch.int64 and grad_buf.is_contiguous()
    check(load().lnr_occ_grid_apply(_ptr(grid), _ptr(grad_buf), grid.numel(), float(lr), int(zero_grad), _ptr(poison), _stream()),
          "lnr_occ_grid_apply")


def rng_draws(which, seed, n_rays, n_per_ray, device="cuda"):
    out = torch.empty(int(n_rays), int(n_per_ray), device=device, dtype=torch.float32)
    check(load().lnr_rng_draws(int(which), int(seed) & (2 ** 64 - 1), int(n_rays), int(n_per_ray), _ptr(out), _stream()), "lnr_rng_draws")
    return out


def selftest_mfma(device="cuda"):
    out = torch.full((3,), -1.0, device=device)
    check(load().lnr_selftest_mfma(_ptr(out), _stream()), "lnr_selftest_mfma")
    return float(out.abs().max().item()) if bool((out >= 0).all()) else -1.0
```

Measured before the change: 2.044 million.

## Fuse pose transform, ray build, compaction and opaque count into one window-front kernel

Result: slower. 2.017 million (-1.3%).

```diff
diff --git a/include/loner_hip.h b/include/loner_hip.h
--- a/include/loner_hip.h
+++ b/include/loner_hip.h
@@ -152,6 +152,15 @@
                            int32_t* counts_dev , const int32_t* seg_order , int32_t cap,
                            float* record , void* stream);
 
+int lnr_window_front(const float* const* directions, const float* const* distances, const float* const_distance,
+                     const int64_t* n_points, const int32_t* seg_start, const int32_t* seg_pose, int32_t n_seg,
+                     const float* pose6, const uint8_t* free_mask, const float* fixed_transforms, int32_t n_poses,
+                     const int64_t* index, uint64_t seed, float range_min, float range_max, float scale, const float* shift ,
+                     float* transforms_out, float* rays, float* depths, int64_t* src_index, int64_t* index_out,
+                     int32_t* out_seg_start, int32_t* n_out_dev, int32_t* counts_dev ,
+                     const int32_t* seg_order , int32_t cap, float* record ,
+                     void* stream);
+
 int lnr_first_ray_key(const float* rays, const int32_t* out_seg_start , const int32_t* seg_order ,
                       int32_t n_seg, int64_t* key_out , void* stream);
 
@@ -336,6 +345,7 @@
                              const float* noise , float noise_std, uint64_t seed, float* transmittance, float* depth_acc, float* opacity_acc, int32_t* next_idx, int32_t* next_count_dev,
                              int32_t last, void* stream);
 
+#define LNR_LOSS_REDUCE_LAUNCH 1
 int lnr_count_opaque(const float* rays, const float* depth_gt, int32_t n_rays, const int32_t* n_rays_dev,
                      const float* far0_dev, int32_t* counts_dev , void* stream);
 int lnr_los_loss_fused(const float* sigma, const float* z, const float* rays, const float* depth_gt,
@@ -343,7 +353,8 @@
                        const float* noise, float noise_std, uint64_t seed,
                        float scale, const LnrLossConfig* cfg , const int32_t* counts_dev, const float* far0_dev,
                        float* loss_out, float* d_sigma, float* d_rays, float* ray_stats,
-                       float* weights_out, float* block_partials, int32_t* poison_dev, int32_t poison_tag, void* stream);
+                       float* weights_out, float* block_partials, int32_t* poison_dev, int32_t poison_tag,
+                       int32_t* reduce_counter, int32_t flags, void* stream);
 
 int lnr_adam_step(float* params, float* grads, float* exp_avg, float* exp_avg_sq, int64_t count,
                   float lr, float beta1, float beta2, float eps, int32_t step, float grad_scale,
diff --git a/loner_amd/csrc/lnr_pose.h b/loner_amd/csrc/lnr_pose.h
--- /dev/null
+++ b/loner_amd/csrc/lnr_pose.h
@@ -0,0 +1,26 @@
+#pragma once
+#include "lnr_common.h"
+
+struct QuatParts { float w, x, y, z, k, theta, half; bool small; };
+
+__device__ __forceinline__ QuatParts pose_quat(const float* __restrict__ p) {
+#pragma clang fp contract(fast)
+    QuatParts q;
+    const float a = p[3], b = p[4], c = p[5];
+    q.theta = sqrtf(a * a + b * b + c * c);
+    q.half = 0.5f * q.theta;
+    q.small = fabsf(q.theta) < 1e-6f;
+    q.k = q.small ? 0.5f - q.theta * q.theta / 48.0f : sinf(q.half) / q.theta;
+    q.w = cosf(q.half); q.x = a * q.k; q.y = b * q.k; q.z = c * q.k;
+    return q;
+}
+
+__device__ __forceinline__ void pose_to_T12(const float* __restrict__ p, float* __restrict__ T) {
+#pragma clang fp contract(fast)
+    const QuatParts q = pose_quat(p);
+    const float w = q.w, x = q.x, y = q.y, z = q.z;
+    const float s2 = 2.0f / (w * w + x * x + y * y + z * z);
+    T[0] = 1.0f - s2 * (y * y + z * z); T[1] = s2 * (x * y - z * w);        T[2] = s2 * (x * z + y * w);        T[3] = p[0];
+    T[4] = s2 * (x * y + z * w);        T[5] = 1.0f - s2 * (x * x + z * z); T[6] = s2 * (y * z - x * w);        T[7] = p[1];
+    T[8] = s2 * (x * z - y * w);        T[9] = s2 * (y * z + x * w);        T[10] = 1.0f - s2 * (x * x + y * y); T[11] = p[2];
+}
diff --git a/loner_amd/csrc/lnr_pose.hip b/loner_amd/csrc/lnr_pose.hip
--- a/loner_amd/csrc/lnr_pose.hip
+++ b/loner_amd/csrc/lnr_pose.hip
@@ -1,29 +1,10 @@
 #include "lnr_common.h"
-
-struct QuatParts { float w, x, y, z, k, theta, half; bool small; };
-
-__device__ __forceinline__ QuatParts pose_quat(const float* __restrict__ p) {
-    QuatParts q;
-    const float a = p[3], b = p[4], c = p[5];
-    q.theta = sqrtf(a * a + b * b + c * c);
-    q.half = 0.5f * q.theta;
-    q.small = fabsf(q.theta) < 1e-6f;
-    q.k = q.small ? 0.5f - q.theta * q.theta / 48.0f : sinf(q.half) / q.theta;
-    q.w = cosf(q.half); q.x = a * q.k; q.y = b * q.k; q.z = c * q.k;
-    return q;
-}
+#include "lnr_pose.h"
 
 __global__ void pose_forward_kernel(const float* __restrict__ pose6, int n, float* __restrict__ T12) {
     const int i = blockIdx.x * blockDim.x + threadIdx.x;
     if (i >= n) return;
-    const float* p = pose6 + 6 * i;
-    const QuatParts q = pose_quat(p);
-    const float w = q.w, x = q.x, y = q.y, z = q.z;
-    const float s2 = 2.0f / (w * w + x * x + y * y + z * z);
-    float* T = T12 + 12 * i;
-    T[0] = 1.0f - s2 * (y * y + z * z); T[1] = s2 * (x * y - z * w);        T[2] = s2 * (x * z + y * w);        T[3] = p[0];
-    T[4] = s2 * (x * y + z * w);        T[5] = 1.0f - s2 * (x * x + z * z); T[6] = s2 * (y * z - x * w);        T[7] = p[1];
-    T[8] = s2 * (x * z - y * w);        T[9] = s2 * (y * z + x * w);        T[10] = 1.0f - s2 * (x * x + y * y); T[11] = p[2];
+    pose_to_T12(pose6 + 6 * i, T12 + 12 * i);
 }
 
 __global__ void pose_backward_kernel(const float* __restrict__ pose6, const float* __restrict__ dT12, const uint8_t* __restrict__ mask,
diff --git a/loner_amd/csrc/lnr_rays.hip b/loner_amd/csrc/lnr_rays.hip
--- a/loner_amd/csrc/lnr_rays.hip
+++ b/loner_amd/csrc/lnr_rays.hip
@@ -1,4 +1,5 @@
 #include "lnr_common.h"
+#include "lnr_pose.h"
 
 #define LNR_MAX_SEG 64
 
@@ -318,6 +319,238 @@
     return LNR_OK;
 }
 
+#define LNR_FRONT_HOLD 16
+#define LNR_FRONT_CHUNK 4
+
+struct FrontOut {
+    float* T12; float* rays; float* depths; int64_t* src; int64_t* index_out; int32_t* out_seg_start; int32_t* n_out;
+    int32_t* counts; float* record; int cap;
+};
+
+__device__ __forceinline__ int64_t front_pick(const WindowTable& tab, const int64_t* __restrict__ index, uint64_t seed, int i, int& seg) {
+    while (seg + 1 < tab.n_seg && i >= tab.start[seg + 1]) ++seg;
+    const int64_t n_points = tab.n_points[seg];
+    int64_t src;
+    if (index) src = index[i];
+    else {
+        const float u = lnr_rand_uniform(seed, 0x44ull + (uint64_t)seg, (uint64_t)(i - tab.start[seg]) >> 2, (uint32_t)(i - tab.start[seg]) & 3u);
+        src = (int64_t)(u * (float)n_points);
+        if (src >= n_points) src = n_points - 1;
+    }
+    return src;
+}
+
+struct FrontRay { float o[3], d[3], near, far; bool keep; };
+
+__device__ __forceinline__ FrontRay front_ray(const float* T, float l0, float l1, float l2, float range_min, float range_max, float scale,
+                                              float sx, float sy, float sz) {
+    FrontRay r;
+    float v[3];
+    r.o[0] = (T[3] + sx) / scale; r.o[1] = (T[7] + sy) / scale; r.o[2] = (T[11] + sz) / scale;
+#pragma unroll
+    for (int a = 0; a < 3; ++a) v[a] = T[4 * a] * l0 + T[4 * a + 1] * l1 + T[4 * a + 2] * l2;
+    const float nrm = sqrtf(v[0] * v[0] + v[1] * v[1] + v[2] * v[2]);
+#pragma unroll
+    for (int a = 0; a < 3; ++a) r.d[a] = v[a] / nrm;
+    r.near = range_min / scale;
+    r.far = fminf(range_max / scale, cube_exit(r.o, r.d, nullptr, nullptr, nullptr));
+    r.keep = r.far > r.near + 1.0f / scale;
+    return r;
+}
+
+__device__ __forceinline__ bool front_opaque(float d, float far0) { return (d > 0.0f) && !(d > far0); }
+
+__global__ void __launch_bounds__(256)
+window_front_kernel(const WindowTable tab, const SegOrder ord, const float* __restrict__ pose6, const uint8_t* __restrict__ free_mask,
+                    const float* __restrict__ fixed_T12, int n_pose, const int64_t* __restrict__ index, uint64_t seed, float range_min,
+                    float range_max, float scale, float sx, float sy, float sz, const FrontOut out) {
+    __shared__ float Tl[LNR_MAX_SEG * 12];
+    __shared__ float s_dep[LNR_FRONT_HOLD * 256];
+    __shared__ int s_cnt[4], s_first[4], s_own[4], s_opq[4], s_seg0;
+    __shared__ float s_far0;
+    const int tid = threadIdx.x, lane = tid & 63, wave = tid >> 6, b = blockIdx.x;
+    const int total = tab.start[tab.n_seg];
+    const bool last = b == (int)gridDim.x - 1;
+    const bool hold = last && out.counts != nullptr;
+    if (tid < n_pose) {
+        float T[12];
+        if (free_mask == nullptr || free_mask[tid]) pose_to_T12(pose6 + 6 * tid, T);
+        else {
+#pragma unroll
+            for (int c = 0; c < 12; ++c) T[c] = fixed_T12[12 * tid + c];
+        }
+#pragma unroll
+        for (int c = 0; c < 12; ++c) Tl[12 * tid + c] = T[c];
+        if (b == 0 && out.T12 != nullptr) {
+#pragma unroll
+            for (int c = 0; c < 12; ++c) out.T12[12 * tid + c] = T[c];
+        }
+    }
+    __syncthreads();
+    int cnt = 0, first = 0x7FFFFFFF, first_seg = 0, seg = 0;
+    float first_far = 0.0f;
+    for (int m0 = 0; m0 < b; m0 += LNR_FRONT_CHUNK) {
+        int sg[LNR_FRONT_CHUNK];
+        int64_t src[LNR_FRONT_CHUNK];
+        float l[LNR_FRONT_CHUNK][3], dist[LNR_FRONT_CHUNK];
+#pragma unroll
+        for (int u = 0; u < LNR_FRONT_CHUNK; ++u) {
+            src[u] = front_pick(tab, index, seed, min(m0 + u, b - 1) * 256 + tid, seg);
+            sg[u] = seg;
+        }
+#pragma unroll
+        for (int u = 0; u < LNR_FRONT_CHUNK; ++u) {
+            const float* D = tab.dirs[sg[u]];
+            const int64_t n_points = tab.n_points[sg[u]];
+            l[u][0] = D[src[u]]; l[u][1] = D[n_points + src[u]]; l[u][2] = D[2 * n_points + src[u]];
+            dist[u] = 0.0f;
+            if (hold) dist[u] = tab.dist[sg[u]] ? tab.dist[sg[u]][src[u]] : tab.const_dist[sg[u]];
+        }
+#pragma unroll
+        for (int u = 0; u < LNR_FRONT_CHUNK; ++u) {
+            const int m = m0 + u;
+            const FrontRay r = front_ray(Tl + 12 * tab.pose[sg[u]], l[u][0], l[u][1], l[u][2], range_min, range_max, scale, sx, sy, sz);
+            const bool k = r.keep && m < b;
+            cnt += k ? 1 : 0;
+            if (k && m * 256 + tid < first) { first = m * 256 + tid; first_far = r.far; first_seg = sg[u]; }
+            if (hold && m < b && m < LNR_FRONT_HOLD) s_dep[m * 256 + tid] = k ? dist[u] / scale : 0.0f;
+        }
+    }
+    int wc = cnt, wf = first;
+#pragma unroll
+    for (int o = 32; o > 0; o >>= 1) { wc += __shfl_xor(wc, o, 64); wf = min(wf, __shfl_xor(wf, o, 64)); }
+    if (lane == 0) { s_cnt[wave] = wc; s_first[wave] = wf; }
+    const int i = b * 256 + tid;
+    const bool valid = i < total;
+    int64_t my_src = 0;
+    float my_depth = 0.0f;
+    FrontRay my;
+    my.keep = false;
+    if (valid) {
+        my_src = front_pick(tab, index, seed, i, seg);
+        const float* D = tab.dirs[seg];
+        const int64_t n_points = tab.n_points[seg];
+        const float l0 = D[my_src], l1 = D[n_points + my_src], l2 = D[2 * n_points + my_src];
+        const float dist = tab.dist[seg] ? tab.dist[seg][my_src] : tab.const_dist[seg];
+        my = front_ray(Tl + 12 * tab.pose[seg], l0, l1, l2, range_min, range_max, scale, sx, sy, sz);
+        my_depth = dist / scale;
+    }
+    const bool k = valid && my.keep;
+    const unsigned long long bal = __ballot(k);
+    const int within = __popcll(bal & ((1ull << lane) - 1ull));
+    if (lane == 0) s_own[wave] = __popcll(bal);
+    __syncthreads();
+    const int prefix = s_cnt[0] + s_cnt[1] + s_cnt[2] + s_cnt[3];
+    int pos = prefix + within;
+    for (int w = 0; w < wave; ++w) pos += s_own[w];
+    const int n = prefix + s_own[0] + s_own[1] + s_own[2] + s_own[3];
+    if (valid) {
+        if (out.index_out != nullptr) out.index_out[i] = my_src;
+        for (int s = 0; s <= tab.n_seg; ++s) if (tab.start[s] == i) out.out_seg_start[s] = pos;
+    }
+    if (k) {
+        float* rec = out.rays + (size_t)pos * LNR_RAY_STRIDE;
+        rec[0] = my.o[0]; rec[1] = my.o[1]; rec[2] = my.o[2];
+        rec[3] = my.d[0]; rec[4] = my.d[1]; rec[5] = my.d[2];
+        rec[6] = -my.d[0]; rec[7] = -my.d[1]; rec[8] = -my.d[2];
+        rec[9] = 0.0f; rec[10] = 0.0f; rec[11] = my.near; rec[12] = my.far;
+        out.depths[pos] = my_depth;
+        if (out.src != nullptr) out.src[pos] = my_src;
+        if (out.record != nullptr) out.record[LNR_FRONT_HEADER + pos] = my_depth;
+    }
+    if (!last) return;
+    if (tid <= tab.n_seg && tab.start[tid] >= total) out.out_seg_start[tid] = n;
+    if (tid == 0) *out.n_out = n;
+    if (out.counts == nullptr && out.record == nullptr) return;
+    const int gfirst = min(min(s_first[0], s_first[1]), min(s_first[2], s_first[3]));
+    if (gfirst != 0x7FFFFFFF) {
+        if (first == gfirst) { s_far0 = first_far; s_seg0 = first_seg; }
+    } else if (k && pos == 0) { s_far0 = my.far; s_seg0 = seg; }
+    __syncthreads();
+    if (out.counts != nullptr) {
+        const float far0 = n > 0 ? s_far0 : 0.0f;
+        int c = (k && front_opaque(my_depth, far0)) ? 1 : 0;
+        for (int m = 0; m < min(b, LNR_FRONT_HOLD); ++m) c += front_opaque(s_dep[m * 256 + tid], far0) ? 1 : 0;
+        int seg2 = 0;
+        for (int m = LNR_FRONT_HOLD; m < b; ++m) {
+            const int64_t src2 = front_pick(tab, index, seed, m * 256 + tid, seg2);
+            const float* D = tab.dirs[seg2];
+            const int64_t n_points = tab.n_points[seg2];
+            const float dist = tab.dist[seg2] ? tab.dist[seg2][src2] : tab.const_dist[seg2];
+            const FrontRay r = front_ray(Tl + 12 * tab.pose[seg2], D[src2], D[n_points + src2], D[2 * n_points + src2], range_min, range_max,
+                                         scale, sx, sy, sz);
+            c += (r.keep && front_opaque(dist / scale, far0)) ? 1 : 0;
+        }
+#pragma unroll
+        for (int o = 32; o > 0; o >>= 1) c += __shfl_xor(c, o, 64);
+        if (lane == 0) s_opq[wave] = c;
+        __syncthreads();
+        if (tid == 0) {
+            out.counts[0] = n;
+            out.counts[1] = s_opq[0] + s_opq[1] + s_opq[2] + s_opq[3];
+        }
+    }
+    if (out.record != nullptr) {
+        if (tid == 0) {
+            long long key = 0x7FFFFFFFFFFFFFFFll;
+            if (n > 0) key = ((long long)ord.order[s_seg0] << 32) | (long long)__float_as_uint(s_far0);
+            out.record[0] = __uint_as_float((uint32_t)((unsigned long long)key & 0xFFFFFFFFull));
+            out.record[1] = __uint_as_float((uint32_t)((unsigned long long)key >> 32));
+            out.record[2] = __int_as_float(n);
+            out.record[3] = 0.0f;
+        }
+        for (int j = n + tid; j < out.cap; j += 256) out.record[LNR_FRONT_HEADER + j] = 0.0f;
+    }
+}
+
+extern "C" int lnr_window_front(const float* const* directions, const float* const* distances, const float* const_distance,
+                                const int64_t* n_points, const int32_t* seg_start, const int32_t* seg_pose, int32_t n_seg,
+                                const float* pose6, const uint8_t* free_mask, const float* fixed_transforms, int32_t n_poses,
+                                const int64_t* index, uint64_t seed, float range_min, float range_max, float scale, const float* shift,
+                                float* transforms_out, float* rays, float* depths, int64_t* src_index, int64_t* index_out,
+                                int32_t* out_seg_start, int32_t* n_out_dev, int32_t* counts_dev, const int32_t* seg_order, int32_t cap,
+                                float* record, void* stream) {
+    LNR_REQUIRE(directions && distances && const_distance && n_points && seg_start && seg_pose && shift && rays && depths && out_seg_start && n_out_dev,
+                "lnr_window_front: null argument");
+    LNR_REQUIRE(n_seg >= 1 && n_seg <= LNR_MAX_SEG, "lnr_window_front: n_seg must be in [1,%d]", LNR_MAX_SEG);
+    LNR_REQUIRE(n_poses >= 1 && n_poses <= LNR_MAX_SEG, "lnr_window_front: n_poses must be in [1,%d]", LNR_MAX_SEG);
+    LNR_REQUIRE(free_mask == nullptr ? pose6 != nullptr : fixed_transforms != nullptr,
+                "lnr_window_front: pass pose6 (every pose derived from it) or free_mask with fixed_transforms for the rows it clears");
+    LNR_REQUIRE(free_mask == nullptr || pose6 != nullptr, "lnr_window_front: null argument");
+    LNR_REQUIRE(counts_dev == nullptr || record == nullptr, "lnr_window_front: pass counts_dev (unsharded batch) or record (sharded), not both");
+    LNR_REQUIRE(scale > 0.0f, "lnr_window_front: bad sizes");
+    WindowTable tab;
+    tab.n_seg = n_seg;
+    for (int s = 0; s < n_seg; ++s) {
+        tab.start[s] = seg_start[s]; tab.pose[s] = seg_pose[s]; tab.dirs[s] = directions[s]; tab.dist[s] = distances[s];
+        tab.const_dist[s] = const_distance[s]; tab.n_points[s] = n_points[s];
+        LNR_REQUIRE(directions[s] != nullptr && n_points[s] > 0, "lnr_window_front: segment %d has no points", s);
+        LNR_REQUIRE(seg_pose[s] >= 0 && seg_pose[s] < n_poses, "lnr_window_front: segment %d names pose row %d of %d", s, seg_pose[s], n_poses);
+        LNR_REQUIRE(seg_start[s + 1] >= seg_start[s], "lnr_window_front: seg_start must ascend");
+    }
+    tab.start[n_seg] = seg_start[n_seg];
+    const int total = seg_start[n_seg];
+    LNR_REQUIRE(seg_start[0] == 0 && total >= 0, "lnr_window_front: seg_start must run from 0");
+    SegOrder ord;
+    ord.n = 0;
+    if (record != nullptr) {
+        LNR_REQUIRE(seg_order != nullptr && cap >= total, "lnr_window_front: a front record of %d depth slots cannot hold the %d candidate rays of this rank", cap, total);
+        ord.n = n_seg;
+        for (int s = 0; s < n_seg; ++s) {
+            LNR_REQUIRE(seg_order[s] >= 0 && (s == 0 || seg_order[s] > seg_order[s - 1]), "lnr_window_front: seg_order must be non-negative and ascending");
+            ord.order[s] = seg_order[s];
+        }
+    }
+    FrontOut out;
+    out.T12 = transforms_out; out.rays = rays; out.depths = depths; out.src = src_index; out.index_out = index_out;
+    out.out_seg_start = out_seg_start; out.n_out = n_out_dev; out.counts = counts_dev; out.record = record; out.cap = cap;
+    const int blocks = total > 0 ? lnr_div_up(total, 256) : 1;
+    hipLaunchKernelGGL(window_front_kernel, dim3(blocks), dim3(256), 0, (hipStream_t)stream, tab, ord, pose6, free_mask, fixed_transforms,
+                       n_poses, index, seed, range_min, range_max, scale, shift[0], shift[1], shift[2], out);
+    LNR_CHECK_LAUNCH("lnr_window_front");
+    return LNR_OK;
+}
+
 __global__ void first_ray_key_kernel(const float* __restrict__ rays, const int32_t* __restrict__ out_seg_start, const SegOrder ord, long long* __restrict__ key) {
     if (threadIdx.x != 0 || blockIdx.x != 0) return;
     long long k = 0x7FFFFFFFFFFFFFFFll;
diff --git a/loner_amd/csrc/lnr_render.hip b/loner_amd/csrc/lnr_render.hip
--- a/loner_amd/csrc/lnr_render.hip
+++ b/loner_amd/csrc/lnr_render.hip
@@ -217,6 +217,32 @@
 }
 
 
+template <bool COHERENT>
+__device__ __forceinline__ void loss_reduce_block(const float* block_partials, int n_blocks, float* __restrict__ loss_out,
+                                                  int32_t* __restrict__ poison, int32_t poison_tag, float (*part)[8]) {
+    const int term = threadIdx.x & 7, slice = threadIdx.x >> 3;
+    float v = 0.0f;
+    for (int b = slice; b < n_blocks; b += 32) {
+        const float* p = block_partials + (size_t)b * 8 + term;
+        v += COHERENT ? __hip_atomic_load(p, __ATOMIC_RELAXED, __HIP_MEMORY_SCOPE_AGENT) : *p;
+    }
+    v += __shfl_xor(v, 8, 64); v += __shfl_xor(v, 16, 64); v += __shfl_xor(v, 32, 64);
+    if ((threadIdx.x & 63) < 8) part[threadIdx.x >> 6][term] = v;
+    __syncthreads();
+    if (threadIdx.x < 5) {
+        const float t = loss_out[threadIdx.x] + (part[0][threadIdx.x] + part[1][threadIdx.x] + part[2][threadIdx.x] + part[3][threadIdx.x]);
+        loss_out[threadIdx.x] = t;
+        if (threadIdx.x == 0 && poison != nullptr && t != t && atomicCAS(poison, 0, LNR_POISON_NAN_LOSS) == 0) poison[1] = poison_tag;
+    }
+}
+
+__global__ void __launch_bounds__(256)
+loss_reduce_kernel(const float* __restrict__ block_partials, int n_blocks, float* __restrict__ loss_out,
+                   int32_t* __restrict__ poison, int32_t poison_tag) {
+    __shared__ float part[4][8];
+    loss_reduce_block<false>(block_partials, n_blocks, loss_out, poison, poison_tag, part);
+}
+
 template <int C>
 __global__ void __launch_bounds__(RENDER_BLOCK)
 los_loss_fused_kernel(const float* __restrict__ sigma, const float* __restrict__ z, const float* __restrict__ rays,
@@ -224,7 +250,8 @@
                       const float* __restrict__ noise, float noise_std, uint64_t seed, float scale, const LnrLossConfig cfg,
                       const int32_t* __restrict__ counts, float* __restrict__ loss_out, float* __restrict__ d_sigma,
                       float* __restrict__ d_rays, float* __restrict__ ray_stats, float* __restrict__ weights_out,
-                      float* __restrict__ block_partials, const float* __restrict__ far0_dev) {
+                      float* block_partials, const float* __restrict__ far0_dev, int32_t* __restrict__ done_counter,
+                      int32_t* __restrict__ poison, int32_t poison_tag) {
     __shared__ float s_terms[RAYS_PER_BLOCK][5];
     const int lane = threadIdx.x & 63;
     const int ray = blockIdx.x * RAYS_PER_BLOCK + (threadIdx.x >> 6);
@@ -238,26 +265,25 @@
             float v = 0.0f;
             if (threadIdx.x < 5) for (int r = 0; r < RAYS_PER_BLOCK; ++r) v += s_terms[r][threadIdx.x];
             block_partials[(size_t)blockIdx.x * 8 + threadIdx.x] = v;
+            __threadfence();
+        }
+        if (done_counter != nullptr) {
+            __shared__ int s_last;
+            __shared__ float part[4][8];
+            __syncthreads();
+            if (threadIdx.x == 0) {
+                s_last = atomicAdd(done_counter, 1) == (int)gridDim.x - 1;
+                if (s_last) atomicExch(done_counter, 0);
+            }
+            __syncthreads();
+            if (s_last) {
+                __threadfence();
+                loss_reduce_block<true>(block_partials, (int)gridDim.x, loss_out, poison, poison_tag, part);
+            }
         }
     } else if (alive) {
         los_loss_ray<C>(sigma, z, rays, depth_gt, S, noise, noise_std, seed, scale, cfg, counts, loss_out, true,
                         d_sigma, d_rays, ray_stats, weights_out, ray, lane, far0_dev);
-    }
-}
-
-__global__ void loss_reduce_kernel(const float* __restrict__ block_partials, int n_blocks, float* __restrict__ loss_out,
-                                   int32_t* __restrict__ poison, int32_t poison_tag) {
-    __shared__ float part[4][8];
-    const int term = threadIdx.x & 7, slice = threadIdx.x >> 3;
-    float v = 0.0f;
-    for (int b = slice; b < n_blocks; b += 32) v += block_partials[(size_t)b * 8 + term];
-    v += __shfl_xor(v, 8, 64); v += __shfl_xor(v, 16, 64); v += __shfl_xor(v, 32, 64);
-    if ((threadIdx.x & 63) < 8) part[threadIdx.x >> 6][term] = v;
-    __syncthreads();
-    if (threadIdx.x < 5) {
-        const float t = loss_out[threadIdx.x] + (part[0][threadIdx.x] + part[1][threadIdx.x] + part[2][threadIdx.x] + part[3][threadIdx.x]);
-        loss_out[threadIdx.x] = t;
-        if (threadIdx.x == 0 && poison != nullptr && t != t && atomicCAS(poison, 0, LNR_POISON_NAN_LOSS) == 0) poison[1] = poison_tag;
     }
 }
 
@@ -477,7 +503,7 @@
                                   const int32_t* n_rays_dev, int32_t n_samples, const float* noise, float noise_std, uint64_t seed,
                                   float scale, const LnrLossConfig* cfg, const int32_t* counts_dev, const float* far0_dev, float* loss_out,
                                   float* d_sigma, float* d_rays, float* ray_stats, float* weights_out, float* block_partials,
-                                  int32_t* poison_dev, int32_t poison_tag, void* stream) {
+                                  int32_t* poison_dev, int32_t poison_tag, int32_t* reduce_counter, int32_t flags, void* stream) {
     LNR_REQUIRE(sigma && z && rays && depth_gt && cfg && counts_dev && loss_out && d_sigma && d_rays, "lnr_los_loss_fused: null argument");
     LNR_REQUIRE(poison_dev == nullptr || block_partials != nullptr, "lnr_los_loss_fused: the failure guard needs block_partials (the deterministic reduction)");
     LNR_REQUIRE(cfg->selection >= 0 && cfg->selection <= 3, "lnr_los_loss_fused: unknown loss selection %d", cfg->selection);
@@ -485,11 +511,13 @@
     if (n_rays == 0) return LNR_OK;
     const dim3 grid(lnr_div_up(n_rays, RAYS_PER_BLOCK)), block(RENDER_BLOCK);
     hipStream_t st = (hipStream_t)stream;
+    const bool fused_reduce = block_partials != nullptr && reduce_counter != nullptr && !(flags & LNR_LOSS_REDUCE_LAUNCH);
     DISPATCH_C(n_samples, hipLaunchKernelGGL(los_loss_fused_kernel<C>, grid, block, 0, st, sigma, z, rays, depth_gt, n_rays, n_rays_dev,
                                              n_samples, noise, noise_std, seed, scale, *cfg, counts_dev, loss_out, d_sigma, d_rays,
-                                             ray_stats, weights_out, block_partials, far0_dev));
+                                             ray_stats, weights_out, block_partials, far0_dev, fused_reduce ? reduce_counter : nullptr,
+                                             poison_dev, poison_tag));
     LNR_CHECK_LAUNCH("lnr_los_loss_fused");
-    if (block_partials) {
+    if (block_partials && !fused_reduce) {
         hipLaunchKernelGGL(loss_reduce_kernel, dim3(1), dim3(256), 0, st, block_partials, (int)grid.x, loss_out, poison_dev, poison_tag);
         LNR_CHECK_LAUNCH("lnr_los_loss_fused(reduce)");
     }
diff --git a/loner_amd/hip.py b/loner_amd/hip.py
--- a/loner_amd/hip.py
+++ b/loner_amd/hip.py
@@ -25,6 +25,7 @@
 PRECISIONS = {"fp32": 0, "float32": 0, "fp16": 1, "half": 1, "float16": 1, "fp32_chain": 2}
 POS_ROUNDINGS = {"fma": 0, "mul_add": 1}
 BWD_TABLE_ATOMICS = 1
+LOSS_REDUCE_LAUNCH = 1
 BWD_REPORT_REGIONS = 2
 BWD_DEFER_WEIGHT_FOLD = 16
 BWD_BINS = 4
@@ -93,6 +94,10 @@
     "lnr_pose_backward": (C.c_int, [P, P, P, C.c_int32, P, C.c_int32, P, C.c_int32, P]),
     "lnr_compact_rays": (C.c_int, [P, P, P, P, C.c_int32, C.POINTER(C.c_int32), C.c_int32, P, P, P, P, P, P]),
     "lnr_compact_rays_front": (C.c_int, [P, P, P, P, C.c_int32, C.POINTER(C.c_int32), C.c_int32, P, P, P, P, P, P, C.POINTER(C.c_int32), C.c_int32, P, P]),
+    "lnr_window_front": (C.c_int, [C.POINTER(C.c_void_p), C.POINTER(C.c_void_p), C.POINTER(C.c_float), C.POINTER(C.c_int64),
+                                   C.POINTER(C.c_int32), C.POINTER(C.c_int32), C.c_int32, P, P, P, C.c_int32, P, C.c_uint64, C.c_float,
+                                   C.c_float, C.c_float, C.POINTER(C.c_float), P, P, P, P, P, P, P, P, C.POINTER(C.c_int32), C.c_int32,
+                                   P, P]),
     "lnr_lidar_rays_backward": (C.c_int, [P, P, P, P, C.c_int32, C.POINTER(C.c_void_p), C.POINTER(C.c_int64), P,
                                           C.c_float, P, P]),
     "lnr_occ_interpolate": (C.c_int, [P, C.c_int32, P, C.c_int64, P, P]),
@@ -142,7 +147,7 @@
     "lnr_logits_grad": (C.c_int, [P, P, C.c_int32, C.c_int32, C.c_float, C.c_float, C.c_float, P, P]),
     "lnr_count_opaque": (C.c_int, [P, P, C.c_int32, P, P, P, P]),
     "lnr_los_loss_fused": (C.c_int, [P, P, P, P, C.c_int32, P, C.c_int32, P, C.c_float, C.c_uint64, C.c_float,
-                                     C.POINTER(LossConfig), P, P, P, P, P, P, P, P, P, C.c_int32, P]),
+                                     C.POINTER(LossConfig), P, P, P, P, P, P, P, P, P, C.c_int32, P, C.c_int32, P]),
     "lnr_adam_step": (C.c_int, [P, P, P, P, C.c_int64, C.c_float, C.c_float, C.c_float, C.c_float, C.c_int32,
                                 C.c_float, C.c_int32, P, P]),
     "lnr_occ_grid_step": (C.c_int, [P, C.c_int32, P, P, P, C.c_int32, P, C.c_int32, C.c_float, C.c_float, C.c_float,
diff --git a/loner_amd/mapping/optimizer.py b/loner_amd/mapping/optimizer.py
--- a/loner_amd/mapping/optimizer.py
+++ b/loner_amd/mapping/optimizer.py
@@ -130,6 +130,8 @@
         self._pipeline = True
         self._side_stream = None
         self._grad_event = None
+        self._loss_counter = None
+        self._step_event = None
         self._poison = None
         self.last_failure = None
         self._pc = None
@@ -274,8 +276,7 @@
                     fixed = [(torch.zeros(12) if fr else p.get_transformation_matrix().detach().float().cpu()[:3, :4].reshape(12))
                              for p, fr in zip(pose_objs, free_list)]
                 tab.fixed_T12 = torch.stack(fixed).to(self._device).contiguous()
-                tab.free_col = free_rows.bool()[:, None]
-                tab.any_free = any(free_list)
+                tab.free_u8 = free_rows.contiguous()
             elif tab is not None:
                 tab.fixed_T12 = None
             any_free = bool(optimize_poses and any(not kf.is_anchored for kf in active))
@@ -284,6 +285,7 @@
                 groups.append({'params': [pose_dev], 'lr': self._model_config.train.lrate_pose})
             poison = torch.zeros(2, device=self._device, dtype=torch.int32)
             self._poison = poison
+            self._loss_counter = torch.zeros(1, device=self._device, dtype=torch.int32)
             self._idle_grad_cleared = False
             self._optimizer = HipAdam(groups if groups else [{'params': []}], poison=poison)
             gamma = float(self._model_config.train.lrate_gamma)
@@ -301,7 +303,8 @@
                     self._side_stream = torch.cuda.Stream(self._device)
                     self._grad_event = torch.cuda.Event()
                     self._grad_event.record(main)
-                side, ev = self._side_stream, self._grad_event
+                    self._step_event = torch.cuda.Event()
+                side, ev, ev_step = self._side_stream, self._grad_event, self._step_event
                 sp = sigma_params[0] if sigma_params else self._model.nerf_model._model_sigma.params
 
                 def front_end(it_next):
@@ -323,6 +326,9 @@
                                                           overwrite_grad=self._overwrite_grads)
                         if any_free:
                             self._pose_backward(batch, out["d_rays"], pose_dev, free_rows, poison=poison, poison_tag=it_idx)
+                        early = density_group is not None and bool(groups)
+                        if early:
+                            ev_step.record(side)
                         if groups:
                             for g, lr0 in zip(self._optimizer.param_groups, base_lrs):
                                 g['lr'] = lr0 * (gamma ** it_idx)
@@ -339,6 +345,9 @@
                         if density_group is None:
                             main.wait_stream(side)
                             self._step_density(out["grad_work"], dg)
+                        elif early:
+                            main.wait_event(ev_step)
+                            self._step_density(out["grad_work"], density_group)
                         else:
                             self._pending_density = (out["grad_work"], density_group, self._optimizer.param_groups[density_group]['lr'])
                     main.wait_stream(side)
@@ -404,6 +413,7 @@
             pose_host = host[3].reshape(pose_dev.shape)
             pose_finite, origins_outside = bool(host[4][0] != 0), bool(host[5][0] != 0)
             self._poison = None
+            self._loss_counter = None
             self._model.nerf_model.warn_if_clipped(self._device)
             loss_host = loss_terms_host[:, 0]
 
@@ -498,22 +508,15 @@
         return torch.cat(out)
 
     def _build_window_rays(self, active, pose_dev, tab, n_out=None):
-        if tab.fixed_T12 is not None and not tab.any_free:
-            T12 = tab.fixed_T12
-        else:
-            T12 = ops.pose_forward(pose_dev)
-            if tab.fixed_T12 is not None:
-                T12 = torch.where(tab.free_col, T12, tab.fixed_T12)
         rr = self._ray_range_f
         index = self._draw_window_indices(active, tab)
         seed = int(torch.randint(0, 2 ** 62, (1,)).item()) if index is None else 0
-        rays_c, depths_c, keep, src_c = ops.build_window_rays(tab, T12, rr, self._scale_f, self._shift_f, index=index, seed=seed)
-        if self._dist is not None:
-            rays, depths, src, out_seg, n_dev, rec = ops.compact_rays(rays_c, depths_c, keep, src_c, tab.seg_start, n_out=n_out,
-                                                                      front=(tab.seg_order_c, self._front_cap))
-            return dict(rays=rays, depths=depths, src=src, seg_start=out_seg, n_dev=n_dev, T12=T12, tab=tab, front_record=rec)
-        rays, depths, src, out_seg, n_dev, counts = ops.compact_rays(rays_c, depths_c, keep, src_c, tab.seg_start, n_out=n_out, want_counts=True)
-        return dict(rays=rays, depths=depths, src=src, seg_start=out_seg, n_dev=n_dev, T12=T12, tab=tab, counts=counts)
+        fixed = tab.fixed_T12 is not None
+        b = ops.window_front(tab, pose_dev, rr, self._scale_f, self._shift_f, free_mask=tab.free_u8 if fixed else None,
+                             fixed_T12=tab.fixed_T12, index=index, seed=seed, n_out=n_out, want_counts=self._dist is None,
+                             front=(tab.seg_order_c, self._front_cap) if self._dist is not None else None)
+        b["tab"] = tab
+        return b
 
     def _pose_backward(self, batch, d_rays, pose_dev, free_mask_u8, poison=None, poison_tag=0):
         tab = batch["tab"]
@@ -603,7 +606,8 @@
         loss, d_sigma, d_rays, stats, _ = ops.los_loss_fused(sigma, z, rays, depths, self._scale_f, self._loss_config(iteration_idx),
                                                             counts, noise=noise, noise_std=noise_std, seed=seed + 1,
                                                             n_rays_dev=n_rays_dev, want_stats=want_stats, loss_out=loss_out, far0=far0,
-                                                            poison=poison, poison_tag=iteration_idx, zero_dead_rows=not defer_grad_wait)
+                                                            poison=poison, poison_tag=iteration_idx, zero_dead_rows=not defer_grad_wait,
+                                                            reduce_counter=self._loss_counter if poison is not None else None)
         grad_params = None
         grad_work = None
         if want_param_grads or want_ray_grads:
diff --git a/loner_amd/ops.py b/loner_amd/ops.py
--- a/loner_amd/ops.py
+++ b/loner_amd/ops.py
@@ -278,6 +278,45 @@
                                   _ptr(rays_out), _ptr(depths_out), _ptr(src_out), _ptr(out_seg), _ptr(n_out), _stream()),
           "lnr_compact_rays")
     return rays_out, depths_out, src_out, out_seg, n_out
+
+
+def window_front(tab: WindowTables, pose6, ray_range, scale, shift, free_mask=None, fixed_T12=None, index=None, seed=0, n_out=None,
+                 want_counts=False, front=None, want_index=False):
+    require_device(pose6, free_mask, fixed_T12, index, n_out)
+    p = _f32c(pose6.detach()).reshape(-1, 6)
+    dev = p.device
+    k = p.shape[0]
+    T12 = torch.empty(k, 12, device=dev, dtype=torch.float32)
+    rays = torch.empty(tab.total, hip.RAY_STRIDE, device=dev, dtype=torch.float32)
+    depths = torch.empty(tab.total, device=dev, dtype=torch.float32)
+    src = torch.empty(tab.total, device=dev, dtype=torch.int64)
+    idx_out = torch.empty(tab.total, device=dev, dtype=torch.int64) if want_index else None
+    out_seg = torch.empty(tab.n_seg + 1, device=dev, dtype=torch.int32)
+    if n_out is None:
+        n_out = torch.empty(1, device=dev, dtype=torch.int32)
+    else:
+        assert n_out.dtype == torch.int32 and n_out.numel() == 1 and n_out.is_contiguous()
+    if index is not None:
+        index = index.to(torch.int64).contiguous()
+        assert index.numel() == tab.total
+    if free_mask is not None:
+        assert free_mask.dtype == torch.uint8 and free_mask.numel() == k and fixed_T12 is not None and fixed_T12.shape == (k, 12)
+    counts = rec = order = None
+    cap = 0
+    if front is not None:
+        order, cap = front
+        if not isinstance(order, C.Array):
+            order = (C.c_int32 * tab.n_seg)(*[int(v) for v in order])
+        rec = torch.empty(hip.FRONT_HEADER + int(cap), device=dev, dtype=torch.float32)
+    elif want_counts:
+        counts = torch.empty(2, device=dev, dtype=torch.int32)
+    sh = (C.c_float * 3)(float(shift[0]), float(shift[1]), float(shift[2]))
+    check(load().lnr_window_front(tab.dirs, tab.dist, tab.const_dist, tab.n_points, tab.seg_start, tab.seg_pose, tab.n_seg,
+                                  _ptr(p), _ptr(free_mask), _ptr(_f32c(fixed_T12)) if free_mask is not None else None, k,
+                                  _ptr(index), int(seed) & (2 ** 64 - 1), float(ray_range[0]), float(ray_range[1]), float(scale), sh,
+                                  _ptr(T12), _ptr(rays), _ptr(depths), _ptr(src), _ptr(idx_out), _ptr(out_seg), _ptr(n_out),
+                                  _ptr(counts), order, int(cap), _ptr(rec), _stream()), "lnr_window_front")
+    return dict(T12=T12, rays=rays, depths=depths, src=src, seg_start=out_seg, n_dev=n_out, counts=counts, front_record=rec, index=idx_out)
 
 
 def first_ray_key(rays, out_seg_start, seg_order):
@@ -963,8 +1002,9 @@
 
 def los_loss_fused(sigma, z, rays, depth_gt, scale, cfg: hip.LossConfig, counts, noise=None, noise_std=0.0, seed=0,
                    n_rays_dev=None, want_stats=False, want_weights=False, loss_out=None, far0=None, poison=None, poison_tag=0,
-                   zero_dead_rows=True):
-    require_device(sigma, z, rays, depth_gt, counts, noise, far0, poison)
+                   zero_dead_rows=True, reduce_counter=None, reduce_launch=False):
+    require_device(sigma, z, rays, depth_gt, counts, noise, far0, poison, reduce_counter)
+    assert reduce_counter is None or (reduce_counter.dtype == torch.int32 and reduce_counter.numel() == 1)
     sigma, z, rays, depth_gt = _f32c(sigma), _f32c(z), _f32c(rays), _f32c(depth_gt)
     n, s = z.shape
     dev = z.device
@@ -978,7 +1018,8 @@
     check(load().lnr_los_loss_fused(_ptr(sigma), _ptr(z), _ptr(rays), _ptr(depth_gt), n, _ptr(n_rays_dev), s,
                                     _ptr(_f32c(noise)), float(noise_std), int(seed), float(scale), C.byref(cfg), _ptr(counts),
                                     _ptr(far0), _ptr(loss_out), _ptr(d_sigma), _ptr(d_rays), _ptr(stats), _ptr(w), _ptr(partials),
-                                    _ptr(poison), int(poison_tag), _stream()),
+                                    _ptr(poison), int(poison_tag), _ptr(reduce_counter), hip.LOSS_REDUCE_LAUNCH if reduce_launch else 0,
+                                    _stream()),
           "lnr_los_loss_fused")
     return loss_out, d_sigma, d_rays, stats, w
 
```
